# proycon/analiticcl

Hardware: AMD Instinct MI355X
Metric: scored (query,candidate) pairs/sec + queries/sec, 200k-lexicon, len≤16, 1/2/4/8 GPU (higher is better)
Workload: dtype u8

## Files before the change

### analiticcl_amd/csrc/conf.hip

```cpp
#include <hip/hip_runtime.h>

#include <mutex>
#include <string>
#include <vector>

#include <rocprim/device/device_radix_sort.hpp>

#include "engine_internal.h"

namespace anx {

#define HIP_TRY(expr)                                                                          \
  do {                                                                                         \
    hipError_t _e = (expr);                                                                    \
    if (_e != hipSuccess) {                                                                    \
      err = std::string(#expr) + ": " + hipGetErrorString(_e);                                 \
      return ANX_ENODEVICE;                                                                    \
    }                                                                                          \
  } while (0)

#include "kernels_common.hpp"

struct DeviceConf {
  int device = 0;
// ... 96 lines not shown
      if (need) {
        const uint32_t nin = t1 - t0, c0 = a.v_off[id], ncand = a.v_off[id + 1] - c0, nmin = nin < ncand ? nin : ncand;
        uint32_t p = 0;
        while (p < nmin) {
          const uint32_t x = a.text[t0 + p];
          if (x >= 128u || x != a.v_pool[c0 + p]) break;
          ++p;
        }
        uint32_t sfx = 0;
        while (sfx < nmin - p) {
          const uint32_t x = a.text[t1 - 1u - sfx];
          if (x >= 128u || x != a.v_pool[c0 + ncand - 1u - sfx]) break;
          ++sfx;
        }
        uint64_t im0 = 0, im1 = 0, cm0 = 0, cm1 = 0;
        for (uint32_t x = p; x < nin - sfx; ++x) {
          const uint32_t ch = a.text[t0 + x];
          if (ch < 64u) im0 |= 1ull << ch; else if (ch < 128u) im1 |= 1ull << (ch - 64u);
        }
        for (uint32_t x = p; x < ncand - sfx; ++x) {
          const uint32_t ch = a.v_pool[c0 + x];
          if (ch < 64u) cm0 |= 1ull << ch; else if (ch < 128u) cm1 |= 1ull << (ch - 64u);
        }
        need = false;
        for (uint32_t j = 0; j < a.P.nconf && !need; ++j) {
          const cdiff::FlatConf& cf = a.P.conf[j];
          bool may = true;
          for (uint32_t o_ = 0; o_ < cf.nops && may; ++o_) {
            const cdiff::FlatOp& o = a.P.ops[cf.op_begin + o_];
            if (!o.simple) continue;
            uint64_t h0 = o.bits[0], h1 = o.bits[1];
            if (o.op == '-') { h0 &= im0; h1 &= im1; }
            else if (o.op == '+') { h0 &= cm0; h1 &= cm1; }
            else { h0 &= ins.w[0] & cs.w[0]; h1 &= ins.w[1] & cs.w[1]; }
            if (!(h0 | h1)) may = false;
          }
          need = may;
        }
      }
    }
    a.weight[slot] = 1.0;
    if (need) {
      if (k < 64u) needmask |= 1ull << k;
      else a.need[atomicAdd(&a.ctr[0], 1u)] = make_uint2(slot, s);
    }
  }
  const uint32_t cnt = (uint32_t)__popcll(needmask), lane = threadIdx.x & 63u;
  uint32_t incl = cnt;
#pragma unroll
  for (int o = 1; o < 64; o <<= 1) {
    const uint32_t up = (uint32_t)__shfl_up((int)incl, o);
    if ((int)lane >= o) incl += up;
  }
  const uint32_t total = (uint32_t)__shfl((int)incl, 63);
  if (total == 0) return;
  uint32_t first = 0;
  if (lane == 0) first = atomicAdd(&a.ctr[0], total);
  uint32_t pos = (uint32_t)__shfl((int)first, 0) + incl - cnt;
  for (unsigned long long m = needmask; m; m &= m - 1ull) a.need[pos++] = make_uint2(base + (uint32_t)__ffsll((long long)m) - 1u, s);
}

__global__ void k_conf_iota(uint32_t* p, uint32_t n) {
  const uint32_t i = blockIdx.x * 256 + threadIdx.x;
  if (i < n) p[i] = i;
}
__global__ __launch_bounds__(256) void k_conf_key(ConfArgs a) {
  const uint32_t k = blockIdx.x * 256 + threadIdx.x;
  if (k >= a.row_cap) return;
  uint32_t key = 0x1FFFu;
  if (k < a.ctr[0]) {
    const uint32_t slot = a.need[k].x, s = a.need[k].y, id = row_item(a, slot);
    const uint32_t i = a.q_orig[s], t0 = a.textoff[i], nin = a.textoff[i + 1] - 1u - t0;
    const uint32_t c0 = a.v_off[id], ncand = a.v_off[id + 1] - c0;
    const uint32_t nmin = nin < ncand ? nin : ncand;
    uint32_t p = 0;
    while (p < nmin) {
      const uint32_t x = a.text[t0 + p];
      if (x >= 128u || x != a.v_pool[c0 + p]) break;
      ++p;
    }
    uint32_t sfx = 0;
    while (sfx < nmin - p) {
      const uint32_t x = a.text[t0 + nin - 1u - sfx];
      if (x >= 128u || x != a.v_pool[c0 + ncand - 1u - sfx]) break;
      ++sfx;
    }
    const uint32_t ma = nin - p - sfx, mb = ncand - p - sfx;
    key = ((ma < 6u ? ma : 6u) << 5) | ((mb < 6u ? mb : 6u) << 2) | (p ? 2u : 0u) | (sfx ? 1u : 0u);
    key = key << 5 | (nin < 31u ? nin : 31u);
  }
  a.key[k] = key;
}

__global__ __launch_bounds__(CF_THREADS) void k_conf_script(ConfArgs a) {
  const uint32_t n = a.ctr[0];
  static_assert(CF_THREADS == 64, "one wave per block: the lane memories of a wave interleave");
  cdiff::Ctx c;
  c.mem = a.work + (size_t)blockIdx.x * CF_WORDS * 64u + threadIdx.x * CF_G;
  c.arena_off = CF_ARENA_OFF; c.arena_cap = CF_ARENA; c.arena_used = 0;
  c.d_off = CF_D_OFF; c.d_cap = CF_DIFFS; c.nd = 0;
  c.v_off = CF_V_OFF; c.v_cap = CF_V;
  c.f_off = CF_F_OFF; c.frame_cap = CF_FRAMES;
  c.alpha = a.alpha; c.nalpha = a.nalpha;
  c.overflow = false;
  for (uint32_t k = blockIdx.x * CF_THREADS + threadIdx.x; k < n; k += gridDim.x * CF_THREADS) {
    const uint2 nd = a.need[a.order[k]];
    const uint32_t slot = nd.x, s = nd.y, id = row_item(a, slot);
    const uint32_t i = a.q_orig[s], t0 = a.textoff[i], t1 = a.textoff[i + 1] - 1u;
    uint32_t nin = 0;
    bool fits = true;
    for (uint32_t p = t0; p < t1;) {
      const uint32_t b0 = a.text[p];
      uint32_t cp = b0, len = 1;
      const uint32_t avail = t1 - p;
      if (b0 >= 0xC0u && b0 < 0xE0u && avail >= 2 && (a.text[p + 1] & 0xC0u) == 0x80u) { cp = ((b0 & 0x1Fu) << 6) | (a.text[p + 1] & 0x3Fu); len = 2; }
      else if (b0 >= 0xE0u && b0 < 0xF0u && avail >= 3 && (a.text[p + 1] & 0xC0u) == 0x80u && (a.text[p + 2] & 0xC0u) == 0x80u) {
        cp = ((b0 & 0x0Fu) << 12) | ((a.text[p + 1] & 0x3Fu) << 6) | (a.text[p + 2] & 0x3Fu); len = 3;
      } else if (b0 >= 0xF0u && b0 < 0xF8u && avail >= 4 && (a.text[p + 1] & 0xC0u) == 0x80u && (a.text[p + 2] & 0xC0u) == 0x80u && (a.text[p + 3] & 0xC0u) == 0x80u) {
        cp = ((b0 & 0x07u) << 18) | ((a.text[p + 1] & 0x3Fu) << 12) | ((a.text[p + 2] & 0x3Fu) << 6) | (a.text[p + 3] & 0x3Fu); len = 4;
      }
      if (nin >= CF_MAXCP) { fits = false; break; }
      DC::W(c, CF_IN_OFF + nin++) = cp;
      p += len;
    }
    const uint32_t c0 = a.v_off[id], ncand = a.v_off[id + 1] - c0;
    double w = 1.0;
    bool ok = fits && ncand <= CF_MAXCP;
    if (ok) {
      for (uint32_t x = 0; x < ncand; ++x) DC::W(c, CF_CAND_OFF + x) = a.v_pool[c0 + x];
      const cdiff::View in = cdiff::mk(CF_IN_OFF, nin), cand = cdiff::mk(CF_CAND_OFF, ncand);
      ok = DC::confusable_weight(c, a.P, in, DC::charset_of(c, in), cand, a.v_cs[id], &w);
    }
    if (!ok) atomicAdd(&a.ctr[1], 1u);
    a.weight[slot] = w;
  }
}

__global__ __launch_bounds__(256) void k_conf_apply_early(ConfArgs a) {
  const uint32_t slot = blockIdx.x * 256 + threadIdx.x;
  if (slot >= a.soff[a.nq] || a.soff[a.nq] > a.row_cap) return;
  const double w = a.weight[slot];
  if (w != 1.0) a.c_rows[slot].score *= w;
}

__device__ inline double conf_vr_score(const DevRow& r, float fw) {
  if (fw == 0.0f) return r.dist_score;
  return (r.dist_score + ((double)fw * r.freq_score)) / (1.0 + (double)fw);
}
__device__ inline bool conf_before(const DevRow& x, const DevRow& y, float fw) {
  if (fw > 0.0f) return conf_vr_score(x, fw) > conf_vr_score(y, fw);
  if (x.dist_score != y.dist_score) return x.dist_score > y.dist_score;
  return x.freq_score > y.freq_score;
}
__global__ __launch_bounds__(256) void k_conf_apply_late(ConfArgs a, uint32_t* __restrict__ r_count) {
  const uint32_t s = blockIdx.x * 256 + threadIdx.x;
  if (s >= a.nq || a.soff[a.nq] > a.row_cap || *a.overflow) return;
  const uint32_t n = r_count[s], base = a.soff[s];
  if (n == 0) return;
  DevRow* __restrict__ v = a.r_rows + base;
  bool any = false;
  for (uint32_t k = 0; k < n; ++k) {
    const double w = a.weight[base + k];
    if (w != 1.0) { v[k].dist_score *= w; any = true; }
  }
  if (any)
    for (uint32_t k = 1; k < n; ++k) {
      const DevRow x = v[k];
      uint32_t j = k;
      while (j > 0 && conf_before(x, v[j - 1], a.freq_weight)) { v[j] = v[j - 1]; --j; }
      v[j] = x;
    }
  uint32_t len = n;
  if (a.cutoff_threshold >= 1.0) {
    const double best = conf_vr_score(v[0], a.freq_weight);
    for (uint32_t k = 1; k < n; ++k)
      if (conf_vr_score(v[k], a.freq_weight) <= best / a.cutoff_threshold) { len = k; break; }
  }
  r_count[s] = len;
}

namespace {
std::mutex g_conf_mu;
template <typename T>
int cf_upload(T** dst, const void* src, size_t count, std::string& err) {
  if (*dst) { pool_free(*dst); *dst = nullptr; }
  HIP_TRY(pool_malloc(reinterpret_cast<void**>(dst), std::max<size_t>(count * sizeof(T), 16)));
  if (count) HIP_TRY(hipMemcpy(*dst, src, count * sizeof(T), hipMemcpyHostToDevice));
  return ANX_OK;
}
}

void conf_free(DeviceConf* dc) {
  if (!dc) return;
  (void)hipSetDevice(dc->device);
  for (void* p : {(void*)dc->conf, (void*)dc->ops, (void*)dc->opts, (void*)dc->pool, (void*)dc->v_pool, (void*)dc->v_off, (void*)dc->v_cs, (void*)dc->alpha})
    if (p) pool_free(p);
  delete dc;
}

static int conf_ensure(const HostModel& m, const DeviceLexicon* dl, std::string& err) {
  std::lock_guard<std::mutex> g(g_conf_mu);
  DeviceConf*& dc = dl->dconf;
  if (!dc) { dc = new DeviceConf(); dc->device = dl->device; }
  int rc;
  if (dc->built_patterns != m.confusables.size() || !dc->conf) {
    const HostModel::ConfTables& t = m.conf_tables;
    if ((rc = cf_upload(&dc->conf, t.conf.data(), t.conf.size(), err)) || (rc = cf_upload(&dc->ops, t.ops.data(), t.ops.size(), err)) ||
        (rc = cf_upload(&dc->opts, t.opts.data(), t.opts.size(), err)) || (rc = cf_upload(&dc->pool, t.pool.data(), t.pool.size(), err)))
      return rc;
    dc->nconf = (uint32_t)t.conf.size();
    dc->built_patterns = m.confusables.size();
  }
  if (dc->built_vocab != m.decoder.size() || !dc->v_cs) {
    const uint32_t *pool, *off;
    const void* cs;
    size_t npool, n;
    m.conf_vocab_arrays(&pool, &npool, &off, &cs, &n);
    if ((rc = cf_upload(&dc->v_pool, pool, npool, err)) || (rc = cf_upload(&dc->v_off, off, n + 1, err)) ||
        (rc = cf_upload(&dc->v_cs, cs, n, err)))
      return rc;
    dc->nvocab = (uint32_t)n;
    dc->built_vocab = m.decoder.size();
  }
  if (!dc->alpha) {
    uint32_t na = 0;
    const uint32_t(*al)[2] = alphabetic_ranges(&na);
    uint32_t* p = nullptr;
    if ((rc = cf_upload(&p, al, (size_t)na * 2, err))) return rc;
    dc->alpha = reinterpret_cast<uint32_t(*)[2]>(p);
    dc->nalpha = na;
  }
  return ANX_OK;
}

int conf_launch(const HostModel& m, const DeviceLexicon* dl, Batch* b, hipStream_t st, bool early, uint32_t row_cap, std::string& err) {
  int rc = conf_ensure(m, dl, err);
  if (rc) return rc;
  b->conf_skipped = false;
  const DeviceConf* dc = dl->dconf;
  const uint32_t nq = (uint32_t)b->nq;
  if (!b->cf_weight || b->cf_cap < row_cap) {
    for (void* p : {(void*)b->cf_weight, (void*)b->cf_need, (void*)b->cf_sort, b->cf_sort_tmp})
      if (p) pool_free(p);
    b->cf_weight = nullptr; b->cf_need = nullptr; b->cf_sort = nullptr; b->cf_sort_tmp = nullptr;
    HIP_TRY(pool_malloc(reinterpret_cast<void**>(&b->cf_weight), std::max<size_t>((size_t)row_cap * sizeof(double), 16)));
    HIP_TRY(pool_malloc(reinterpret_cast<void**>(&b->cf_need), std::max<size_t>((size_t)row_cap * sizeof(uint2), 16)));
    b->cf_cap = row_cap;
  }
  if (!b->cf_sort) {
    HIP_TRY(pool_malloc(reinterpret_cast<void**>(&b->cf_sort), std::max<size_t>(4 * (size_t)row_cap * sizeof(uint32_t), 16)));
    size_t bytes = 0;
    HIP_TRY(rocprim::radix_sort_pairs(nullptr, bytes, b->cf_sort, b->cf_sort, b->cf_sort, b->cf_sort, (size_t)row_cap, 0u, 13u, st));
    HIP_TRY(pool_malloc(&b->cf_sort_tmp, std::max<size_t>(bytes, 16)));
    b->cf_sort_tmp_bytes = bytes;
  }
  uint32_t* sort_buf = b->cf_sort;
  if (!b->cf_ctr) HIP_TRY(pool_malloc(reinterpret_cast<void**>(&b->cf_ctr), 16));
  const uint32_t cf_blocks = std::min<uint32_t>(CF_BLOCKS, std::max<uint32_t>(1u, (row_cap + 63u) / 64u));
  if (b->cf_work && b->cf_work_blocks < cf_blocks) { pool_free(b->cf_work); b->cf_work = nullptr; }
  if (!b->cf_work) {
    if (pool_malloc(&b->cf_work, (size_t)cf_blocks * CF_WORDS * 64u * sizeof(uint32_t)) != hipSuccess) {
      b->cf_work = nullptr;
      (void)hipGetLastError();
      b->conf_skipped = true;
      return ANX_OK;
    }
    b->cf_work_blocks = cf_blocks;
  }
  HIP_TRY(hipMemsetAsync(b->cf_ctr, 0, 16, st));
  ConfArgs a;
  a.nq = nq; a.row_cap = row_cap; a.early = early ? 1 : 0; a.soff = b->soff; a.r_count = b->r_count; a.c_rows = b->c_rows; a.r_rows = b->r_rows;
  a.overflow = b->counters + CTR_OVERFLOW;
  a.q_orig = b->q_orig; a.text = b->d_text; a.textoff = b->d_textoff; a.weight = b->cf_weight; a.need = reinterpret_cast<uint2*>(b->cf_need); a.ctr = b->cf_ctr;
  a.P.conf = dc->conf; a.P.nconf = dc->nconf; a.P.ops = dc->ops; a.P.opts = dc->opts; a.P.pool = dc->pool;
  a.v_pool = dc->v_pool; a.v_off = dc->v_off; a.v_cs = dc->v_cs; a.nvocab = dc->nvocab;
  a.alpha = dc->alpha; a.nalpha = dc->nalpha; a.work = static_cast<uint32_t*>(b->cf_work);
  a.key = sort_buf; a.order = sort_buf + 3 * (size_t)row_cap;
  a.cutoff_threshold = b->params.cutoff_threshold; a.freq_weight = b->params.freq_weight;
  const uint32_t nblk = (row_cap + 255u) / 256u;
  hipLaunchKernelGGL(k_conf_screen, dim3((nq + 255u) / 256u), dim3(256), 0, st, a);
  if (nblk) {
    hipLaunchKernelGGL(k_conf_key, dim3(nblk), dim3(256), 0, st, a);
    hipLaunchKernelGGL(k_conf_iota, dim3(nblk), dim3(256), 0, st, sort_buf + (size_t)row_cap, row_cap);
    HIP_TRY(rocprim::radix_sort_pairs(b->cf_sort_tmp, b->cf_sort_tmp_bytes, sort_buf, sort_buf + 2 * (size_t)row_cap, sort_buf + (size_t)row_cap,
                                      sort_buf + 3 * (size_t)row_cap, (size_t)row_cap, 0u, 13u, st));
  }
  const int kt = ktimer_begin("k_conf_script", st);
  hipLaunchKernelGGL(k_conf_script, dim3(b->cf_work_blocks), dim3(CF_THREADS), 0, st, a);
  ktimer_end(kt, st);
  if (early) { if (nblk) hipLaunchKernelGGL(k_conf_apply_early, dim3(nblk), dim3(256), 0, st, a); }
  else hipLaunchKernelGGL(k_conf_apply_late, dim3((nq + 255u) / 256u), dim3(256), 0, st, a, b->r_count);
  HIP_TRY(hipGetLastError());
  return ANX_OK;
}

}
```

### analiticcl_amd/csrc/engine.hip

```cpp
#include <hip/hip_runtime.h>

#include <algorithm>
#include <atomic>
#include <functional>
#include <chrono>
#include <cmath>
#include <cstdio>
#include <cstdlib>
#include <cstring>
#include <map>
#include <memory>
#include <mutex>
#include <unordered_map>
#include <numeric>
#include <thread>
#include <type_traits>

#include "engine_internal.h"

namespace anx {

#define HIP_TRY(expr)                                                                          \
  do {                                                                                         \
    hipError_t _e = (expr);                                                                    \
    if (_e != hipSuccess) {                                                                    \
      err = std::string(#expr) + ": " + hipGetErrorString(_e);                                 \
      return ANX_ENODEVICE;                                                                    \
    }                                                                                          \
  } while (0)

#include "kernels_common.hpp"
#include "kernels_swar.hpp"
#include "kernels_scan.hpp"
#include "kernels_prefix.hpp"
#include "kernels_score.hpp"
#include "kernels_rank.hpp"

enum { HR_RCTR = 0, HR_SCTR = SCAN_REGIONS * RC_STRIDE, HR_LCTR = 2 * SCAN_REGIONS * RC_STRIDE, HR_CTR = 5 * SCAN_REGIONS * RC_STRIDE,
       HR_TOTAL_SURV = HR_CTR + CTR_N, HR_TOTAL_RESULTS = HR_TOTAL_SURV + 1, HR_CONF = HR_TOTAL_RESULTS + 1 , HR_N = HR_CONF + 2 };
constexpr size_t HR_COLD_OFF = (HR_N * sizeof(uint32_t) + 63) & ~(size_t)63;
static void shells_destroy(int device);
static void small_ctxs_destroy(int device);

int device_count(std::string& err) {
  int n = 0;
  hipError_t e = hipGetDeviceCount(&n);
  if (e != hipSuccess) {
    err = std::string("hipGetDeviceCount: ") + hipGetErrorString(e);
    return 0;
  }
  return n;
}

struct SmallCtx;
namespace {
struct DevPool {
  std::mutex mu;
  std::multimap<size_t, void*> free_blocks;
  std::unordered_map<void*, size_t> size_of;
  size_t cached = 0;
  std::unordered_map<void*, uint64_t> freed_at;
  uint64_t clock = 0;
  int lexicons = 0;
  std::vector<hipStream_t> idle_streams;
  hipStream_t run_streams[2] = {nullptr, nullptr};
  unsigned run_counter = 0;
  std::vector<BatchShell> shells;
  std::vector<SmallCtx*> small_idle;
  std::vector<std::pair<void*, size_t>> doomed;
  size_t doomed_bytes = 0;
};
static size_t pool_cache_limit() {
  static const size_t lim = []() {
    const char* e = getenv("ANX_POOL_CACHE_MB");
    const long long v = e ? atoll(e) : -1;
    return v >= 0 ? (size_t)v << 20 : (size_t)96 << 30;
  }();
  return lim;
}
DevPool& pool_of(int device) {
  static DevPool pools[64];
  return pools[device >= 0 && device < 64 ? device : 0];
}
}
static thread_local hipStream_t t_encoder_stream = nullptr;
void* make_stream(bool high) {
  hipStream_t s = nullptr;
  int least = 0, greatest = 0;
  if (high && switches().enc_priority && hipDeviceGetStreamPriorityRange(&least, &greatest) == hipSuccess && greatest < least) {
    if (hipStreamCreateWithPriority(&s, hipStreamNonBlocking, greatest) == hipSuccess) return s;
    (void)hipGetLastError();
  }
  if (hipStreamCreateWithFlags(&s, hipStreamNonBlocking) != hipSuccess) { (void)hipGetLastError(); return nullptr; }
  return s;
}
void encoder_stream_set_override(void* s) { t_encoder_stream = reinterpret_cast<hipStream_t>(s); }
hipStream_t encoder_stream_acquire(int device) {
  if (t_encoder_stream) return t_encoder_stream;
  DevPool& pl = pool_of(device);
  {
    std::lock_guard<std::mutex> g(pl.mu);
    if (!pl.idle_streams.empty()) { hipStream_t s = pl.idle_streams.back(); pl.idle_streams.pop_back(); return s; }
  }
  return static_cast<hipStream_t>(make_stream(true));
}
void encoder_stream_release(int device, hipStream_t s) {
  if (!s || s == t_encoder_stream) return;
  DevPool& pl = pool_of(device);
  std::lock_guard<std::mutex> g(pl.mu);
  pl.idle_streams.push_back(s);
}
struct DeviceGuard {
  int prev = -1;
  DeviceGuard() { if (hipGetDevice(&prev) != hipSuccess) { prev = -1; (void)hipGetLastError(); } }
  ~DeviceGuard() { if (prev >= 0) (void)hipSetDevice(prev); }
};
void* thread_stream_begin(int device) {
  if (t_encoder_stream) return nullptr;
  DeviceGuard guard;
  if (hipSetDevice(device) != hipSuccess) { (void)hipGetLastError(); return nullptr; }
  hipStream_t s = encoder_stream_acquire(device);
  t_encoder_stream = s;
  return s;
}
void thread_stream_end(int device, void* s) {
  if (!s) return;
  t_encoder_stream = nullptr;
  encoder_stream_release(device, reinterpret_cast<hipStream_t>(s));
}
void* stream_create(int device, std::string& err, bool high_priority) {
  DeviceGuard guard;
  void* s = nullptr;
  if (hipSetDevice(device) != hipSuccess || !(s = make_stream(high_priority))) {
    err = std::string("hipStreamCreate: ") + hipGetErrorString(hipGetLastError());
    return nullptr;
  }
  return s;
}
void stream_destroy(int device, void* s) {
  DeviceGuard guard;
  if (!s) return;
  (void)hipSetDevice(device);
  (void)hipStreamDestroy(reinterpret_cast<hipStream_t>(s));
}

static void pool_reap(DevPool& pl) {
  std::vector<std::pair<void*, size_t>> drop;
  { std::lock_guard<std::mutex> g(pl.mu); drop.swap(pl.doomed); pl.doomed_bytes = 0; }
  for (auto& d : drop) (void)hipFree(d.first);
}
hipError_t pool_malloc(void** p, size_t bytes) {
  int dev = 0;
  (void)hipGetDevice(&dev);
  DevPool& pl = pool_of(dev);
  bytes = (bytes + 255) & ~(size_t)255;
  {
    std::lock_guard<std::mutex> g(pl.mu);
    auto it = pl.free_blocks.lower_bound(bytes);
    if (it != pl.free_blocks.end() && it->first <= 2 * bytes + (1u << 20)) {
      *p = it->second;
      pl.cached -= it->first;
      pl.free_blocks.erase(it);
      pl.freed_at.erase(*p);
      return hipSuccess;
    }
  }
  pool_reap(pl);
  hipError_t e = hipMalloc(p, bytes);
  if (e != hipSuccess) {
    std::vector<void*> drop;
    {
      std::lock_guard<std::mutex> g(pl.mu);
      for (auto& kv : pl.free_blocks) { drop.push_back(kv.second); pl.size_of.erase(kv.second); }
      pl.free_blocks.clear();
      pl.freed_at.clear();
      pl.cached = 0;
    }
    for (void* d : drop) (void)hipFree(d);
    (void)hipGetLastError();
    e = hipMalloc(p, bytes);
    if (e != hipSuccess) return e;
  }
  std::lock_guard<std::mutex> g(pl.mu);
  pl.size_of[*p] = bytes;
  return hipSuccess;
}
void pool_free(void* p) {
  if (!p) return;
  int dev = 0;
  (void)hipGetDevice(&dev);
  DevPool& pl = pool_of(dev);
  std::vector<void*> evicted;
// ... 576 lines not shown
      memcpy(&h_qrec[2 * s], row, 16);
      {
        uint32_t pw[3];
        symbol_planes16(reinterpret_cast<const uint8_t*>(row), e.meta & 0xFFu, pw);
        h_qrec[2 * s + 1] = make_uint4(e.meta, pw[0], pw[1], pw[2]);
      }
      h_meta[s] = e.meta;
      h_orig[s] = (uint32_t)i;
      h_kind[s] = e.kind;
      h_sig[s] = e.sig;
    }
  };
  {
    std::vector<std::thread> th;
    for (unsigned t = 0; t < nthreads; ++t) {
      const size_t lo = nq * t / nthreads, hi = nq * (t + 1) / nthreads;
      if (nthreads == 1) fill_range(lo, hi);
      else th.emplace_back(fill_range, lo, hi);
    }
    for (auto& x : th) x.join();
  }
  lap("fill device images");
  for (size_t i = 0; i < nq;) {
    size_t j = i;
    const bool sad = h_kind[i] == 0;
    while (j < nq && (h_kind[j] == 0) == sad && (h_meta[j] & 0xFF) == (h_meta[i] & 0xFF) && h_sig[j] == h_sig[i]) ++j;
    const uint32_t lq = h_meta[i] & 0xFF, k = (h_meta[i] >> 8) & 0xFF;
    const int lo = std::max<int>(1, (int)lq - (int)k), hi = std::min<int>(kMaxSymbols, (int)lq + (int)k);
    const uint32_t s0 = m.lex.siglen_begin[lo] & ~63u, s1 = (m.lex.siglen_begin[hi + 1] + 63u) & ~63u;
    const uint32_t tq = scan_tq_of(sig_group_count(m.lex.sym_group));
    uint32_t ball0 = 0, balln = 0;
    if (probe_enabled() && k <= 12 && tile_probes(dl->ball_n[k], s1 - s0, h_sig[i])) { ball0 = dl->ball_off[k]; balln = dl->ball_n[k]; }
    const uint32_t nsplit = (sad && !balln) ? 8u : 1u;
    const uint32_t step = (((s1 - s0) + nsplit - 1) / nsplit + 63u) & ~63u;
    uint32_t adj = 0;
    if (!sad && k <= (uint32_t)kAdjRadius && switches().scan_adj && dl->adj_mask && dl->adj_hash_host.empty()) {
      const int rca = adjacency_host_copies(dl, err);
      if (rca) return rca;
    }
    if (!sad && k <= (uint32_t)kAdjRadius && switches().scan_adj && !dl->adj_hash_host.empty()) {
      uint32_t h = sig_hash((uint32_t)h_sig[i], (uint32_t)(h_sig[i] >> 32)) & dl->adj_mask;
      for (int pr = 0; pr < 17; ++pr) {
        const AdjSlot& e = dl->adj_hash_host[h];
        if (!e.hdr1) break;
        if (e.lo == (uint32_t)h_sig[i] && e.hi == (uint32_t)(h_sig[i] >> 32)) { adj = e.hdr1; break; }
        h = (h + 1u) & dl->adj_mask;
      }
    }
    for (size_t s = i; s < j; s += tq) {
      const uint32_t tn = (uint32_t)std::min<size_t>(tq, j - s);
      uint32_t ke[3] = {0, 0, 0};
      for (uint32_t x = 0; x < tn; ++x)
        for (uint32_t kd = h_kind[s + x]; kd >= 1 && kd <= 3; ++kd) ke[kd - 1]++;
      const uint32_t kend = sad ? 0u : (ke[0] | ke[1] << 8 | ke[2] << 16);
      for (uint32_t part = 0; part < nsplit; ++part) {
        const uint32_t a0 = s0 + part * step, a1 = std::min(s1, a0 + step);
        if (a0 >= a1 && part) break;
        b->tiles.push_back(Tile{(uint32_t)s, tn, a0, a1, k, lq, (uint32_t)h_sig[i], (uint32_t)(h_sig[i] >> 32), sad ? 0u : 1u,
                                (h_meta[i] >> 16) & 0xFFu, kend, ball0, balln, adj, (s == i && part == 0u) ? 1u : 0u});
      }
    }
    i = j;
  }
  auto tile_cost = [&](const Tile& x) {
    return x.adj ? (uint64_t)dl->adj_hdr_host[x.adj - 1].cum[kAdjSections - 1] * (8u + x.nq) + 16u : (uint64_t)x.nq * (x.s1 - x.s0 + 64);
  };
  std::stable_sort(b->tiles.begin(), b->tiles.end(), [&](const Tile& x, const Tile& y) {
    if ((x.kind == 0) != (y.kind == 0)) return y.kind == 0;
    if ((x.adj == 0) != (y.adj == 0)) return y.adj == 0;
    return tile_cost(x) > tile_cost(y);
  });
  b->n_adj_tiles = 0;
  for (const Tile& t : b->tiles) { b->n_sad_tiles += t.kind == 0; b->n_adj_tiles += t.adj != 0; }
  lap("tiles + LPT order");
  std::vector<uint32_t> h_xcls(nq, 0xFFFFFFFFu);
  if (p.stop_at_exact_match) {
    auto lookup_range = [&](size_t lo, size_t hi) {
      std::string key(cvbytes, '\0');
      for (size_t s = lo; s < hi; ++s) {
        memcpy(&key[0], &cv_all[(size_t)b->order[s] * cvbytes], cvbytes);
        auto it = m.class_of_cv.find(key);
        if (it != m.class_of_cv.end()) h_xcls[s] = it->second;
      }
    };
    std::vector<std::thread> th;
    for (unsigned t = 0; t < nthreads; ++t) {
      const size_t lo = nq * t / nthreads, hi = nq * (t + 1) / nthreads;
      if (nthreads == 1) lookup_range(lo, hi);
      else th.emplace_back(lookup_range, lo, hi);
    }
    for (auto& x : th) x.join();
  }
  int rc;
  if ((rc = upload(&b->q_rec, h_qrec.data(), h_qrec.size(), err, nullptr)) ||
      (rc = upload(&b->qexact, h_xcls.data(), nq, err, nullptr)) ||
      (rc = upload(&b->q_cv, h_cv.data(), h_cv.size(), err, nullptr)) ||
      (rc = upload(&b->q_bits, h_bits.data(), h_bits.size(), err, nullptr)) ||
      (rc = upload(reinterpret_cast<uint8_t**>(&b->q_rows), h_rows.data(), h_rows.size(), err, nullptr)) ||
      (rc = upload(&b->q_meta, h_meta.data(), nq, err, nullptr)) || (rc = upload(&b->q_orig, h_orig.data(), nq, err, nullptr)) ||
      (rc = upload(&b->d_tiles, b->tiles.data(), b->tiles.size(), err, nullptr)))
    return rc;
  b->ntiles = (uint32_t)b->tiles.size();
  std::vector<Tile>().swap(b->tiles);
  lap("uploads");
  return ANX_OK;
}

static int shell_acquire(Batch* b, std::string& err) {
  DevPool& pl = pool_of(b->device);
  BatchShell sh;
  bool have = false;
  {
    std::lock_guard<std::mutex> g(pl.mu);
    if (!pl.shells.empty()) { sh = pl.shells.back(); pl.shells.pop_back(); have = true; }
  }
  if (!have) {
    for (auto& e : sh.ev) HIP_TRY(hipEventCreate(&e));
    HIP_TRY(hipEventCreate(&sh.ev_fs0));
    HIP_TRY(hipEventCreate(&sh.ev_fs1));
    HIP_TRY(hipEventCreate(&sh.ev_scan0));
    HIP_TRY(hipEventCreate(&sh.ev_done));
    HIP_TRY(hipEventCreateWithFlags(&sh.ev_in, hipEventDisableTiming));
    HIP_TRY(hipHostMalloc(reinterpret_cast<void**>(&sh.h_read), HR_COLD_OFF + sizeof(FsCold), hipHostMallocDefault));
  }
  for (int i = 0; i < 6; ++i) b->ev[i] = sh.ev[i];
  b->ev_fs0 = sh.ev_fs0; b->ev_fs1 = sh.ev_fs1; b->ev_scan0 = sh.ev_scan0; b->ev_done = sh.ev_done; b->ev_in = sh.ev_in; b->h_read = sh.h_read;
  return ANX_OK;
}
static void shell_release(Batch* b) {
  if (!b->ev_done) return;
  BatchShell sh;
  for (int i = 0; i < 6; ++i) { sh.ev[i] = b->ev[i]; b->ev[i] = nullptr; }
  sh.ev_fs0 = b->ev_fs0; sh.ev_fs1 = b->ev_fs1; sh.ev_scan0 = b->ev_scan0; sh.ev_done = b->ev_done; sh.ev_in = b->ev_in; sh.h_read = b->h_read;
  b->ev_fs0 = b->ev_fs1 = b->ev_scan0 = b->ev_done = b->ev_in = nullptr; b->h_read = nullptr;
  DevPool& pl = pool_of(b->device);
  std::lock_guard<std::mutex> g(pl.mu);
  pl.shells.push_back(sh);
}
static void shells_destroy(int device) {
  DevPool& pl = pool_of(device);
  std::vector<BatchShell> drop;
  { std::lock_guard<std::mutex> g(pl.mu); drop.swap(pl.shells); }
  for (BatchShell& sh : drop) {
    for (auto& e : sh.ev) if (e) (void)hipEventDestroy(e);
    for (hipEvent_t e : {sh.ev_fs0, sh.ev_fs1, sh.ev_scan0, sh.ev_done, sh.ev_in}) if (e) (void)hipEventDestroy(e);
    if (sh.h_read) (void)hipHostFree(sh.h_read);
  }
}

static int encode_tail(Batch* b, std::string& err) {
  const size_t nq = b->nq;
  int rc;
  const size_t nblk = (nq + SCAN_TILE - 1) / SCAN_TILE + 2;
  if ((rc = dalloc(&b->counters, CTR_N, err)) || (rc = dalloc(&b->rctr, SCAN_REGIONS * RC_STRIDE, err)) || (rc = dalloc(&b->sctr, SCAN_REGIONS * RC_STRIDE, err)) || (rc = dalloc(&b->lctr, 3 * SCAN_REGIONS * RC_STRIDE, err)) || (rc = dalloc(&b->qexpand, nq, err)) || (rc = dalloc(&b->qsurv, nq, err)) ||
      (rc = dalloc(&b->soff, nq + 1, err)) || (rc = dalloc(&b->qcur, nq, err)) || (rc = dalloc(&b->qmaxfreq, nq, err)) ||
      (rc = dalloc(&b->scan_tmp, nblk, err)) || (rc = dalloc(&b->r_count, nq, err)) || (rc = dalloc(&b->r_off, nq + 1, err)))
    return rc;
  return shell_acquire(b, err);
}

Batch* batch_encode_spans(const HostModel& m, const DeviceLexicon* dl, const char* blob, size_t blob_bytes, const uint32_t* off, size_t n,
                          const anx_params& p, std::string& err, int* code, bool keep_text, bool blob_on_device, bool after_stream, void* src_stream) {
  *code = ANX_OK;
  if (blob_on_device && (off || switches().encode_host)) { err = "inputs in device memory need the device-side encoder and no host offsets"; *code = ANX_EINVAL; return nullptr; }
  if (!dl) { err = "model is not resident on a device (no HIP device / anx_model_to_device not called)"; *code = ANX_ENODEVICE; return nullptr; }
  if (hipSetDevice(dl->device) != hipSuccess) { err = "hipSetDevice failed"; *code = ANX_ENODEVICE; return nullptr; }
  if (n >= (1u << 27)) { err = "more than 2^27 inputs per batch"; *code = ANX_ELIMIT; return nullptr; }
  Batch* b = new Batch();
  b->device = dl->device;
  b->params = p;
  b->n_input = n;
  b->keep_text = keep_text;
  int rc;
  if (switches().encode_host) {
    std::vector<uint32_t> hoff;
    if (!off) {
      if (!packed_offsets(blob, blob_bytes, n, hoff)) { err = "packed inputs hold fewer strings than announced"; *code = ANX_EINVAL; batch_free(b); return nullptr; }
      off = hoff.data();
    }
    std::vector<const char*> ptrs(n);
    for (size_t i = 0; i < n; ++i) ptrs[i] = blob + off[i];
    rc = encode_host(m, dl, b, ptrs.data(), n, p, err);
    if (!rc && keep_text) {
      const size_t bytes = n ? (size_t)off[n] : 0;
      std::vector<uint32_t> o(off, off + n + 1);
      if (!n) o.assign(1, 0u);
      if ((rc = upload(&b->d_text, blob, bytes, err, nullptr)) == 0) rc = upload(&b->d_textoff, o.data(), o.size(), err, nullptr);
      b->text_bytes = bytes;
    }
  } else {
    rc = batch_encode_device(m, dl, b, blob, blob_bytes, off, n, p, err, blob_on_device, after_stream, src_stream);
  }
  if (!rc) rc = encode_tail(b, err);
  if (rc) { *code = rc; batch_free(b); return nullptr; }
  return b;
}

Batch* batch_encode(const HostModel& m, const DeviceLexicon* dl, const char* const* utf8, size_t n, const anx_params& p,
                    std::string& err, int* code, bool keep_text) {
  std::vector<uint32_t> off(n + 1, 0);
  unsigned nthreads = std::max(1u, std::min(16u, usable_hw_threads()));
  if (n < 16384) nthreads = 1;
  std::vector<size_t> part(nthreads + 1, 0);
  auto run_threads = [&](const std::function<void(unsigned, size_t, size_t)>& f) {
    std::vector<std::thread> th;
    for (unsigned t = 0; t < nthreads; ++t) {
      const size_t lo = n * t / nthreads, hi = n * (t + 1) / nthreads;
      if (nthreads == 1) f(0, lo, hi);
      else th.emplace_back(f, t, lo, hi);
    }
    for (auto& x : th) x.join();
  };
  std::vector<uint32_t> lens(n);
  std::atomic<bool> too_big{false};
  run_threads([&](unsigned t, size_t lo, size_t hi) {
    size_t sum = 0;
    for (size_t i = lo; i < hi; ++i) {
      const size_t l = utf8[i] ? strlen(utf8[i]) : 0;
      if (l >= (1u << 28)) too_big.store(true, std::memory_order_relaxed);
      lens[i] = (uint32_t)l;
      sum += l + 1;
    }
    part[t + 1] = sum;
  });
  for (unsigned t = 0; t < nthreads; ++t) part[t + 1] += part[t];
  if (too_big.load() || part[nthreads] >= ((size_t)1 << 32)) { err = "inputs exceed 4 GB per batch: split the batch"; *code = ANX_ELIMIT; return nullptr; }
  HostBuf<char> blob(part[nthreads] + 1);
  if (!blob.data()) { err = "out of memory"; *code = ANX_ELIMIT; return nullptr; }
  run_threads([&](unsigned t, size_t lo, size_t hi) {
    size_t pos = part[t];
    for (size_t i = lo; i < hi; ++i) {
      off[i] = (uint32_t)pos;
      if (lens[i]) memcpy(&blob[pos], utf8[i], lens[i]);
      blob[pos + lens[i]] = '\0';
      pos += (size_t)lens[i] + 1;
    }
  });
  off[n] = (uint32_t)part[nthreads];
  return batch_encode_spans(m, dl, blob.data(), blob.size(), off.data(), n, p, err, code, keep_text);
}

static int exclusive_scan(const uint32_t* in, uint32_t n, uint32_t* out, uint32_t* tmp, hipStream_t st, uint32_t* maxout = nullptr, uint32_t* copy = nullptr) {
  const uint32_t nb = (n + SCAN_TILE - 1) / SCAN_TILE;
  if (nb == 0) return hipMemsetAsync(out, 0, sizeof(uint32_t), st) == hipSuccess ? 0 : -1;
  hipLaunchKernelGGL(k_scan_local, dim3(nb), dim3(SCAN_THREADS), 0, st, in, n, out, tmp, maxout);
  hipLaunchKernelGGL(k_scan_sums, dim3(1), dim3(SCAN_THREADS), 0, st, tmp, nb);
  hipLaunchKernelGGL(k_scan_add, dim3(nb), dim3(SCAN_THREADS), 0, st, out, n, tmp, nb, copy);
  return 0;
}

namespace {
struct KTimerRec { std::string name; hipEvent_t e0 = nullptr, e1 = nullptr; int device = 0; bool closed = false; };
struct KTimer {
  std::mutex mu;
  std::atomic<bool> on{false};
  std::vector<KTimerRec> pending;
  uint32_t generation = 0;
  std::map<std::string, std::pair<double, uint64_t>> acc;
};
KTimer& ktimer() { static KTimer* t = new KTimer; return *t; }
void ktimer_resolve_locked(KTimer& t) {
  for (KTimerRec& r : t.pending) {
    if (r.closed && hipEventSynchronize(r.e1) == hipSuccess) {
      float ms = 0.f;
      if (hipEventElapsedTime(&ms, r.e0, r.e1) == hipSuccess) { auto& a = t.acc[r.name]; a.first += ms; a.second += 1; }
    }
    if (r.e0) (void)hipEventDestroy(r.e0);
    if (r.e1) (void)hipEventDestroy(r.e1);
  }
  t.pending.clear();
  ++t.generation;
}
}
int ktimer_begin(const char* name, hipStream_t st) {
  KTimer& t = ktimer();
  if (!t.on.load(std::memory_order_relaxed)) return -1;
  KTimerRec r;
  r.name = name;
  if (hipEventCreate(&r.e0) != hipSuccess || hipEventCreate(&r.e1) != hipSuccess || hipEventRecord(r.e0, st) != hipSuccess) {
    if (r.e0) (void)hipEventDestroy(r.e0);
    if (r.e1) (void)hipEventDestroy(r.e1);
    return -1;
  }
  std::lock_guard<std::mutex> lk(t.mu);
  if (t.pending.size() >= 0xFFFFu) return -1;
  t.pending.push_back(r);
  return (int)(((t.generation & 0x7FFFu) << 16) | (uint32_t)(t.pending.size() - 1));
}
void ktimer_end(int handle, hipStream_t st) {
  if (handle < 0) return;
  KTimer& t = ktimer();
  std::lock_guard<std::mutex> lk(t.mu);
  const uint32_t idx = (uint32_t)handle & 0xFFFFu;
  if ((((uint32_t)handle >> 16) & 0x7FFFu) != (t.generation & 0x7FFFu) || idx >= t.pending.size()) return;
  KTimerRec& r = t.pending[idx];
  if (hipEventRecord(r.e1, st) == hipSuccess) r.closed = true;
}
void kernel_timer_enable(bool on) {
  KTimer& t = ktimer();
  std::lock_guard<std::mutex> lk(t.mu);
  ktimer_resolve_locked(t);
  t.acc.clear();
  t.on.store(on);
}
bool kernel_timer_read(const char* name, double* total_ms, uint64_t* launches) {
  KTimer& t = ktimer();
  std::lock_guard<std::mutex> lk(t.mu);
  ktimer_resolve_locked(t);
  auto it = t.acc.find(name ? name : "");
  if (it == t.acc.end()) { if (total_ms) *total_ms = 0.0; if (launches) *launches = 0; return false; }
  if (total_ms) *total_ms = it->second.first;
  if (launches) *launches = it->second.second;
  return true;
}

#include "launch_plan.hpp"

template <int NP>
static void launch_scan(ScanArgs A, uint32_t nadj, uint32_t nbits, uint32_t nsad, hipStream_t st, hipEvent_t e0, hipEvent_t e1) {
  (void)hipEventRecord(e0, st);
  const bool gen = A.want_exact || A.qpairs || !A.drop_len;
  if (nadj) {
    A.ntiles = nadj;
    if (gen) hipLaunchKernelGGL((k_scan_adj<true>), dim3((nadj + 3) / 4), dim3(256), 0, st, A);
    else hipLaunchKernelGGL((k_scan_adj<false>), dim3((nadj + 3) / 4), dim3(256), 0, st, A);
    A.tiles += nadj;
    nbits -= nadj;
  }
  if (nbits) {
    A.ntiles = nbits;
    if (A.want_exact || A.qpairs || !A.drop_len) hipLaunchKernelGGL((k_scan_bits<true>), dim3((nbits + 3) / 4), dim3(256), 0, st, A);
    else hipLaunchKernelGGL((k_scan_bits<false>), dim3((nbits + 3) / 4), dim3(256), 0, st, A);
  }
  (void)hipEventRecord(e1, st);
  if (nsad) {
    A.tiles += nbits;
    A.ntiles = nsad;
    hipLaunchKernelGGL((k_scan_sad<NP>), dim3((nsad + 3) / 4), dim3(256), 0, st, A);
  }
}

static int ensure_raw(Batch* b, size_t slots_per_region, std::string& err) {
  uint32_t shift = 10;
  while (((size_t)1 << shift) < slots_per_region) ++shift;
  if (shift > 25) { err = "pair list exceeds 2^31 slots: split the batch"; return ANX_ELIMIT; }
  const size_t cap = (size_t)SCAN_REGIONS << shift;
  if (cap <= b->raw_cap) return ANX_OK;
  for (void* p : {(void*)b->raw, (void*)b->p_score, (void*)b->p_meta})
    if (p) pool_free(p);
  b->raw = nullptr; b->p_score = nullptr; b->p_meta = nullptr; b->raw_cap = 0;
  int rc;
  if ((rc = dalloc(&b->raw, cap, err))) return rc;
  b->raw_cap = cap;
  b->region_shift = shift;
  return ANX_OK;
}
static int ensure_pair_outputs(Batch* b, std::string& err) {
  if (b->p_meta) return ANX_OK;
  int rc;
  if ((rc = dalloc(&b->p_score, b->raw_cap, err)) || (rc = dalloc(&b->p_meta, b->raw_cap, err))) return rc;
  return ANX_OK;
}

static int ensure_surv(Batch* b, size_t cap, std::string& err) {
  if (cap <= b->surv_cap) return ANX_OK;
  for (void* p : {(void*)b->c_rows, (void*)b->r_rows, (void*)b->t_key})
    if (p) pool_free(p);
  b->c_rows = nullptr;
  b->r_rows = nullptr;
  b->t_key = nullptr;
  b->surv_cap = 0;
  int rc;
  if ((rc = dalloc(&b->c_rows, cap, err)) || (rc = dalloc(&b->r_rows, cap, err)) || (rc = dalloc(&b->t_key, cap, err))) return rc;
  b->surv_cap = cap;
  return ANX_OK;
}
static int ensure_surv_records(Batch* b, size_t need, std::string& err) {
  if (need <= b->surv_region_cap) return ANX_OK;
  if (b->surv) pool_free(b->surv);
  b->surv = nullptr;
  b->surv_region_cap = 0;
  int rc;
  if ((rc = dalloc(&b->surv, need * SCAN_REGIONS, err))) return rc;
  b->surv_region_cap = need;
  return ANX_OK;
}
static int ensure_slot_lists(Batch* b, size_t need, std::string& err) {
  if (need <= b->list_cap) return ANX_OK;
  for (void* p : {(void*)b->list8, (void*)b->listg, (void*)b->listw})
    if (p) pool_free(p);
  b->list8 = b->listg = b->listw = nullptr;
  b->list_cap = 0;
  int rc;
  if ((rc = dalloc(&b->list8, need * SCAN_REGIONS, err)) || (rc = dalloc(&b->listg, need * SCAN_REGIONS, err)) || (rc = dalloc(&b->listw, need * SCAN_REGIONS, err))) return rc;
  b->list_cap = need;
  return ANX_OK;
}


static size_t cap_div() { return (size_t)switches().cap_div; }

constexpr size_t kSegBudget = (size_t)4 << 30;
static uint32_t seg_wanted(const Batch* b) {
  const uint32_t C = (uint32_t)switches().surv_seg;
  return (b->conf_mode == 2 || b->params.stop_at_exact_match || b->params.freq_weight != 0.0f) ? 0u : C;
}
static uint32_t seg_capacity(const DeviceLexicon* dl, Batch* b) {
  const uint32_t C = seg_wanted(b);
  if (!C || dl->any_variants) return 0;
  const size_t need = b->nq * (size_t)C;
  if (need * sizeof(SurvSeg) > kSegBudget) return 0;
  if (need > b->sseg_cap) {
    if (b->sseg) pool_free(b->sseg);
    b->sseg = nullptr;
    b->sseg_cap = 0;
    std::string e;
    if (dalloc(&b->sseg, need, e)) { (void)hipGetLastError(); return 0; }
    b->sseg_cap = need;
  }
  return C;
}
static bool same_threshold(const anx_threshold& a, const anx_threshold& b) { return a.kind == b.kind && a.value == b.value && a.ratio == b.ratio; }
static bool hints_match(const RunHints& h, const Batch* b) {
  return h.valid && same_threshold(h.kth, b->params.max_anagram_distance) && same_threshold(h.dth, b->params.max_edit_distance) &&
         h.score_threshold == b->params.score_threshold && h.stop == (b->params.stop_at_exact_match ? 1 : 0) && h.seg == seg_wanted(b);
}
static void hints_apply(const DeviceLexicon* dl, Batch* b) {
  if (b->runs_finished || b->hinted || b->prev_maxfill || !switches().hints || switches().cap_div != 1 || b->nq < 4096) return;
  RunHints& h = dl->hints;
  std::lock_guard<std::mutex> g(h.mu);
  if (!hints_match(h, b)) return;
  const double nq = (double)b->nq, m = 1.25;
  const double worst_fill = (nq * 140.0 + (double)b->ntiles * SCAN_CHUNK) / SCAN_REGIONS + 4096.0;
  const double fill = h.maxfill * nq * m + 8192.0;
  if (fill >= worst_fill) return;
  b->prev_maxfill = (uint32_t)fill;
  b->prev_surv_fill = (uint32_t)(h.surv_fill * nq * m + 1024.0);
  b->prev_list_fill = h.list_fill > 0 ? (uint32_t)(h.list_fill * nq * m + 1024.0) : 0u;
  b->hint_rows = (size_t)std::min(nq * 16.0 + 1024.0, h.total_surv * nq * m + 4096.0);
  b->hinted = true;
}
static void hints_record(const DeviceLexicon* dl, const Batch* b, uint32_t maxfill, uint32_t surv_fill, uint32_t list_fill, uint32_t total_surv) {
  if (b->nq < 4096 || !switches().hints) return;
  RunHints& h = dl->hints;
  std::lock_guard<std::mutex> g(h.mu);
  const double nq = (double)b->nq, decay = hints_match(h, b) ? 0.9 : 0.0;
  h.maxfill = std::max(maxfill / nq, h.maxfill * decay);
  h.surv_fill = std::max(surv_fill / nq, h.surv_fill * decay);
  h.list_fill = std::max(list_fill / nq, h.list_fill * decay);
  h.total_surv = std::max(total_surv / nq, h.total_surv * decay);
  h.kth = b->params.max_anagram_distance; h.dth = b->params.max_edit_distance; h.score_threshold = b->params.score_threshold;
  h.stop = b->params.stop_at_exact_match ? 1 : 0;
  h.seg = seg_wanted(b);
  h.nq = nq;
  h.valid = true;
}

namespace {
struct Run {
  const HostModel& m;
  const DeviceLexicon* dl;
  Batch* b;
  hipStream_t st;
  std::string& err;
  uint32_t nq;
  int stop;
  uint32_t region_cap = 0, fill_cap = 0;
  SurvOut so{};
  int setup(), scan(), score(), compact_rank(), readback();
};
}

int Run::setup() {
  int rc;
  hints_apply(dl, b);
  if (b->raw_cap == 0 && b->hinted && (rc = ensure_raw(b, (size_t)b->prev_maxfill + (b->prev_maxfill >> 3) + 4096, err))) return rc;
  if (b->raw_cap == 0 && (rc = ensure_raw(b, (nq * (size_t)140 + (size_t)b->ntiles * SCAN_CHUNK) / SCAN_REGIONS / cap_div() + 4096, err)))
    return rc;
  region_cap = 1u << b->region_shift;
  fill_cap = b->prev_maxfill ? (uint32_t)std::min<size_t>(region_cap, (size_t)b->prev_maxfill + (b->prev_maxfill >> 3) + FS_BLK) : region_cap;
  b->fill_cap_launched = fill_cap;
  HIP_TRY(hipEventRecord(b->ev[0], st));
  return ANX_OK;
}

int Run::scan() {
  int rc;
  HIP_TRY(hipMemsetAsync(b->counters, 0, CTR_N * sizeof(uint32_t), st));
  HIP_TRY(hipMemsetAsync(b->rctr, 0, SCAN_REGIONS * RC_STRIDE * sizeof(uint32_t), st));
  if (b->ntiles == 0) { HIP_TRY(hipEventRecord(b->ev_scan0, st)); HIP_TRY(hipEventRecord(b->ev[5], st)); }
  if (b->ntiles) {
    ScanArgs A = scan_args_of(dl);
    A.tiles = b->d_tiles; A.ntiles = b->ntiles; A.q_bits = b->q_bits; A.q_cv = b->q_cv;
    A.chunk = SCAN_CHUNK;
    A.chunk_fused = switches().scan_chunk_fused ? (uint32_t)switches().scan_chunk_fused : SCAN_CHUNK_FUSED;
#ifdef ANX_DEBUG_SWITCHES
    { const char* e = getenv("ANX_SCAN_CHUNK"); const int v = e ? atoi(e) : 0; if (v >= 32 && v <= 1024) A.chunk = (uint32_t)v; }
#endif
    A.raw = b->raw; A.region_cap = region_cap; A.rctr = b->rctr; A.qexact = b->qexact; A.want_exact = stop;
    A.drop_len = (!stop && !b->keep_all_pairs) ? 1 : 0;
    A.q_rec = b->q_rec;
    A.fuse = (switches().fuse_prefilter && switches().prefilter && A.drop_len) ? 1 : 0;
    A.qpairs = nullptr;
    if (b->count_pairs) {
      if (!b->qpairs && (rc = dalloc(&b->qpairs, nq, err))) return rc;
      HIP_TRY(hipMemsetAsync(b->qpairs, 0, nq * sizeof(uint32_t), st));
      A.qpairs = b->qpairs;
    }
    A.dbg = 0;
#ifdef ANX_DEBUG_SWITCHES
    { const char* e = getenv("ANX_SCAN_DBG"); A.dbg = e ? atoi(e) : 0; }
#endif
    const uint32_t nsad = b->n_sad_tiles, nbits = A.ntiles - nsad, nadj = std::min(b->n_adj_tiles, nbits);
    with_nplanes(dl->nplanes, [&](auto np) { launch_scan<decltype(np)::value>(A, nadj, nbits, nsad, st, b->ev_scan0, b->ev[5]); });
  }
  HIP_TRY(hipMemcpyAsync(b->h_read + HR_RCTR, b->rctr, SCAN_REGIONS * RC_STRIDE * sizeof(uint32_t), hipMemcpyDeviceToHost, st));
  HIP_TRY(hipEventRecord(b->ev[1], st));
  b->n_raw = (uint32_t)(SCAN_REGIONS << b->region_shift);
  return ANX_OK;
}

int Run::score() {
  int rc;
  HIP_TRY(hipMemsetAsync(b->qsurv, 0, nq * sizeof(uint32_t), st));
  HIP_TRY(hipMemsetAsync(b->qmaxfreq, 0, nq * sizeof(uint32_t), st));
  if (dl->any_variants) HIP_TRY(hipMemsetAsync(b->qexpand, 0, nq * sizeof(uint32_t), st));
  ScorePlan plan = score_plan_of(m, dl, b->params.score_threshold, b->qw, b->dmax);
  ScoreArgs& sa = plan.sa;
#ifdef ANX_DEBUG_SWITCHES
  { const char* e = getenv("ANX_SCORE_DBG"); sa.dbg = e ? atoi(e) : 0; }
#endif
  sa.store_pairs = b->keep_all_pairs ? 1 : 0;
  if (sa.store_pairs && (rc = ensure_pair_outputs(b, err))) return rc;
  if (!plan.fits()) { err = "per-lane scoring state exceeds the LDS budget"; return ANX_ELIMIT; }
  const int fastD = plan.fastD;
  if ((rc = ensure_surv_records(b, b->prev_surv_fill ? (size_t)b->prev_surv_fill + (b->prev_surv_fill >> 3) + 256 : (size_t)fill_cap / 2 / cap_div() + 256, err))) return rc;
  so = SurvOut{b->surv, b->sctr, (uint32_t)b->surv_region_cap, nullptr, seg_capacity(dl, b)};
  so.seg = so.seg_cap ? b->sseg : nullptr;
  const bool need_lists = !fastD || plan.have_long_q || dl->max_len > 16;
  if (need_lists && (rc = ensure_slot_lists(b, b->prev_list_fill ? (size_t)b->prev_list_fill + (b->prev_list_fill >> 3) + 256 : (fastD ? (size_t)fill_cap / 2 : (size_t)fill_cap) / cap_div() + 256, err)))
    return rc;
  HIP_TRY(hipMemsetAsync(b->sctr, 0, SCAN_REGIONS * RC_STRIDE * sizeof(uint32_t), st));
  HIP_TRY(hipMemsetAsync(b->lctr, 0, 3 * SCAN_REGIONS * RC_STRIDE * sizeof(uint32_t), st));
  const SlotLists sl = slot_lists_of(b->list8, b->listg, b->listw, b->lctr, (uint32_t)b->list_cap);
  const PairArgs pa = pair_args_of(dl, b->raw, b->q_meta, b->q_rows, b->q_rec, b->p_score, b->p_meta, b->qmaxfreq, b->qsurv, b->qexpand);
  FilterArgs fa;
  fa.region_shift = b->region_shift; fa.rctr = b->rctr; fa.qexact = b->qexact; fa.stop = stop; fa.enable = plan.enable_filter;
  fa.use_nw8 = (plan.have_long_q || fastD > 0) ? 1 : 0; fa.counters = b->counters; fa.stat_ctr = b->sctr; fa.fill_cap = fill_cap; fa.blk = FS_BLK;
  const dim3 fgrid(((fill_cap + FS_BLK - 1) / FS_BLK) * SCAN_REGIONS);
  {
    FsCold* cold = reinterpret_cast<FsCold*>(reinterpret_cast<char*>(b->h_read) + HR_COLD_OFF);
    *cold = FsCold{sa, so, sl.l8, sl.lg, sl.lw};
    if (!b->d_cold && (rc = dalloc(reinterpret_cast<char**>(&b->d_cold), sizeof(FsCold), err))) return rc;
    HIP_TRY(hipMemcpyAsync(b->d_cold, cold, sizeof(FsCold), hipMemcpyHostToDevice, st));
  }
  HIP_TRY(hipEventRecord(b->ev_fs0, st));
  launch_filter_score(plan, fgrid, st, fa, pa, static_cast<const FsCold*>(b->d_cold));
  HIP_TRY(hipEventRecord(b->ev_fs1, st));
  if (need_lists) {
    const dim3 lgrid(LIST_P * SCAN_REGIONS);
    if (plan.split_wide && plan.enable_filter) hipLaunchKernelGGL(k_filter_wide, lgrid, dim3(256), 0, st, sl.lw, fa, pa, sa, fastD, sl.l8, sl.lg);
    if (fastD) launch_score_fast8(fastD, lgrid, st, sl.l8, pa, sa, so);
    hipLaunchKernelGGL(k_score_pairs, lgrid, dim3(plan.threads), plan.lds_bytes(), st, sl.lg, pa, sa, so);
  }
  HIP_TRY(hipEventRecord(b->ev[2], st));
  return ANX_OK;
}

int Run::compact_rank() {
  int rc;
  const RankArgs ra = rank_args_of(m, dl, b->params, b->conf_mode == 1 ? 0.0 : b->params.cutoff_threshold);
  exclusive_scan(b->qsurv, nq, b->soff, b->scan_tmp, st, nullptr, b->qcur);
  if (dl->any_variants) {
    uint32_t total_surv = 0;
    HIP_TRY(hipMemcpyAsync(&total_surv, b->soff + nq, sizeof(uint32_t), hipMemcpyDeviceToHost, st));
    HIP_TRY(hipMemcpyAsync(b->h_read + HR_SCTR, b->sctr, SCAN_REGIONS * RC_STRIDE * sizeof(uint32_t), hipMemcpyDeviceToHost, st));
    HIP_TRY(hipStreamSynchronize(st));
    uint32_t surv_fill = 0;
    for (uint32_t r = 0; r < SCAN_REGIONS; ++r) surv_fill = std::max(surv_fill, b->h_read[HR_SCTR + r * RC_STRIDE]);
    if ((size_t)surv_fill > b->surv_region_cap) {
      surv_fill = 0;
      HIP_TRY(hipMemsetAsync(b->counters + CTR_OVERFLOW, 0xFF, sizeof(uint32_t), st));
    }
    if ((rc = ensure_surv(b, (size_t)total_surv + (total_surv >> 2) + 1024, err))) return rc;
    if (surv_fill) {
      CompactArgs ca{m.have_freq ? 1 : 0, dl->any_variants};
      hipLaunchKernelGGL(k_compact, dim3(((surv_fill + 255) / 256) * SCAN_REGIONS), dim3(256), 0, st, b->surv, b->sctr,
                         (uint32_t)b->surv_region_cap, ca, b->qcur, dl->ent_rec, dl->ent_var_off, dl->var_target,
                         dl->var_target_freq, dl->var_score, b->c_rows);
    }
  } else if (b->surv_cap == 0 && (rc = ensure_surv(b, b->hint_rows ? b->hint_rows : (size_t)nq * 16 / cap_div() + 1024, err))) return rc;
  const uint32_t row_cap = (uint32_t)std::min<size_t>(b->surv_cap, 0xFFFFFFFFu);
  if (!dl->any_variants)
    hipLaunchKernelGGL(k_compact_grouped, dim3(COMPACT_P * SCAN_REGIONS), dim3(COMPACT_B), 0, st, b->surv, b->sctr,
                       (uint32_t)b->surv_region_cap, m.have_freq ? 1 : 0, b->qcur, dl->ent_rec, b->c_rows, b->soff + nq, row_cap,
                       b->counters + CTR_OVERFLOW);
  HIP_TRY(hipEventRecord(b->ev[3], st));
  if (b->conf_mode == 2 && (rc = conf_launch(m, dl, b, st, true, row_cap, err))) return rc;
  launch_rank(ra, st, nq, b->soff, b->c_rows, b->qmaxfreq, b->qexpand, b->t_key, b->r_rows, b->r_count, dl->any_variants ? 0xFFFFFFFFu : row_cap, b->counters + CTR_OVERFLOW,
              dl->any_variants ? SegRows{nullptr, 0u, nullptr} : SegRows{so.seg, so.seg_cap, dl->ent_rec});
  if (b->conf_mode == 1 && (rc = conf_launch(m, dl, b, st, false, row_cap, err))) return rc;
  exclusive_scan(b->r_count, nq, b->r_off, b->scan_tmp, st, b->counters + CTR_MAXROWS);
  HIP_TRY(hipEventRecord(b->ev[4], st));
  return ANX_OK;
}

int Run::readback() {
  HIP_TRY(hipMemcpyAsync(b->h_read + HR_SCTR, b->sctr, SCAN_REGIONS * RC_STRIDE * sizeof(uint32_t), hipMemcpyDeviceToHost, st));
  HIP_TRY(hipMemcpyAsync(b->h_read + HR_LCTR, b->lctr, 3 * SCAN_REGIONS * RC_STRIDE * sizeof(uint32_t), hipMemcpyDeviceToHost, st));
  HIP_TRY(hipMemcpyAsync(b->h_read + HR_CTR, b->counters, CTR_N * sizeof(uint32_t), hipMemcpyDeviceToHost, st));
  HIP_TRY(hipMemcpyAsync(b->h_read + HR_TOTAL_SURV, b->soff + nq, sizeof(uint32_t), hipMemcpyDeviceToHost, st));
  HIP_TRY(hipMemcpyAsync(b->h_read + HR_TOTAL_RESULTS, b->r_off + nq, sizeof(uint32_t), hipMemcpyDeviceToHost, st));
  b->h_read[HR_CONF] = b->h_read[HR_CONF + 1] = 0;
  if (b->conf_mode && b->cf_ctr) HIP_TRY(hipMemcpyAsync(b->h_read + HR_CONF, b->cf_ctr, 2 * sizeof(uint32_t), hipMemcpyDeviceToHost, st));
  HIP_TRY(hipEventRecord(b->ev_done, st));
  HIP_TRY(hipGetLastError());
  return ANX_OK;
}

static int batch_launch(const HostModel& m, const DeviceLexicon* dl, Batch* b, void* stream, std::string& err) {
  if (!dl) { err = "model is not resident on a device"; return ANX_ENODEVICE; }
  if (b->nq >= (1u << 27) || dl->nentries >= (1u << 26)) { err = "more than 2^27 queries per batch or 2^26 lexicon entries (32-bit record offsets, packed pair records)"; return ANX_ELIMIT; }
  HIP_TRY(hipSetDevice(dl->device));
  if (b->launched) {
    HIP_TRY(hipEventSynchronize(b->ev_done));
    b->launched = false;
  }
  b->last_stream = stream;
  b->ran = false;
  b->ran_keep_all = b->keep_all_pairs;
  b->n_pairs = b->n_results = b->n_surv = 0;
  b->n_raw = 0;
  if (b->nq == 0) { b->ran = true; return ANX_OK; }
  Run r{m, dl, b, reinterpret_cast<hipStream_t>(stream), err, (uint32_t)b->nq, b->params.stop_at_exact_match ? 1 : 0};
  int rc;
  if ((rc = r.setup()) || (rc = r.scan()) || (rc = r.score()) || (rc = r.compact_rank()) || (rc = r.readback())) return rc;
  b->launched = true;
  return ANX_OK;
}

static int batch_finish(const HostModel& m, const DeviceLexicon* dl, Batch* b, bool* retry, std::string& err) {
  (void)m;
  *retry = false;
  if (!b->launched) return ANX_OK;
  HIP_TRY(hipSetDevice(dl->device));
  HIP_TRY(hipEventSynchronize(b->ev_done));
  b->launched = false;
  const uint32_t nq = (uint32_t)b->nq;
  const uint32_t* h = b->h_read;
  uint32_t maxfill = 0, surv_fill = 0, list_fill = 0;
  uint64_t n_valid = 0, n_slots = 0, nsel = 0, n_fused = 0, n_adj_rows = 0, n_adj_rows_first = 0;
  b->n_class_tests = 0;
  for (int i = 0; i <= NBITPLANES; ++i) b->n_tests_kind[i] = 0;
  for (uint32_t r = 0; r < SCAN_REGIONS; ++r) {
    const uint32_t* c = h + HR_RCTR + r * RC_STRIDE;
    maxfill = std::max(maxfill, c[RC_RAW]);
    b->region_fill[r] = c[RC_RAW];
    n_slots += c[RC_RAW];
    n_valid += c[RC_VALID];
    n_fused += c[RC_FUSED];
    n_adj_rows += c[RC_ADJ];
    n_adj_rows_first += c[RC_ADJ_FIRST];
    for (int i = 0; i <= NBITPLANES; ++i) {
      uint64_t v;
      memcpy(&v, c + RC_TESTS + 2 * i, sizeof v);
      b->n_tests_kind[i] += v;
      b->n_class_tests += v;
    }
    surv_fill = std::max(surv_fill, h[HR_SCTR + r * RC_STRIDE]);
    nsel += h[HR_SCTR + r * RC_STRIDE + 1];
    for (int l = 0; l < 3; ++l) list_fill = std::max(list_fill, h[HR_LCTR + (l * SCAN_REGIONS + r) * RC_STRIDE]);
  }
  const uint32_t total_surv = h[HR_TOTAL_SURV], total_results = h[HR_TOTAL_RESULTS];
  b->conf_fallback = b->conf_mode != 0 && (h[HR_CONF + 1] != 0 || b->conf_skipped);
  b->stats.n_conf_scripts = b->conf_mode ? h[HR_CONF] : 0;
  b->stats.n_adj_tiles = std::min(b->n_adj_tiles, b->ntiles - b->n_sad_tiles);
  int rc;
  bool again = false;
  if (maxfill > (1u << b->region_shift)) {
    if ((rc = ensure_raw(b, (size_t)maxfill + (maxfill >> 3) + 4096, err))) return rc;
    again = true;
  }
  if (maxfill > b->fill_cap_launched) again = true;
  if ((size_t)surv_fill > b->surv_region_cap) again = true;
  if (list_fill && (size_t)list_fill > b->list_cap) again = true;
  if (!dl->any_variants && (size_t)total_surv > b->surv_cap) {
    if ((rc = ensure_surv(b, (size_t)total_surv + (total_surv >> 2) + 1024, err))) return rc;
    again = true;
  }
  b->prev_maxfill = std::max(b->prev_maxfill, maxfill);
  b->prev_surv_fill = std::max(b->prev_surv_fill, surv_fill);
  b->prev_list_fill = std::max(b->prev_list_fill, list_fill);
  if (again) { *retry = true; b->runs_finished++; return ANX_OK; }
  if (b->runs_finished++ == 0) hints_record(dl, b, maxfill, surv_fill, list_fill, total_surv);
  if (maxfill == 0) b->n_raw = 0;
  b->n_pairs = n_valid - h[HR_CTR + CTR_SKIPPED];
  b->n_surv = total_surv;
  b->n_sel = nsel;
  b->n_results = total_results;
  b->max_rows = h[HR_CTR + CTR_MAXROWS];
  b->ran = true;
  anx_batch_stats& s = b->stats;
  s.n_queries = nq;
  s.n_pairs = b->n_pairs;
  s.n_class_tests = b->n_class_tests;
  s.n_results = total_results;
  s.n_scan_blocks = b->ntiles;
  for (int i = 0; i <= NBITPLANES; ++i) s.n_tests_kind[i] = b->n_tests_kind[i];
  s.n_pair_slots = n_slots;
  s.n_survivors = total_surv;
  s.n_selected = b->n_sel;
  s.n_prefiltered_in_scan = n_fused;
  s.n_adj_records = n_adj_rows * kAdjRow;
  s.n_adj_records_first = n_adj_rows_first * kAdjRow;
  (void)hipEventElapsedTime(&s.ms_scan, b->ev[0], b->ev[1]);
  (void)hipEventElapsedTime(&s.ms_score, b->ev[1], b->ev[2]);
  (void)hipEventElapsedTime(&s.ms_group, b->ev[2], b->ev[3]);
  (void)hipEventElapsedTime(&s.ms_rank, b->ev[3], b->ev[4]);
  (void)hipEventElapsedTime(&s.ms_total, b->ev[0], b->ev[4]);
  (void)hipEventElapsedTime(&s.ms_scan_kernel, b->ev_scan0, b->ev[5]);
  (void)hipEventElapsedTime(&s.ms_filter_score_kernel, b->ev_fs0, b->ev_fs1);
  return ANX_OK;
}

int batch_run_async(const HostModel& m, const DeviceLexicon* dl, Batch* b, void* stream, bool own_streams, std::string& err) {
  void* use = stream;
  if (own_streams && dl && switches().run_overlap) {
    HIP_TRY(hipSetDevice(dl->device));
    DevPool& pl = pool_of(dl->device);
    hipStream_t s = nullptr;
    {
      std::lock_guard<std::mutex> g(pl.mu);
      hipStream_t& slot = pl.run_streams[pl.run_counter++ & 1u];
      if (!slot && hipStreamCreateWithFlags(&slot, hipStreamNonBlocking) != hipSuccess) { (void)hipGetLastError(); slot = nullptr; }
      s = slot;
    }
    if (s) {
      HIP_TRY(hipEventRecord(b->ev_in, reinterpret_cast<hipStream_t>(stream)));
      HIP_TRY(hipStreamWaitEvent(s, b->ev_in, 0));
      use = s;
    }
  }
  const int rc = batch_launch(m, dl, b, use, err);
  if (rc == ANX_OK && use != stream) b->last_stream = stream;
  return rc;
}
int batch_wait(const HostModel& m, const DeviceLexicon* dl, Batch* b, std::string& err) {
  for (int attempt = 0;; ++attempt) {
    bool retry = false;
    int rc = batch_finish(m, dl, b, &retry, err);
    if (rc || !retry) return rc;
    if (attempt == 3) { err = "the run did not fit its buffers after three regrows"; return ANX_ENODEVICE; }
    if ((rc = batch_launch(m, dl, b, b->last_stream, err))) return rc;
  }
}
int batch_run(const HostModel& m, const DeviceLexicon* dl, Batch* b, void* stream, std::string& err) {
  const int rc = batch_launch(m, dl, b, stream, err);
  return rc ? rc : batch_wait(m, dl, b, err);
}

void batch_set_last_stream(Batch* b, void* stream) { if (b && !b->launched) b->last_stream = stream; }
size_t batch_n_results(const Batch* b) { return b->ran ? (size_t)b->n_results : 0; }
size_t batch_n_input(const Batch* b) { return b->n_input; }

static size_t scan_tmp_bytes(size_t n) { return ((n + SCAN_TILE - 1) / SCAN_TILE + 2) * sizeof(uint32_t); }
template <typename Emit>
static int enqueue_rows(const Batch* b, uint32_t* d_cnt, uint32_t* d_off, uint32_t* d_tmp, hipStream_t st, const Emit& emit, std::string& err) {
  const uint32_t n32 = (uint32_t)b->n_input, nq32 = (uint32_t)b->nq;
  HIP_TRY(hipMemsetAsync(d_cnt, 0, n32 * sizeof(uint32_t), st));
  hipLaunchKernelGGL(k_fetch_counts, dim3((nq32 + 255) / 256), dim3(256), 0, st, nq32, b->r_count, b->q_orig, d_cnt);
  exclusive_scan(d_cnt, n32, d_off, d_tmp, st);
  hipLaunchKernelGGL(k_emit_rows<Emit>, dim3((nq32 + 255) / 256), dim3(256), 0, st, nq32, b->soff, b->r_count, b->r_rows, b->q_orig, d_off, emit);
  return ANX_OK;
}

template <typename Row, typename Off, typename MakeEmit>
static int fetch_rows(const Batch* b, Row* out, Off* off, uint32_t* via, Off base, const MakeEmit& make_emit, std::string& err) {
  if (!b->ran) { err = "batch has not been run"; return ANX_EINVAL; }
  HIP_TRY(hipSetDevice(b->device));
  const size_t n = b->n_input;
  if (!b->nq || !b->n_results) {
    for (size_t i = 0; i <= n; ++i) off[i] = base;
    return ANX_OK;
  }
  uint32_t *d_cnt = nullptr, *d_off = nullptr, *d_tmp = nullptr, *d_via = nullptr;
  Row* d_out = nullptr;
  hipStream_t st = reinterpret_cast<hipStream_t>(b->last_stream);
  auto body = [&]() -> int {
    HIP_TRY(pool_malloc(reinterpret_cast<void**>(&d_cnt), n * sizeof(uint32_t)));
    HIP_TRY(pool_malloc(reinterpret_cast<void**>(&d_off), (n + 1) * sizeof(uint32_t)));
    HIP_TRY(pool_malloc(reinterpret_cast<void**>(&d_tmp), scan_tmp_bytes(n)));
    HIP_TRY(pool_malloc(reinterpret_cast<void**>(&d_out), b->n_results * sizeof(Row)));
    if (via) HIP_TRY(pool_malloc(reinterpret_cast<void**>(&d_via), b->n_results * sizeof(uint32_t)));
    if (const int rc = enqueue_rows(b, d_cnt, d_off, d_tmp, st, make_emit(d_out, d_via), err)) return rc;
    std::vector<uint32_t> staged;
    uint32_t* h_off;
    if constexpr (sizeof(Off) == sizeof(uint32_t)) h_off = off;
    else { staged.resize(n + 1); h_off = staged.data(); }
    HIP_TRY(hipMemcpyAsync(h_off, d_off, (n + 1) * sizeof(uint32_t), hipMemcpyDeviceToHost, st));
    HIP_TRY(hipMemcpyAsync(out, d_out, b->n_results * sizeof(Row), hipMemcpyDeviceToHost, st));
    if (via) HIP_TRY(hipMemcpyAsync(via, d_via, b->n_results * sizeof(uint32_t), hipMemcpyDeviceToHost, st));
    HIP_TRY(hipStreamSynchronize(st));
    if (base || !staged.empty())
      for (size_t i = 0; i <= n; ++i) off[i] = base + h_off[i];
    return ANX_OK;
  };
  const int rc = body();
  if (rc) (void)hipStreamSynchronize(st);
  for (void* p : {(void*)d_cnt, (void*)d_off, (void*)d_tmp, (void*)d_out, (void*)d_via}) pool_free(p);
  return rc;
}

int batch_fetch_into(const Batch* b, anx_result* out, size_t* off, size_t base, std::string& err) {
  return fetch_rows(b, out, off, nullptr, base, [](anx_result* d_out, uint32_t*) { return EmitResult{d_out}; }, err);
}

int batch_fetch_compact_into(const Batch* b, anx_topk_record* out, uint32_t* off, uint32_t* via, uint32_t base, bool plain, std::string& err) {
  if (via && !plain)
    return fetch_rows(b, out, off, via, base, [](anx_topk_record* d_out, uint32_t* d_via) { return EmitRecordVia{d_out, d_via}; }, err);
  const int rc = fetch_rows(b, out, off, nullptr, base, [](anx_topk_record* d_out, uint32_t*) { return EmitRecord{d_out}; }, err);
  if (rc == ANX_OK && via && b->n_results) memset(via, 0xFF, (size_t)b->n_results * sizeof(uint32_t));
  return rc;
}

int batch_fetch(const HostModel& m, const DeviceLexicon* dl, const Batch* b, anx_result** rows, size_t** offs,
                std::string& err) {
  (void)m;
  (void)dl;
  if (!b->ran) { err = "batch has not been run"; return ANX_EINVAL; }
  HIP_TRY(hipSetDevice(b->device));
  size_t* off = static_cast<size_t*>(malloc((b->n_input + 1) * sizeof(size_t)));
  anx_result* out = static_cast<anx_result*>(host_result_alloc(std::max<size_t>(1, b->n_results) * sizeof(anx_result)));
  if (!off || !out) { free(off); host_result_free(out); err = "out of memory"; return ANX_EINVAL; }
  const int rc = batch_fetch_into(b, out, off, 0, err);
  if (rc) { free(off); host_result_free(out); return rc; }
  *rows = out;
  *offs = off;
  return ANX_OK;
}

static int ensure_order(const Batch* cb, std::string& err) {
  Batch* b = const_cast<Batch*>(cb);
  if (b->order.size() == b->nq) return ANX_OK;
  b->order.resize(b->nq);
  if (b->nq) HIP_TRY(hipMemcpy(b->order.data(), b->q_orig, b->nq * sizeof(uint32_t), hipMemcpyDeviceToHost));
  return ANX_OK;
}

int batch_fetch_pairs(const HostModel& m, const DeviceLexicon* dl, const Batch* cb, anx_pair** out, size_t* n,
                      std::string& err) {
  if (!cb->ran) { err = "batch has not been run"; return ANX_EINVAL; }
  HIP_TRY(hipSetDevice(cb->device));
  if (!cb->ran_keep_all) {
// ... 16 lines not shown
    HIP_TRY(hipMemcpy(pm.data(), b->p_meta, R * 4, hipMemcpyDeviceToHost));
    HIP_TRY(hipMemcpy(ps.data(), b->p_score, R * 8, hipMemcpyDeviceToHost));
    HIP_TRY(hipMemcpy(ev.data(), dl->ent_vocab, (size_t)dl->nentries * 4, hipMemcpyDeviceToHost));
    for (size_t i = 0; i < R; ++i) {
      if ((i & (((size_t)1 << b->region_shift) - 1)) >= b->region_fill[i >> b->region_shift]) continue;
      if (pm[i] == META_SKIPPED || w >= b->n_pairs) continue;
      anx_pair& r = res[w++];
      r.query = b->order[pr[i].x];
      r.vocab_id = ev[pr[i].y & RAW_ENTRY_MASK];
      const uint32_t ld = pm[i] & 0x7F;
      r.ld = ld == PAIR_NONE ? (int16_t)-1 : (int16_t)ld;
      r.samecase = (pm[i] >> 7) & 1;
      r.lcs = (pm[i] >> 8) & 0xFF;
      r.prefixlen = (pm[i] >> 16) & 0xFF;
      r.suffixlen = (pm[i] >> 24) & 0xFF;
      r._pad = 0;
      r.score = ld == PAIR_NONE ? 0.0 : ps[i];
    }
  }
  *out = res;
  *n = w;
  return ANX_OK;
}

int batch_export_topk(const DeviceLexicon* dl, const Batch* b, void* dst, uint32_t stride, void* stream,
                      std::string& err) {
  (void)dl;
  if (!b->ran) { err = "batch has not been run"; return ANX_EINVAL; }
  if (!dst || stride == 0) { err = "bad export arguments"; return ANX_EINVAL; }
  if (stride < b->max_rows) {
    err = "export stride " + std::to_string(stride) + " is smaller than the longest result list (" + std::to_string(b->max_rows) + " rows): use a larger stride or anx_batch_export_compact";
    return ANX_ELIMIT;
  }
  HIP_TRY(hipSetDevice(b->device));
  b->async_stream = stream; b->async_pending = true;
  const uint64_t total = (uint64_t)b->nq * stride;
  if (total)
    hipLaunchKernelGGL(k_export_topk, dim3((uint32_t)((total + 255) / 256)), dim3(256), 0,
                       reinterpret_cast<hipStream_t>(stream), (uint32_t)b->nq, stride, b->soff, b->r_count,
                       b->r_rows, b->q_orig, static_cast<anx_topk_record*>(dst));
  HIP_TRY(hipGetLastError());
  return ANX_OK;
}

int batch_export_compact(const DeviceLexicon* dl, const Batch* b, void* dst, size_t capacity, void* stream,
                         size_t* used, std::string& err) {
  (void)dl;
  if (!b->ran) { err = "batch has not been run"; return ANX_EINVAL; }
  if (!dst || !used) { err = "bad export arguments"; return ANX_EINVAL; }
  const size_t n = b->n_input;
  const size_t off_bytes = ((n + 1) * sizeof(uint32_t) + 15) & ~(size_t)15;
  *used = off_bytes + (size_t)b->n_results * sizeof(anx_topk_record);
  if (capacity < *used) { err = "export buffer too small: " + std::to_string(*used) + " bytes needed"; return ANX_ELIMIT; }
  HIP_TRY(hipSetDevice(b->device));
  hipStream_t st = reinterpret_cast<hipStream_t>(stream);
  b->async_stream = stream; b->async_pending = true;
  uint32_t* d_off = static_cast<uint32_t*>(dst);
  anx_topk_record* d_rows = reinterpret_cast<anx_topk_record*>(static_cast<char*>(dst) + off_bytes);
  if (n == 0 || b->nq == 0) { HIP_TRY(hipMemsetAsync(d_off, 0, off_bytes, st)); return ANX_OK; }
  if (!b->x_cnt) {
    HIP_TRY(pool_malloc(reinterpret_cast<void**>(&b->x_cnt), n * sizeof(uint32_t)));
    HIP_TRY(pool_malloc(reinterpret_cast<void**>(&b->x_tmp), scan_tmp_bytes(n)));
  }
  if (const int rc = enqueue_rows(b, b->x_cnt, d_off, b->x_tmp, st, EmitRecord{d_rows}, err)) return rc;
  HIP_TRY(hipGetLastError());
  return ANX_OK;
}

size_t batch_compact_bytes(const Batch* b) {
  return (((b->n_input + 1) * sizeof(uint32_t) + 15) & ~(size_t)15) + (b->ran ? (size_t)b->n_results : 0) * sizeof(anx_topk_record);
}
int batch_gather_compact(const DeviceLexicon* dl, const Batch* b, int dst_device, void* dst, size_t capacity, void* stream, std::string& err) {
  if (!b->ran) { err = "batch has not been run"; return ANX_EINVAL; }
  const size_t need = batch_compact_bytes(b);
  if (capacity < need) { err = "gather buffer too small: " + std::to_string(need) + " bytes needed for this shard"; return ANX_ELIMIT; }
  size_t used = 0;
  if (b->device == dst_device) {
    const int rc = batch_export_compact(dl, b, dst, capacity, stream, &used, err);
    if (rc) return rc;
    HIP_TRY(hipStreamSynchronize(reinterpret_cast<hipStream_t>(stream)));
    return ANX_OK;
  }
  HIP_TRY(hipSetDevice(b->device));
  {
    int can = 0;
    if (hipDeviceCanAccessPeer(&can, b->device, dst_device) == hipSuccess && can) {
      const hipError_t e = hipDeviceEnablePeerAccess(dst_device, 0);
      if (e != hipSuccess && e != hipErrorPeerAccessAlreadyEnabled) (void)hipGetLastError();
      else (void)hipGetLastError();
    } else (void)hipGetLastError();
  }
  void* tmp = nullptr;
  HIP_TRY(pool_malloc(&tmp, std::max<size_t>(need, 16)));
  hipStream_t st = reinterpret_cast<hipStream_t>(stream);
  int rc = batch_export_compact(dl, b, tmp, need, stream, &used, err);
  if (rc == ANX_OK) {
    const hipError_t e = hipMemcpyPeerAsync(dst, dst_device, tmp, b->device, used, st);
    if (e != hipSuccess) { err = std::string("hipMemcpyPeerAsync: ") + hipGetErrorString(e); rc = ANX_ENODEVICE; }
  }
  (void)hipStreamSynchronize(st);
  pool_free(tmp);
  return rc;
}

int batch_pair_counts(const HostModel& m, const DeviceLexicon* dl, Batch* b, uint32_t** out, std::string& err) {
  if (!b->ran) { err = "batch has not been run"; return ANX_EINVAL; }
  HIP_TRY(hipSetDevice(b->device));
  const bool keep = b->keep_all_pairs;
  b->keep_all_pairs = false;
  b->count_pairs = true;
  const int rc = batch_run(m, dl, b, b->last_stream, err);
  b->count_pairs = false;
  b->keep_all_pairs = keep;
  if (rc) return rc;
  { const int rc2 = ensure_order(b, err); if (rc2) return rc2; }
  uint32_t* res = static_cast<uint32_t*>(calloc(std::max<size_t>(1, b->n_input), sizeof(uint32_t)));
  if (!res) { err = "out of memory"; return ANX_EINVAL; }
  if (b->nq) {
    std::vector<uint32_t> h(b->nq);
    if (hipMemcpy(h.data(), b->qpairs, b->nq * sizeof(uint32_t), hipMemcpyDeviceToHost) != hipSuccess) { free(res); err = "hipMemcpy failed"; return ANX_ENODEVICE; }
    for (size_t s = 0; s < b->nq; ++s) res[b->order[s]] = h[s];
  }
  *out = res;
  return ANX_OK;
}

void batch_set_run_mode(Batch* b, const anx_params& p, int conf_mode) {
  b->params = p;
  b->conf_mode = conf_mode;
}
bool batch_conf_fallback(const Batch* b) { return b->conf_fallback; }
int batch_download_text(const Batch* b, std::string& text, std::vector<uint32_t>& off, std::string& err) {
  if (b->n_input == 0) {
    text.clear();
    off.assign(1, 0u);
    return ANX_OK;
  }
  if (!b->d_text || !b->d_textoff) { err = "the batch does not hold its inputs"; return ANX_EINVAL; }
  HIP_TRY(hipSetDevice(b->device));
  off.assign(b->n_input + 1, 0u);
  HIP_TRY(hipMemcpy(off.data(), b->d_textoff, (b->n_input + 1) * sizeof(uint32_t), hipMemcpyDeviceToHost));
  text.assign(b->n_input ? (size_t)off[b->n_input] : 0, '\0');
  if (!text.empty()) HIP_TRY(hipMemcpy(&text[0], b->d_text, text.size(), hipMemcpyDeviceToHost));
  return ANX_OK;
}

void batch_stats(const Batch* b, anx_batch_stats* s) { *s = b->stats; }

void batch_free(Batch* b) {
  if (!b) return;
  (void)hipSetDevice(b->device);
  if (b->async_pending) (void)hipStreamSynchronize(reinterpret_cast<hipStream_t>(b->async_stream));
  if (b->launched) (void)hipEventSynchronize(b->ev_done);
  for (void* p : {(void*)b->q_cv, (void*)b->q_bits, (void*)b->q_rows, (void*)b->q_rec, (void*)b->q_meta, (void*)b->q_orig, (void*)b->d_tiles, (void*)b->rctr, (void*)b->sctr, (void*)b->surv,
                  (void*)b->counters, (void*)b->qexact, (void*)b->qsurv, (void*)b->soff, (void*)b->qcur,
                  (void*)b->qmaxfreq, (void*)b->d_cold, (void*)b->qpairs, (void*)b->x_cnt, (void*)b->x_tmp, (void*)b->scan_tmp, (void*)b->raw, (void*)b->p_score, (void*)b->p_meta, (void*)b->list8, (void*)b->listg, (void*)b->listw, (void*)b->lctr,
                  (void*)b->c_rows, (void*)b->sseg, (void*)b->qexpand, (void*)b->r_rows, (void*)b->t_key, (void*)b->r_count, (void*)b->r_off,
                  (void*)b->d_text, (void*)b->d_textoff, (void*)b->cf_weight, (void*)b->cf_need, (void*)b->cf_ctr, b->cf_work, (void*)b->cf_sort, b->cf_sort_tmp})
    if (p) pool_free(p);
  shell_release(b);
  delete b;
}

#include "small_path.hpp"

__global__ __launch_bounds__(64) void k_debug_band_bound(const uint4* __restrict__ q, const uint4* __restrict__ c, const uint8_t* __restrict__ lqs,
                                                         const uint8_t* __restrict__ lcs, uint32_t n, int d, int form, uint8_t* __restrict__ out) {
  const uint32_t i = blockIdx.x * 64u + threadIdx.x;
  const bool act = i < n;
  const uint4 Q = act ? q[i] : make_uint4(0xFEFEFEFEu, 0xFEFEFEFEu, 0xFEFEFEFEu, 0xFEFEFEFEu);
  const uint4 C = act ? c[i] : make_uint4(0xFFFFFFFFu, 0xFFFFFFFFu, 0xFFFFFFFFu, 0xFFFFFFFFu);
  const int lq = act ? lqs[i] : 1, lc = act ? lcs[i] : 1;
  const int ml = lq > lc ? lq : lc;
  bool rej;
  if (form == 2) {
    constexpr uint32_t M = 0xFFFFFFFFu;
    if (__any(act && ml > 12)) { const uint32_t q4[4] = {Q.x, Q.y, Q.z, Q.w}, c6[6] = {M, C.x, C.y, C.z, C.w, M}; rej = band_bound_rejects<4, false>(q4, c6, act, d, lq, lc); }
    else if (__any(act && ml > 8)) { const uint32_t q3[3] = {Q.x, Q.y, Q.z}, c5[5] = {M, C.x, C.y, C.z, M}; rej = band_bound_rejects<3, false>(q3, c5, act, d, lq, lc); }
    else { const uint32_t q2[2] = {Q.x, Q.y}, c4[4] = {M, C.x, C.y, M}; rej = band_bound_rejects<2, false>(q2, c4, act, d, lq, lc); }
  } else {
    constexpr uint32_t M = 0x7F7F7F7Fu;
    const uint32_t q4[4] = {Q.x & M, Q.y & M, Q.z & M, Q.w & M}, c6[6] = {M, C.x & M, C.y & M, C.z & M, C.w & M, M};
    const uint32_t q3[3] = {q4[0], q4[1], q4[2]}, c5[5] = {M, c6[1], c6[2], c6[3], M};
    const uint32_t q2[2] = {q4[0], q4[1]}, c4[4] = {M, c6[1], c6[2], M};
    if (form == 0) {
      if (__any(act && ml > 12)) rej = band_bound_rejects<4, true, true>(q4, c6, act, d, lq, lc);
      else if (__any(act && ml > 8)) rej = band_bound_rejects<3, true, true>(q3, c5, act, d, lq, lc);
      else rej = band_bound_rejects<2, true, true>(q2, c4, act, d, lq, lc);
    } else {
      if (__any(act && ml > 12)) rej = band_bound_rejects<4, true>(q4, c6, act, d, lq, lc);
      else if (__any(act && ml > 8)) rej = band_bound_rejects<3, true>(q3, c5, act, d, lq, lc);
      else rej = band_bound_rejects<2, true>(q2, c4, act, d, lq, lc);
    }
  }
  if (act) out[i] = rej ? 1 : 0;
}
int debug_band_bound(int device, const uint8_t* q_rows, const uint8_t* c_rows, const uint8_t* lq, const uint8_t* lc, size_t n, int d, int form,
                     uint8_t* out, std::string& err) {
  if (n == 0) return ANX_OK;
  if (n > (1u << 30) || d < 0 || d > 3 || form < 0 || form > 2) { err = "band bound: bad arguments"; return ANX_EINVAL; }
  HIP_TRY(hipSetDevice(device));
  uint4 *dq = nullptr, *dc = nullptr;
  uint8_t *dlq = nullptr, *dlc = nullptr, *dout = nullptr;
  int rc = ANX_OK;
  auto cleanup = [&]() { for (void* p : {(void*)dq, (void*)dc, (void*)dlq, (void*)dlc, (void*)dout}) if (p) (void)hipFree(p); };
  auto fail_hip = [&](hipError_t e) { err = std::string("HIP: ") + hipGetErrorString(e); cleanup(); return ANX_ENODEVICE; };
  hipError_t e;
  if ((e = hipMalloc(reinterpret_cast<void**>(&dq), n * 16)) != hipSuccess || (e = hipMalloc(reinterpret_cast<void**>(&dc), n * 16)) != hipSuccess ||
      (e = hipMalloc(reinterpret_cast<void**>(&dlq), n)) != hipSuccess || (e = hipMalloc(reinterpret_cast<void**>(&dlc), n)) != hipSuccess ||
      (e = hipMalloc(reinterpret_cast<void**>(&dout), n)) != hipSuccess)
    return fail_hip(e);
  if ((e = hipMemcpy(dq, q_rows, n * 16, hipMemcpyHostToDevice)) != hipSuccess || (e = hipMemcpy(dc, c_rows, n * 16, hipMemcpyHostToDevice)) != hipSuccess ||
      (e = hipMemcpy(dlq, lq, n, hipMemcpyHostToDevice)) != hipSuccess || (e = hipMemcpy(dlc, lc, n, hipMemcpyHostToDevice)) != hipSuccess)
    return fail_hip(e);
  hipLaunchKernelGGL(k_debug_band_bound, dim3((uint32_t)((n + 63) / 64)), dim3(64), 0, 0, dq, dc, dlq, dlc, (uint32_t)n, d, form, dout);
  if ((e = hipDeviceSynchronize()) != hipSuccess || (e = hipMemcpy(out, dout, n, hipMemcpyDeviceToHost)) != hipSuccess) return fail_hip(e);
  cleanup();
  return rc;
}

}
```

### analiticcl_amd/csrc/kernels_common.hpp

```cpp
#pragma once

struct Tile {
  uint32_t q0, nq;
  uint32_t s0, s1;
  uint32_t k;
  uint32_t lq;
  uint32_t sig_lo, sig_hi;
  uint32_t kind;
  uint32_t d;
  uint32_t kend;
  uint32_t ball0, balln;
  uint32_t adj;
  uint32_t flags;
};
constexpr uint32_t BALL_MAX = 4096;
constexpr uint32_t SIG_BYTE_MAX = 120;

constexpr int kSymbolPlanesMaxA = 61;
__host__ __device__ inline void symbol_planes16(const uint8_t* row, uint32_t len, uint32_t (&w)[3]) {
  uint32_t p[6] = {0u, 0u, 0u, 0u, 0u, 0u};
  for (uint32_t i = 0; i < 16u && i < len; ++i) {
    const uint32_t v = (uint32_t)row[i] + 1u;
    for (uint32_t b = 0; b < 6u; ++b) p[b] |= ((v >> b) & 1u) << i;
  }
  w[0] = p[0] | p[1] << 16; w[1] = p[2] | p[3] << 16; w[2] = p[4] | p[5] << 16;
}

constexpr int NBITPLANES = 4;
constexpr uint32_t SCAN_TQ = 64;
constexpr uint32_t SCAN_TQ_DEFAULT = 48;
constexpr uint32_t SCAN_HITS = 512;
constexpr uint32_t SCAN_MASKW = 2048;
constexpr uint32_t SCAN_PBUF = 128;
constexpr uint32_t SCAN_CHUNK = 256;
constexpr uint32_t SCAN_CHUNK_FUSED = 128;
constexpr uint32_t SCAN_REGIONS = 64;
constexpr uint32_t RC_STRIDE = 32;
constexpr uint32_t RAW_INVALID = 0xFFFFFFFFu;
constexpr uint32_t RAW_ENTRY_MASK = 0x3FFFFFFFu;
constexpr uint32_t RAW_PREFILTERED = 0x40000000u;
constexpr uint32_t META_SKIPPED = 0xFFFFFFFFu;

struct EntRec {
  uint32_t vocab, freq, order, meta;
};

struct DevAlphabet {
  int16_t* fast = nullptr;
  uint32_t* coff = nullptr;
  uint4* cand = nullptr;
  uint8_t* bytes = nullptr;
  uint8_t* sym_group = nullptr;
  uint2* lower = nullptr;
  uint32_t nlower = 0;
  uint32_t* siglen_begin = nullptr;
};

struct BatchShell {
  hipEvent_t ev[6] = {};
  hipEvent_t ev_scan0 = nullptr, ev_fs0 = nullptr, ev_fs1 = nullptr, ev_done = nullptr, ev_in = nullptr;
  uint32_t* h_read = nullptr;
};
struct RunHints {
  std::mutex mu;
  bool valid = false;
  anx_threshold kth = {}, dth = {};
  double score_threshold = 0.0;
  int stop = 0;
  uint32_t seg = 0;
  double nq = 0, maxfill = 0, surv_fill = 0, list_fill = 0, total_surv = 0;
};
struct DeviceLexicon {
  int device = 0;
  int nplanes = 0;
  int nsym = 0;
  uint32_t nclasses = 0, nentries = 0, cstride = 0, max_len = 0;
  uint32_t* cls_planes = nullptr;
  uint32_t* cls_bits = nullptr;
  uint8_t* cls_len = nullptr;
  uint32_t* cls_off = nullptr;
  uint4* scan_rec = nullptr;
  uint2* scan_rec34 = nullptr;
  uint4* sig_e = nullptr;
  uint4* sighash = nullptr;
  uint4* sighash_e = nullptr;
  uint32_t hash_mask = 0;
  unsigned long long* ball = nullptr;
  uint32_t* ball_tab = nullptr;
  uint32_t ball_off[13] = {}, ball_n[13] = {};
  uint4* adj_hash = nullptr;
  uint32_t adj_mask = 0;
  uint32_t* adj_hdr = nullptr;
  uint2* adj_planes = nullptr;
  uint32_t* adj_ids = nullptr;
  uint32_t adj_nhdr = 0;
  mutable std::vector<AdjSlot> adj_hash_host;
  mutable std::vector<AdjHdr> adj_hdr_host;
  uint4* sig = nullptr;
  uint32_t* sig_cbeg = nullptr;
  uint32_t* ent_vocab = nullptr;
  uint32_t* ent_freq = nullptr;
  uint32_t* ent_meta = nullptr;
  uint32_t* ent_rowoff = nullptr;
  uint32_t* ent_order = nullptr;
  EntRec* ent_rec = nullptr;
  uint4* e_rec = nullptr;
  uint4* e_planes = nullptr;
  uint32_t* ent_var_off = nullptr;
  uint32_t* var_target = nullptr;
  uint32_t* var_target_freq = nullptr;
  double* var_score = nullptr;
  int any_variants = 0;
  uint4* rows = nullptr;
  DevAlphabet alpha;
  size_t bytes = 0;
  double* quot = nullptr;
  mutable RunHints hints;
  mutable struct DeviceLm* dlm = nullptr;
  mutable struct DeviceConf* dconf = nullptr;
};

enum { CTR_SKIPPED = 2, CTR_MAXROWS = 3 , CTR_OVERFLOW = 4 , CTR_N = 8 };

struct SurvRow {
  double score;
  unsigned long long ord;
  uint32_t vocab, freq;
  uint32_t via, pad;
};
struct SurvRec {
  uint32_t q, e;
  double score;
};
struct SurvSeg {
  double score;
  uint32_t e, pad;
};
struct DevRow {
  uint32_t vocab_id, via;
  double dist_score, freq_score;
};

struct Batch {
  int device = 0;
  size_t nq = 0;
  anx_params params;
  std::vector<uint32_t> order;
  std::vector<int32_t> status;
  size_t n_input = 0;
  std::vector<Tile> tiles;
  uint32_t ntiles = 0;
  uint32_t n_sad_tiles = 0;
  uint32_t n_adj_tiles = 0;
  uint32_t qw = 1;
  uint32_t dmax = 0;
  uint64_t n_class_tests = 0;
  uint64_t n_tests_kind[NBITPLANES + 1] = {};
  uint32_t* q_cv = nullptr;
  uint32_t* q_bits = nullptr;
  uint4* q_rows = nullptr;
  uint4* q_rec = nullptr;
  uint32_t* q_meta = nullptr;
  uint32_t* q_orig = nullptr;
  Tile* d_tiles = nullptr;
  uint32_t* counters = nullptr;
  uint32_t* rctr = nullptr;
  uint32_t region_shift = 0;
  uint32_t region_fill[SCAN_REGIONS] = {};
  uint32_t* qexact = nullptr;
  uint32_t* qsurv = nullptr;
  uint32_t* soff = nullptr;
  uint32_t* qcur = nullptr;
  uint32_t* qmaxfreq = nullptr;
  void* d_cold = nullptr;
  uint32_t* qpairs = nullptr;
  bool count_pairs = false;
  int conf_mode = 0;
  bool keep_text = false;
  uint8_t* d_text = nullptr;
  uint32_t* d_textoff = nullptr;
  size_t text_bytes = 0;
  double* cf_weight = nullptr;
  uint32_t* cf_need = nullptr;
  uint32_t* cf_ctr = nullptr;
  void* cf_work = nullptr;
  uint32_t cf_work_blocks = 0;
  uint32_t* cf_sort = nullptr;
  void* cf_sort_tmp = nullptr;
  size_t cf_sort_tmp_bytes = 0;
  size_t cf_cap = 0;
  bool conf_fallback = false;
  bool conf_skipped = false;
  uint32_t* scan_tmp = nullptr;
  uint2* raw = nullptr;
  double* p_score = nullptr;
  uint32_t* p_meta = nullptr;
  uint32_t* list8 = nullptr;
  uint32_t* listg = nullptr;
  uint32_t* listw = nullptr;
  uint32_t* lctr = nullptr;
  size_t list_cap = 0;
  size_t raw_cap = 0;
  SurvRec* surv = nullptr;
  uint32_t* sctr = nullptr;
  size_t surv_region_cap = 0;
  SurvRow* c_rows = nullptr;
  SurvSeg* sseg = nullptr;
  size_t sseg_cap = 0;
  uint32_t* qexpand = nullptr;
  DevRow* r_rows = nullptr;
  double* t_key = nullptr;
  size_t surv_cap = 0;
  uint32_t* r_count = nullptr;
  uint32_t* r_off = nullptr;
  uint32_t n_raw = 0;
  uint64_t n_sel = 0;
  uint64_t n_pairs = 0, n_surv = 0, n_results = 0;
  mutable uint32_t *x_cnt = nullptr, *x_tmp = nullptr;
  uint32_t max_rows = 0;
  void* last_stream = nullptr;
  mutable void* async_stream = nullptr;
  mutable bool async_pending = false;
  bool ran = false;
  bool keep_all_pairs = false;
  bool ran_keep_all = false;
  hipEvent_t ev[6] = {};
  hipEvent_t ev_scan0 = nullptr;
  hipEvent_t ev_fs0 = nullptr, ev_fs1 = nullptr;
  hipEvent_t ev_done = nullptr;
  hipEvent_t ev_in = nullptr;
  uint32_t* h_read = nullptr;
  bool launched = false;
  uint32_t fill_cap_launched = 0;
  uint32_t prev_maxfill = 0, prev_surv_fill = 0, prev_list_fill = 0;
  bool hinted = false;
  size_t hint_rows = 0;
  int runs_finished = 0;
  anx_batch_stats stats = {};
};

#ifdef ANX_DEBUG_SWITCHES
#define ANX_DBG(x) (x)
#else
#define ANX_DBG(x) 0
#endif

typedef const __attribute__((address_space(4))) uint32_t* cptr_u32;
```

### analiticcl_amd/csrc/kernels_prefix.hpp

```cpp
#pragma once

constexpr int SCAN_ITEMS = 8, SCAN_THREADS = 256, SCAN_TILE = SCAN_ITEMS * SCAN_THREADS;

__device__ inline uint32_t block_exclusive_scan(uint32_t v, uint32_t* total) {
  __shared__ uint32_t wsum[SCAN_THREADS / 64];
  const int lane = threadIdx.x & 63, wid = threadIdx.x >> 6;
  uint32_t inc = v;
#pragma unroll
  for (int o = 1; o < 64; o <<= 1) {
    const uint32_t u = __shfl_up(inc, o);
    if (lane >= o) inc += u;
  }
  if (lane == 63) wsum[wid] = inc;
  __syncthreads();
  uint32_t base = 0, tot = 0;
  for (int i = 0; i < SCAN_THREADS / 64; ++i) {
    if (i < wid) base += wsum[i];
    tot += wsum[i];
  }
  __syncthreads();
  *total = tot;
  return base + inc - v;
}
__global__ __launch_bounds__(SCAN_THREADS) void k_scan_local(const uint32_t* __restrict__ in, uint32_t n,
                                                             uint32_t* __restrict__ out,
                                                             uint32_t* __restrict__ blocksum, uint32_t* __restrict__ maxout) {
  const uint32_t i0 = blockIdx.x * SCAN_TILE + threadIdx.x * SCAN_ITEMS;
  uint32_t v[SCAN_ITEMS], s = 0;
#pragma unroll
  for (int i = 0; i < SCAN_ITEMS; ++i) {
    v[i] = i0 + i < n ? in[i0 + i] : 0;
    s += v[i];
  }
  uint32_t tot;
  uint32_t ex = block_exclusive_scan(s, &tot);
#pragma unroll
  for (int i = 0; i < SCAN_ITEMS; ++i) {
    if (i0 + i < n) out[i0 + i] = ex;
    ex += v[i];
  }
  if (threadIdx.x == 0) blocksum[blockIdx.x] = tot;
  if (maxout) {
    uint32_t mx = 0;
#pragma unroll
    for (int i = 0; i < SCAN_ITEMS; ++i) mx = max(mx, v[i]);
#pragma unroll
    for (int o = 32; o; o >>= 1) mx = max(mx, (uint32_t)__shfl_xor((int)mx, o));
    if ((threadIdx.x & 63) == 0 && mx) atomicMax(maxout, mx);
  }
}
__global__ __launch_bounds__(SCAN_THREADS) void k_scan_sums(uint32_t* __restrict__ blocksum, uint32_t nb) {
  uint32_t carry = 0;
  for (uint32_t b0 = 0; b0 < nb; b0 += SCAN_THREADS) {
    const uint32_t i = b0 + threadIdx.x;
    const uint32_t v = i < nb ? blocksum[i] : 0;
    uint32_t tot;
    const uint32_t ex = block_exclusive_scan(v, &tot);
    if (i < nb) blocksum[i] = carry + ex;
    carry += tot;
  }
  if (threadIdx.x == 0) blocksum[nb] = carry;
}
__global__ __launch_bounds__(SCAN_THREADS) void k_scan_add(uint32_t* __restrict__ out, uint32_t n,
                                                           const uint32_t* __restrict__ blocksum, uint32_t nb, uint32_t* __restrict__ copy) {
  const uint32_t i0 = blockIdx.x * SCAN_TILE + threadIdx.x * SCAN_ITEMS;
  const uint32_t add = blocksum[blockIdx.x];
#pragma unroll
  for (int i = 0; i < SCAN_ITEMS; ++i)
    if (i0 + i < n) {
      const uint32_t v = out[i0 + i] + add;
      out[i0 + i] = v;
      if (copy) copy[i0 + i] = v;
    }
  if (blockIdx.x == 0 && threadIdx.x == 0) out[n] = blocksum[nb];
}
```

### analiticcl_amd/csrc/kernels_rank.hpp

```cpp
#pragma once

struct CompactArgs {
  int have_freq, any_variants;
};
__global__ __launch_bounds__(256) void k_compact(const SurvRec* __restrict__ surv, const uint32_t* __restrict__ sctr,
                                                 uint32_t region_cap, CompactArgs a,
                                                 uint32_t* __restrict__ qcur, const EntRec* __restrict__ ent_rec,
                                                 const uint32_t* __restrict__ ent_var_off,
                                                 const uint32_t* __restrict__ var_target,
                                                 const uint32_t* __restrict__ var_target_freq,
                                                 const double* __restrict__ var_score, SurvRow* __restrict__ c_rows) {
  const uint32_t region = blockIdx.x % SCAN_REGIONS, i = (blockIdx.x / SCAN_REGIONS) * 256 + threadIdx.x;
  const bool live = i < sctr[region * RC_STRIDE];
  if (!live) return;
  const SurvRec sr = surv[(size_t)region * region_cap + i];
  const double s = sr.score;
  const uint32_t e = sr.e, q = sr.q;
  const EntRec er = ent_rec[e];
  const uint32_t f = a.have_freq ? er.freq : 1u;
  const unsigned long long ord = (unsigned long long)er.order << 20;
  uint32_t v0 = 0, v1 = 0, self = 1;
  if (a.any_variants) {
    v0 = ent_var_off[e];
    v1 = ent_var_off[e + 1];
    self = (er.meta & 0x400u) ? 0u : 1u;
  }
  const uint32_t nrows = (v1 - v0) + self;
  uint32_t pos = atomicAdd(&qcur[q], nrows);
  for (uint32_t j = v0; j < v1; ++j, ++pos) {
    const uint32_t tf = var_target_freq[j];
    c_rows[pos] = SurvRow{s * var_score[j], ord | (unsigned long long)(j - v0), var_target[j],
                          a.have_freq ? (tf < f ? tf : f) : (tf < 1u ? tf : 1u), er.vocab, 0u};
  }
  if (self) c_rows[pos] = SurvRow{s, ord | (unsigned long long)(v1 - v0), er.vocab, f, 0xFFFFFFFFu, 0u};
}

constexpr uint32_t COMPACT_B = 1024, COMPACT_H = 2048;
constexpr uint32_t COMPACT_P = 16;
__global__ __launch_bounds__(COMPACT_B) void k_compact_grouped(const SurvRec* __restrict__ surv, const uint32_t* __restrict__ sctr,
                                                               uint32_t region_cap, int have_freq, uint32_t* __restrict__ qcur,
                                                               const EntRec* __restrict__ ent_rec, SurvRow* __restrict__ c_rows,
                                                               const uint32_t* __restrict__ total_rows, uint32_t row_cap, uint32_t* __restrict__ overflow) {
  __shared__ uint32_t h_key[COMPACT_H], h_cnt[COMPACT_H], h_base[COMPACT_H];
  if (*total_rows > row_cap) return;
  const uint32_t region = blockIdx.x % SCAN_REGIONS;
  uint32_t fill = sctr[region * RC_STRIDE];
  if (fill > region_cap) {
    fill = region_cap;
    if (threadIdx.x == 0) *overflow = 1u;
  }
  for (uint32_t i0 = (blockIdx.x / SCAN_REGIONS) * COMPACT_B; i0 < fill; i0 += (gridDim.x / SCAN_REGIONS) * COMPACT_B) {
    for (uint32_t h = threadIdx.x; h < COMPACT_H; h += COMPACT_B) { h_key[h] = 0xFFFFFFFFu; h_cnt[h] = 0; }
    __syncthreads();
    const uint32_t i = i0 + threadIdx.x;
    const bool live = i < fill;
    SurvRec sr{0u, 0u, 0.0};
    uint32_t slot = 0, rank = 0;
    bool owner = false;
    if (live) sr = surv[(size_t)region * region_cap + i];
    EntRec er{};
    if (live) er = ent_rec[sr.e];
    {
      const uint32_t lane = threadIdx.x & 63u;
      const uint32_t qprev = (uint32_t)__shfl_up((int)sr.q, 1);
      const bool head = live && (lane == 0u || qprev != sr.q);
      const unsigned long long hm = __ballot(head), lm = __ballot(live);
      const unsigned long long below = hm & ((2ull << lane) - 1ull);
      const uint32_t start = live ? 63u - (uint32_t)__clzll((long long)below) : 0u;
      const unsigned long long above = hm & ~((2ull << lane) - 1ull);
      const uint32_t nlive = (uint32_t)__popcll(lm);
      const uint32_t end = above ? (uint32_t)__ffsll((long long)above) - 1u : nlive;
      uint32_t base_rank = 0;
      if (head) {
        slot = (sr.q * 2654435761u) >> 21;
        for (;;) {
          const uint32_t prev = atomicCAS(&h_key[slot], 0xFFFFFFFFu, sr.q);
          if (prev == 0xFFFFFFFFu) { owner = true; break; }
          if (prev == sr.q) break;
          slot = (slot + 1u) & (COMPACT_H - 1u);
        }
        base_rank = atomicAdd(&h_cnt[slot], end - lane);
      }
      slot = (uint32_t)__shfl((int)slot, (int)start);
      rank = (uint32_t)__shfl((int)base_rank, (int)start) + (lane - start);
    }
    __syncthreads();
    if (owner) h_base[slot] = atomicAdd(&qcur[sr.q], h_cnt[slot]);
    __syncthreads();
    if (live) {
      c_rows[h_base[slot] + rank] = SurvRow{sr.score, (unsigned long long)er.order << 20, er.vocab, have_freq ? er.freq : 1u, 0xFFFFFFFFu, 0u};
    }
    __syncthreads();
  }
}

constexpr uint32_t EXPAND_B = 256, EXPAND_P = 4;
__global__ __launch_bounds__(EXPAND_B) void k_compact_expand(const SurvRec* __restrict__ surv, const uint32_t* __restrict__ sctr,
                                                             uint32_t region_cap, int have_freq, uint32_t* __restrict__ qcur,
                                                             const EntRec* __restrict__ ent_rec, const uint32_t* __restrict__ ent_var_off,
                                                             const uint32_t* __restrict__ var_target,
                                                             const uint32_t* __restrict__ var_target_freq,
                                                             const double* __restrict__ var_score, SurvRow* __restrict__ c_rows,
                                                             const uint32_t* __restrict__ total_rows, uint32_t row_cap,
                                                             uint32_t* __restrict__ overflow) {
  if (*total_rows > row_cap) return;
  const uint32_t region = blockIdx.x % SCAN_REGIONS;
  const uint32_t fill = sctr[region * RC_STRIDE];
  if (fill > region_cap) {
    if (threadIdx.x == 0) *overflow = 1u;
    return;
  }
  for (uint32_t i = (blockIdx.x / SCAN_REGIONS) * EXPAND_B + threadIdx.x; i < fill; i += (gridDim.x / SCAN_REGIONS) * EXPAND_B) {
    const SurvRec sr = surv[(size_t)region * region_cap + i];
    const uint32_t e = sr.e;
    const EntRec er = ent_rec[e];
    const uint32_t v0 = ent_var_off[e], v1 = ent_var_off[e + 1];
    const uint32_t self = (er.meta & 0x400u) ? 0u : 1u;
    const uint32_t nrows = (v1 - v0) + self;
    const uint32_t f = have_freq ? er.freq : 1u;
    const unsigned long long ord = (unsigned long long)er.order << 20;
    uint32_t pos = atomicAdd(&qcur[sr.q], nrows);
    if (pos > row_cap || nrows > row_cap - pos) { *overflow = 1u; continue; }
    for (uint32_t j = v0; j < v1; ++j, ++pos) {
      const uint32_t tf = var_target_freq[j];
      c_rows[pos] = SurvRow{sr.score * var_score[j], ord | (unsigned long long)(j - v0), var_target[j],
                            have_freq ? (tf < f ? tf : f) : (tf < 1u ? tf : 1u), er.vocab, 0u};
    }
    if (self) c_rows[pos] = SurvRow{sr.score, ord | (unsigned long long)(v1 - v0), er.vocab, f, 0xFFFFFFFFu, 0u};
  }
}

struct RankArgs {
  double cutoff_threshold;
  uint64_t max_matches;
  float freq_weight;
  int have_freq, any_variants;
};
constexpr int RANK_LCAP = 128;

struct SegRows {
  const SurvSeg* seg;
  uint32_t cap;
  const EntRec* ent_rec;
};
__device__ __forceinline__ SurvRow row_of(const SurvRow* __restrict__ c_rows, const SegRows& sr, int have_freq, uint32_t q, uint32_t seg0, uint32_t i) {
  if (i < sr.cap) {
    const uint4 g = *reinterpret_cast<const uint4*>(sr.seg + (size_t)q * sr.cap + i);
    const EntRec er = sr.ent_rec[g.z];
    return SurvRow{__longlong_as_double((long long)((unsigned long long)g.x | (unsigned long long)g.y << 32)), (unsigned long long)er.order << 20,
                   er.vocab, have_freq ? er.freq : 1u, 0xFFFFFFFFu, 0u};
  }
  return c_rows[seg0 + i - sr.cap];
}
__device__ __forceinline__ unsigned long long rank_key1(double score) {
  const unsigned long long b = (unsigned long long)__double_as_longlong(score + 0.0);
  return (b >> 63) ? ~b : b | (1ull << 63);
}
__device__ __forceinline__ unsigned long long rank_key2(uint32_t freq, unsigned long long ord) {
  return (unsigned long long)freq << 32 | (uint32_t)~(uint32_t)(ord >> 20);
}

__device__ inline double result_score(double dist, double freq, float fw) {
  if (fw == 0.0f) return dist;
  return (dist + ((double)fw * freq)) / (1.0 + (double)fw);
}

template <int G, int LCAP>
__device__ inline void rank_query_all(uint32_t q, bool valid, int gl, int gshift, double* __restrict__ s_key,
                                  unsigned long long* __restrict__ s_ord, uint32_t* __restrict__ s_freq,
                                  double* __restrict__ s_sdist, double* __restrict__ s_sfreq, uint32_t seg0, uint32_t n,
                                  uint32_t maxf, uint32_t qex, const SurvRow* __restrict__ c_rows, const SegRows& sr, const RankArgs& a,
                                  double* __restrict__ t_key, DevRow* __restrict__ r_rows, uint32_t* __restrict__ r_count) {
  const unsigned long long gmask = G >= 64 ? ~0ull : ((1ull << (G & 63)) - 1ull);
  if (!valid) n = 0;
  if (valid && n == 0 && gl == 0) r_count[q] = 0;
  const double max_freq = a.have_freq ? (double)maxf : (maxf ? 1.0 : 0.0);
  const bool sort_weighted = a.freq_weight > 0.0f;
  const bool score_weighted = a.freq_weight != 0.0f;
  const bool expanded = n && a.any_variants && qex != 0;
  SurvRow mine{0.0, 0ull, 0u, 0u, 0u, 0u};
  for (uint32_t i = gl; i < n; i += G) {
    const SurvRow r = row_of(c_rows, sr, a.have_freq, q, seg0, i);
    if (i == (uint32_t)gl) mine = r;
    double key = r.score;
    if (sort_weighted) {
      const double fs = max_freq > 0.0 ? (double)r.freq / max_freq : (double)r.freq;
      key = result_score(key, fs, a.freq_weight);
    }
    if (i < (uint32_t)LCAP) { s_key[i] = key; s_freq[i] = r.freq; s_ord[i] = r.ord; }
    else t_key[seg0 + i] = key;
  }
  __builtin_amdgcn_fence(__ATOMIC_SEQ_CST, "workgroup");
  const bool full = score_weighted || a.max_matches == 0 || expanded;
  const uint32_t M = full ? n : (uint32_t)min((uint64_t)n, a.max_matches + 1);
  for (uint32_t i = gl; i < n; i += G) {
    double ki; uint32_t fi; unsigned long long oi;
    if (i < (uint32_t)LCAP) { ki = s_key[i]; fi = s_freq[i]; oi = s_ord[i]; }
    else { ki = t_key[seg0 + i]; const SurvRow r = row_of(c_rows, sr, a.have_freq, q, seg0, i); fi = r.freq; oi = r.ord; }
    uint32_t rank = 0;
    for (uint32_t j = 0; j < n; ++j) {
      double kj; uint32_t fj; unsigned long long oj;
      if (j < (uint32_t)LCAP) { kj = s_key[j]; fj = s_freq[j]; oj = s_ord[j]; }
      else { kj = t_key[seg0 + j]; const SurvRow r = row_of(c_rows, sr, a.have_freq, q, seg0, j); fj = r.freq; oj = r.ord; }
      bool before;
      if (sort_weighted) before = kj > ki || (kj == ki && oj < oi);
      else before = kj > ki || (kj == ki && (fj > fi || (fj == fi && oj < oi)));
      rank += before;
    }
    if (rank < M) {
      const SurvRow r = i == (uint32_t)gl ? mine : row_of(c_rows, sr, a.have_freq, q, seg0, i);
      const double ff = max_freq > 0.0 ? (double)fi / max_freq : (double)fi;
      r_rows[seg0 + rank] = DevRow{r.vocab, a.any_variants ? r.via : 0xFFFFFFFFu, r.score, ff};
      if (rank < (uint32_t)G) { s_sdist[rank] = r.score; s_sfreq[rank] = ff; }
    }
  }
  __builtin_amdgcn_fence(__ATOMIC_SEQ_CST, "workgroup");
  const bool parallel_tail = n && !expanded && M <= (uint32_t)G;
  {
    const float fw = a.freq_weight;
    const bool have = parallel_tail && (uint32_t)gl < M;
    const double di = have ? s_sdist[gl] : 0.0;
    const double si = have ? result_score(di, s_sfreq[gl], fw) : 0.0;
    uint32_t len = n;
    const uint64_t mm = a.max_matches;
    const bool crop = parallel_tail && mm > 0 && (uint64_t)n > mm;
    double last = 0.0, cropped = 0.0;
    if (crop) {
      last = result_score(s_sdist[mm - 1], s_sfreq[mm - 1], fw);
      cropped = result_score(s_sdist[mm], s_sfreq[mm], fw);
    }
    const unsigned long long lt = (__ballot(have && crop && di < cropped) >> gshift) & gmask;
    const uint32_t stop_at = lt ? (uint32_t)__ffsll((long long)lt) - 1 : (uint32_t)G;
    const unsigned long long eq = (__ballot(have && crop && gl >= 1 && (uint32_t)gl <= stop_at && di == cropped) >> gshift) & gmask;
    if (crop) {
      if (cropped < last) len = (uint32_t)mm;
      else {
        const uint32_t early = eq ? (uint32_t)__ffsll((long long)eq) - 1 : 0;
        const uint32_t late = lt ? stop_at : 0;
        if (early > 0) len = early + 1;
        else if (late > 0) len = late + 1;
      }
    }
    const bool docut = parallel_tail && a.cutoff_threshold >= 1.0;
    const double best = docut ? result_score(s_sdist[0], s_sfreq[0], fw) : 0.0;
    const unsigned long long cut = (__ballot(have && docut && gl >= 1 && (uint32_t)gl < len && si <= best / a.cutoff_threshold) >> gshift) & gmask;
    if (cut) len = (uint32_t)__ffsll((long long)cut) - 1;
    if (parallel_tail && gl == 0) r_count[q] = len;
  }
  if (n && !parallel_tail && gl == 0) {
    const float fw = a.freq_weight;
    DevRow* rr = r_rows + seg0;
    uint32_t len = n, avail = M;
    if (expanded) {
      uint32_t w = 0;
      for (uint32_t i = 0; i < n; ++i)
        if (w == 0 || rr[w - 1].vocab_id != rr[i].vocab_id) {
          rr[w] = rr[i];
          ++w;
        }
      len = w;
      avail = w;
    }
    const uint64_t mm = a.max_matches;
    if (mm > 0 && (uint64_t)len > mm) {
      const double last = result_score(rr[mm - 1].dist_score, rr[mm - 1].freq_score, fw);
      const double cropped = result_score(rr[mm].dist_score, rr[mm].freq_score, fw);
      if (cropped < last) len = (uint32_t)mm;
      else {
        uint32_t early = 0, late = 0;
        for (uint32_t i = 0; i < avail; ++i) {
          if (rr[i].dist_score == cropped && early == 0) early = i;
          if (rr[i].dist_score < cropped) { late = i; break; }
        }
        if (early > 0) len = early + 1;
        else if (late > 0) len = late + 1;
      }
    }
    uint32_t cutoff = 0;
    if (a.cutoff_threshold >= 1.0) {
      bool have = false;
      double best = 0.0;
      for (uint32_t i = 0; i < len; ++i) {
        const double sc = result_score(rr[i].dist_score, rr[i].freq_score, fw);
        if (have) {
          if (sc <= best / a.cutoff_threshold) { cutoff = i; break; }
        } else { best = sc; have = true; }
      }
    }
    if (cutoff > 0) len = cutoff;
    r_count[q] = len;
  }
}

template <int G, int LCAP>
__device__ inline void rank_query(uint32_t q, bool valid, int gl, int gshift, uint32_t nloop, double* __restrict__ s_key,
                                  unsigned long long* __restrict__ s_ord, uint32_t* __restrict__ s_freq,
                                  uint16_t* __restrict__ s_src, double* __restrict__ s_sdist, double* __restrict__ s_sfreq,
                                  uint32_t seg0, uint32_t n, uint32_t maxf, uint32_t qex,
                                  const SurvRow* __restrict__ c_rows, const SegRows& sr, const RankArgs& a, double* __restrict__ t_key,
                                  DevRow* __restrict__ r_rows, uint32_t* __restrict__ r_count) {
  const unsigned long long gmask = G >= 64 ? ~0ull : ((1ull << (G & 63)) - 1ull);
  if (!valid) n = 0;
  const double max_freq = a.have_freq ? (double)maxf : (maxf ? 1.0 : 0.0);
  const bool sort_weighted = a.freq_weight > 0.0f;
  const bool score_weighted = a.freq_weight != 0.0f;
  const bool expanded = n && a.any_variants && qex != 0;
  const bool prune = a.cutoff_threshold >= 1.0 && !expanded && !score_weighted && n <= 0xFFFFu;
  const bool packed = !sort_weighted && !a.any_variants;
  unsigned long long* const s_key64 = reinterpret_cast<unsigned long long*>(s_key);
  auto key_of = [&](const SurvRow& r) {
    if (!sort_weighted) return r.score;
    const double fs = max_freq > 0.0 ? (double)r.freq / max_freq : (double)r.freq;
    return result_score(r.score, fs, a.freq_weight);
  };
  SurvRow mine{0.0, 0ull, 0u, 0u, 0u, 0u};
  double best = -1.0;
  for (uint32_t i = gl; i < n; i += G) {
    const SurvRow r = row_of(c_rows, sr, a.have_freq, q, seg0, i);
    if (i == (uint32_t)gl) mine = r;
    best = fmax(best, key_of(r));
  }
#pragma unroll
  for (int o = G / 2; o; o >>= 1) best = fmax(best, __shfl_xor(best, o));
  const double thr = best / a.cutoff_threshold;
  double tau = -1.0;
  if (G == 64 && n > 32 && !(score_weighted || a.max_matches == 0 || expanded)) {
    const uint32_t want = (uint32_t)a.max_matches + 1u;
    double lo = -1.0, hi = __builtin_inf();
    for (int round = 0; round < 96; ++round) {
      double pivot = 0.0;
      bool found = false;
      for (uint32_t base = 0; base < n && !found; base += G) {
        const uint32_t i = base + (uint32_t)gl;
        SurvRow r = mine;
        if (base && i < n) r = row_of(c_rows, sr, a.have_freq, q, seg0, i);
        const double key = key_of(r);
        const bool inr = i < n && !(prune && key <= thr && key < best) && key > lo && key < hi;
        const unsigned long long m = __ballot(inr);
        if (m) {
          const int src = (round & 1) ? 63 - __clzll((long long)m) : __ffsll((long long)m) - 1;
          pivot = __shfl(key, src);
          found = true;
        }
      }
      if (!found) break;
      uint32_t cgt = 0, cge = 0;
      for (uint32_t base = 0; base < n; base += G) {
        const uint32_t i = base + (uint32_t)gl;
        SurvRow r = mine;
        if (base && i < n) r = row_of(c_rows, sr, a.have_freq, q, seg0, i);
        const double key = key_of(r);
        const bool pa = i < n && !(prune && key <= thr && key < best);
        cgt += (uint32_t)__popcll(__ballot(pa && key > pivot));
        cge += (uint32_t)__popcll(__ballot(pa && key >= pivot));
      }
      if (cgt < want && want <= cge) { tau = pivot; break; }
      if (cgt >= want) lo = pivot;
      else hi = pivot;
    }
  }
  uint32_t kept = 0;
  for (uint32_t base = 0; base < nloop; base += G) {
    const uint32_t i = base + (uint32_t)gl;
    SurvRow r = mine;
    if (base && i < n) r = row_of(c_rows, sr, a.have_freq, q, seg0, i);
    const double key = key_of(r);
    const bool keep = i < n && !(prune && key <= thr && key < best) && key >= tau;
    const unsigned long long m = (__ballot(keep) >> gshift) & gmask;
    const uint32_t pos = kept + (uint32_t)__popcll(m & ((1ull << gl) - 1ull));
    if (keep && pos < (uint32_t)LCAP) {
      if (packed) { s_key64[pos] = rank_key1(key); s_ord[pos] = rank_key2(r.freq, r.ord); }
      else { s_key[pos] = key; s_ord[pos] = r.ord; }
      s_freq[pos] = r.freq; s_src[pos] = (uint16_t)i;
    }
    kept += (uint32_t)__popcll(m);
  }
  if (kept > (uint32_t)LCAP) {
    rank_query_all<G, LCAP>(q, valid, gl, gshift, s_key, s_ord, s_freq, s_sdist, s_sfreq, seg0, n, maxf, qex, c_rows, sr, a, t_key,
                            r_rows, r_count);
    return;
  }
  const bool one_row_per_lane = nloop <= (uint32_t)G;
  n = kept;
  if (valid && n == 0 && gl == 0) r_count[q] = 0;
  __builtin_amdgcn_fence(__ATOMIC_SEQ_CST, "workgroup");
  const bool full = score_weighted || a.max_matches == 0 || expanded;
  const uint32_t M = full ? n : (uint32_t)min((uint64_t)n, a.max_matches + 1);
  for (uint32_t base = 0; base < nloop; base += G) {
    const uint32_t i = base + (uint32_t)gl;
    const bool have = i < n;
    const uint32_t fi = have ? s_freq[i] : 0u;
    const unsigned long long oi = have ? s_ord[i] : 0ull;
    uint32_t rank = have ? 0u : 0xFFFFFFFFu;
    if (have) {
    if (packed) {
      const unsigned long long ki = s_key64[i];
#pragma unroll 2
      for (uint32_t j = 0; j < n; ++j) {
        const unsigned long long kj = s_key64[j], oj = s_ord[j];
        rank += (uint32_t)((kj > ki) | ((kj == ki) & (oj > oi)));
      }
    } else if (sort_weighted) {
      const double ki = s_key[i];
      for (uint32_t j = 0; j < n; ++j) {
        const double kj = s_key[j];
        const unsigned long long oj = s_ord[j];
        rank += (uint32_t)((kj > ki) | ((kj == ki) & (oj < oi)));
      }
    } else {
      const double ki = s_key[i];
      for (uint32_t j = 0; j < n; ++j) {
        const double kj = s_key[j];
        const uint32_t fj = s_freq[j];
        const unsigned long long oj = s_ord[j];
        rank += (uint32_t)((kj > ki) | ((kj == ki) & ((fj > fi) | ((fj == fi) & (oj < oi)))));
      }
    }
    }
    uint32_t r_vocab = 0, r_via = 0;
    double r_score = 0.0;
    if (one_row_per_lane) {
      const int from = gshift + (have ? (int)s_src[i] : gl);
      const unsigned long long sbits = (unsigned long long)__double_as_longlong(mine.score);
      r_vocab = (uint32_t)__shfl((int)mine.vocab, from);
      r_via = (uint32_t)__shfl((int)mine.via, from);
      const uint32_t s_lo = (uint32_t)__shfl((int)(uint32_t)sbits, from), s_hi = (uint32_t)__shfl((int)(uint32_t)(sbits >> 32), from);
      r_score = __longlong_as_double((long long)((unsigned long long)s_lo | (unsigned long long)s_hi << 32));
    } else if (have && rank < M) {
      const SurvRow r = row_of(c_rows, sr, a.have_freq, q, seg0, s_src[i]);
      r_vocab = r.vocab; r_via = r.via; r_score = r.score;
    }
    if (have && rank < M) {
      const double ff = (a.have_freq && max_freq > 0.0) ? (double)fi / max_freq : (double)fi;
      r_rows[seg0 + rank] = DevRow{r_vocab, a.any_variants ? r_via : 0xFFFFFFFFu, r_score, ff};
      if (rank < (uint32_t)G) { s_sdist[rank] = r_score; s_sfreq[rank] = ff; }
    }
  }
  __builtin_amdgcn_fence(__ATOMIC_SEQ_CST, "workgroup");
  const bool parallel_tail = n && !expanded && M <= (uint32_t)G;
  {
    const float fw = a.freq_weight;
    const bool have = parallel_tail && (uint32_t)gl < M;
    const double di = have ? s_sdist[gl] : 0.0;
    const double si = have ? result_score(di, s_sfreq[gl], fw) : 0.0;
    uint32_t len = n;
    const uint64_t mm = a.max_matches;
    const bool crop = parallel_tail && mm > 0 && (uint64_t)n > mm;
    double last = 0.0, cropped = 0.0;
    if (crop) {
      last = result_score(s_sdist[mm - 1], s_sfreq[mm - 1], fw);
      cropped = result_score(s_sdist[mm], s_sfreq[mm], fw);
    }
    const unsigned long long lt = (__ballot(have && crop && di < cropped) >> gshift) & gmask;
    const uint32_t stop_at = lt ? (uint32_t)__ffsll((long long)lt) - 1 : (uint32_t)G;
    const unsigned long long eq = (__ballot(have && crop && gl >= 1 && (uint32_t)gl <= stop_at && di == cropped) >> gshift) & gmask;
    if (crop) {
      if (cropped < last) len = (uint32_t)mm;
      else {
        const uint32_t early = eq ? (uint32_t)__ffsll((long long)eq) - 1 : 0;
        const uint32_t late = lt ? stop_at : 0;
        if (early > 0) len = early + 1;
        else if (late > 0) len = late + 1;
      }
    }
    const bool docut = parallel_tail && a.cutoff_threshold >= 1.0;
    double cutthr = thr;
    if (docut && !prune) cutthr = result_score(s_sdist[0], s_sfreq[0], fw) / a.cutoff_threshold;
    const unsigned long long cut = (__ballot(have && docut && gl >= 1 && (uint32_t)gl < len && si <= cutthr) >> gshift) & gmask;
    if (cut) len = (uint32_t)__ffsll((long long)cut) - 1;
    if (parallel_tail && gl == 0) r_count[q] = len;
  }
  if (n && !parallel_tail && gl == 0) {
    const float fw = a.freq_weight;
    DevRow* rr = r_rows + seg0;
    uint32_t len = n, avail = M;
    if (expanded) {
      uint32_t w = 0;
      for (uint32_t i = 0; i < n; ++i)
        if (w == 0 || rr[w - 1].vocab_id != rr[i].vocab_id) {
          rr[w] = rr[i];
          ++w;
        }
      len = w;
      avail = w;
    }
    const uint64_t mm = a.max_matches;
    if (mm > 0 && (uint64_t)len > mm) {
      const double last = result_score(rr[mm - 1].dist_score, rr[mm - 1].freq_score, fw);
      const double cropped = result_score(rr[mm].dist_score, rr[mm].freq_score, fw);
      if (cropped < last) len = (uint32_t)mm;
      else {
        uint32_t early = 0, late = 0;
        for (uint32_t i = 0; i < avail; ++i) {
          if (rr[i].dist_score == cropped && early == 0) early = i;
          if (rr[i].dist_score < cropped) { late = i; break; }
        }
        if (early > 0) len = early + 1;
        else if (late > 0) len = late + 1;
      }
    }
    uint32_t cutoff = 0;
    if (a.cutoff_threshold >= 1.0) {
      bool have = false;
      double best = 0.0;
      for (uint32_t i = 0; i < len; ++i) {
        const double sc = result_score(rr[i].dist_score, rr[i].freq_score, fw);
        if (have) {
          if (sc <= best / a.cutoff_threshold) { cutoff = i; break; }
        } else { best = sc; have = true; }
      }
    }
    if (cutoff > 0) len = cutoff;
    r_count[q] = len;
  }
}

constexpr int RANK_QPW = 4;
constexpr int RANK_WAVE_BYTES = RANK_LCAP * 22 + 64 * 16;
template <bool SIMPLE>
__global__ __launch_bounds__(256) void k_rank(uint32_t nq, const uint32_t* __restrict__ soff,
                                              const SurvRow* __restrict__ c_rows,
                                              const uint32_t* __restrict__ qmaxfreq,
                                              const uint32_t* __restrict__ qexpand, RankArgs aa,
                                              double* __restrict__ t_key, DevRow* __restrict__ r_rows,
                                              uint32_t* __restrict__ r_count, uint32_t row_cap, const uint32_t* __restrict__ overflow,
                                              SegRows sr) {
  RankArgs a = aa;
  if (SIMPLE) { a.any_variants = 0; a.freq_weight = 0.0f; }
  __shared__ __attribute__((aligned(16))) uint8_t s_raw[4 * RANK_WAVE_BYTES];
  if (soff[nq] > row_cap || *overflow) return;
  const int lane = threadIdx.x & 63, wid = threadIdx.x >> 6;
  uint8_t* wl = s_raw + wid * RANK_WAVE_BYTES;
  const uint32_t qbase = (blockIdx.x * 4 + wid) * RANK_QPW;
  uint32_t my_seg0 = 0, my_n = 0, my_maxf = 0, my_qex = 0;
  if (lane < RANK_QPW && qbase + lane < nq) {
    my_seg0 = soff[qbase + lane];
    my_n = soff[qbase + lane + 1] - my_seg0;
    my_maxf = qmaxfreq[qbase + lane];
    if (a.any_variants) my_qex = qexpand[qbase + lane];
  }
  uint32_t nmax = my_n;
  nmax = max(nmax, (uint32_t)__shfl_xor((int)nmax, 1));
  nmax = max(nmax, (uint32_t)__shfl_xor((int)nmax, 2));
  nmax = (uint32_t)__builtin_amdgcn_readfirstlane((int)nmax);
  {
    const int grp = lane >> 4, gl = lane & 15;
    uint8_t* gb = wl + grp * 608;
    const uint32_t ng = (uint32_t)__shfl((int)my_n, grp);
    rank_query<16, 16>(qbase + grp, qbase + grp < nq && ng <= 16u, gl, grp * 16, 16u, reinterpret_cast<double*>(gb),
                       reinterpret_cast<unsigned long long*>(gb + 128), reinterpret_cast<uint32_t*>(gb + 256),
                       reinterpret_cast<uint16_t*>(gb + 320), reinterpret_cast<double*>(gb + 352), reinterpret_cast<double*>(gb + 480),
                       (uint32_t)__shfl((int)my_seg0, grp), ng, (uint32_t)__shfl((int)my_maxf, grp),
                       (uint32_t)__shfl((int)my_qex, grp), c_rows, sr, a, t_key, r_rows, r_count);
  }
  if (nmax > 16) {
    __builtin_amdgcn_fence(__ATOMIC_SEQ_CST, "workgroup");
    uint32_t mask32 = 0;
    for (int k = 0; k < RANK_QPW; ++k) {
      const uint32_t nk = (uint32_t)__builtin_amdgcn_readlane((int)my_n, k);
      if (qbase + k < nq && nk > 16u && nk <= 32u) mask32 |= 1u << k;
    }
    while (mask32) {
      const int k0 = __ffs((int)mask32) - 1;
      mask32 &= mask32 - 1u;
      const int k1 = mask32 ? __ffs((int)mask32) - 1 : -1;
      if (k1 >= 0) mask32 &= mask32 - 1u;
      const int half = lane >> 5, gl = lane & 31, kk = half ? k1 : k0;
      const bool valid = kk >= 0;
      const int src = valid ? kk : 0;
      uint8_t* gb = wl + half * 1216;
      rank_query<32, 32>(qbase + (uint32_t)src, valid, gl, half * 32, 32u, reinterpret_cast<double*>(gb),
                         reinterpret_cast<unsigned long long*>(gb + 256), reinterpret_cast<uint32_t*>(gb + 512),
                         reinterpret_cast<uint16_t*>(gb + 640), reinterpret_cast<double*>(gb + 704), reinterpret_cast<double*>(gb + 960),
                         (uint32_t)__shfl((int)my_seg0, src), (uint32_t)__shfl((int)my_n, src), (uint32_t)__shfl((int)my_maxf, src),
                         (uint32_t)__shfl((int)my_qex, src), c_rows, sr, a, t_key, r_rows, r_count);
      __builtin_amdgcn_fence(__ATOMIC_SEQ_CST, "workgroup");
    }
    for (int k = 0; k < RANK_QPW; ++k) {
      if (qbase + k >= nq) break;
      const uint32_t nk = (uint32_t)__builtin_amdgcn_readlane((int)my_n, k);
      if (nk <= 32u) continue;
      rank_query<64, RANK_LCAP>(qbase + k, true, lane, 0, nk, reinterpret_cast<double*>(wl),
                                reinterpret_cast<unsigned long long*>(wl + RANK_LCAP * 8),
                                reinterpret_cast<uint32_t*>(wl + RANK_LCAP * 16), reinterpret_cast<uint16_t*>(wl + RANK_LCAP * 20),
                                reinterpret_cast<double*>(wl + RANK_LCAP * 22), reinterpret_cast<double*>(wl + RANK_LCAP * 22 + 512),
                                (uint32_t)__shfl((int)my_seg0, k), nk, (uint32_t)__shfl((int)my_maxf, k), (uint32_t)__shfl((int)my_qex, k),
                                c_rows, sr, a, t_key, r_rows, r_count);
      __builtin_amdgcn_fence(__ATOMIC_SEQ_CST, "workgroup");
    }
  }
}

__global__ __launch_bounds__(256) void k_pack_rows(uint32_t nq, const uint32_t* __restrict__ soff,
                                                   const uint32_t* __restrict__ r_off,
                                                   const uint32_t* __restrict__ r_count,
                                                   const DevRow* __restrict__ r_rows, DevRow* __restrict__ out) {
  const uint32_t q = blockIdx.x * 256 + threadIdx.x;
  if (q >= nq) return;
  const uint32_t n = r_count[q], src = soff[q], dst = r_off[q];
  for (uint32_t i = 0; i < n; ++i) out[dst + i] = r_rows[src + i];
}
__global__ __launch_bounds__(256) void k_fetch_counts(uint32_t nq, const uint32_t* __restrict__ r_count,
                                                      const uint32_t* __restrict__ q_orig, uint32_t* __restrict__ cnt_orig) {
  const uint32_t s = blockIdx.x * 256 + threadIdx.x;
  if (s < nq) cnt_orig[q_orig[s]] = r_count[s];
}
__device__ inline anx_topk_record topk_record_of(const DevRow& d) {
  anx_topk_record r;
  r.vocab_id = d.vocab_id;
  r.freq_score = (float)d.freq_score;
  r.dist_score = d.dist_score;
  return r;
}
struct EmitResult {
  anx_result* out;
  __device__ void operator()(uint32_t at, const DevRow& d) const {
    anx_result r;
    r.vocab_id = d.vocab_id;
    r.dist_score = d.dist_score;
    r.freq_score = d.freq_score;
    r.via = d.via == 0xFFFFFFFFu ? ANX_NO_VIA : (uint64_t)d.via;
    out[at] = r;
  }
};
struct EmitRecord {
  anx_topk_record* out;
  __device__ void operator()(uint32_t at, const DevRow& d) const { out[at] = topk_record_of(d); }
};
struct EmitRecordVia {
  anx_topk_record* out;
  uint32_t* via;
  __device__ void operator()(uint32_t at, const DevRow& d) const {
    out[at] = topk_record_of(d);
    via[at] = d.via;
  }
};
template <typename Emit>
__global__ __launch_bounds__(256) void k_emit_rows(uint32_t nq, const uint32_t* __restrict__ soff, const uint32_t* __restrict__ r_count,
                                                   const DevRow* __restrict__ r_rows, const uint32_t* __restrict__ q_orig,
                                                   const uint32_t* __restrict__ off_orig, Emit emit) {
  const uint32_t s = blockIdx.x * 256 + threadIdx.x;
  if (s >= nq) return;
  const uint32_t n = r_count[s], src = soff[s], dst = off_orig[q_orig[s]];
  for (uint32_t i = 0; i < n; ++i) emit(dst + i, r_rows[src + i]);
}
__global__ __launch_bounds__(256) void k_export_topk(uint32_t nq, uint32_t stride, const uint32_t* __restrict__ soff,
                                                     const uint32_t* __restrict__ r_count,
                                                     const DevRow* __restrict__ r_rows,
                                                     const uint32_t* __restrict__ q_orig,
                                                     anx_topk_record* __restrict__ out) {
  const uint64_t t = (uint64_t)blockIdx.x * 256 + threadIdx.x;
  if (t >= (uint64_t)nq * stride) return;
  const uint32_t q = (uint32_t)(t / stride), i = (uint32_t)(t % stride);
  anx_topk_record r;
  r.vocab_id = 0xFFFFFFFFu;
  r.freq_score = 0.0f;
  r.dist_score = 0.0;
  if (i < r_count[q]) r = topk_record_of(r_rows[soff[q] + i]);
  out[(size_t)q_orig[q] * stride + i] = r;
}

constexpr uint32_t SMALL_MAX = 4096;
constexpr uint32_t SMALL_T = 1024;
__device__ inline uint32_t small_block_exscan(uint32_t v, uint32_t* s_w, uint32_t* total) {
  const uint32_t lane = threadIdx.x & 63u, wid = threadIdx.x >> 6;
  uint32_t inc = v;
#pragma unroll
  for (int o = 1; o < 64; o <<= 1) {
    const uint32_t u = (uint32_t)__shfl_up((int)inc, o);
    if ((int)lane >= o) inc += u;
  }
  if (lane == 63u) s_w[wid] = inc;
  __syncthreads();
  uint32_t base = 0, tot = 0;
  for (uint32_t i = 0; i < SMALL_T / 64u; ++i) {
    if (i < wid) base += s_w[i];
    tot += s_w[i];
  }
  __syncthreads();
  *total = tot;
  return base + inc - v;
}
__global__ __launch_bounds__(SMALL_T) void k_small_offsets(const uint32_t* __restrict__ qsurv, uint32_t n, uint32_t* __restrict__ soff, uint32_t* __restrict__ qcur) {
  __shared__ uint32_t s_w[SMALL_T / 64];
  uint32_t v[4], s = 0;
#pragma unroll
  for (uint32_t i = 0; i < 4u; ++i) {
    const uint32_t q = threadIdx.x * 4u + i;
    v[i] = q < n ? qsurv[q] : 0u;
    s += v[i];
  }
  uint32_t tot;
  uint32_t ex = small_block_exscan(s, s_w, &tot);
#pragma unroll
  for (uint32_t i = 0; i < 4u; ++i) {
    const uint32_t q = threadIdx.x * 4u + i;
    if (q < n) { soff[q] = ex; qcur[q] = ex; }
    ex += v[i];
  }
  if (threadIdx.x == 0) soff[n] = tot;
}
struct SmallCtl { uint32_t rows, maxfill, surv_fill, list_fill, total_surv, overflow, pad0, pad1; };
__global__ __launch_bounds__(SMALL_T) void k_small_fetch(uint32_t n, const uint32_t* __restrict__ soff, const uint32_t* __restrict__ r_count, const DevRow* __restrict__ r_rows,
                                                         const uint32_t* __restrict__ rctr, const uint32_t* __restrict__ sctr, const uint32_t* __restrict__ lctr,
                                                         const uint32_t* __restrict__ counters, unsigned long long* __restrict__ off, anx_result* __restrict__ out, uint32_t row_cap,
                                                         uint32_t crow_cap, SmallCtl* __restrict__ ctl) {
  __shared__ uint32_t s_w[SMALL_T / 64];
  __shared__ uint32_t s_max[3];
  if (threadIdx.x < 3u) s_max[threadIdx.x] = 0u;
  const bool ranked = soff[n] <= crow_cap && counters[CTR_OVERFLOW] == 0u;
  uint32_t v[4], s = 0;
#pragma unroll
  for (uint32_t i = 0; i < 4u; ++i) {
    const uint32_t q = threadIdx.x * 4u + i;
    v[i] = (ranked && q < n) ? r_count[q] : 0u;
    s += v[i];
  }
  __shared__ uint32_t s_off[SMALL_MAX + 1];
  uint32_t tot;
  uint32_t ex = small_block_exscan(s, s_w, &tot);
  const bool fits = tot <= row_cap;
#pragma unroll
  for (uint32_t i = 0; i < 4u; ++i) {
    const uint32_t q = threadIdx.x * 4u + i;
    if (q < n) { if (blockIdx.x == 0) off[q] = ex; s_off[q] = ex; }
    ex += v[i];
  }
  if (threadIdx.x == 0) s_off[n] = tot;
  __syncthreads();
  if (fits)
    for (uint32_t r = blockIdx.x * SMALL_T + threadIdx.x; r < tot; r += gridDim.x * SMALL_T) {
      uint32_t lo = 0, hi = n;
      while (hi - lo > 1u) {
        const uint32_t mid = (lo + hi) >> 1;
        if (s_off[mid] <= r) lo = mid; else hi = mid;
      }
      const DevRow d = r_rows[soff[lo] + (r - s_off[lo])];
      anx_result o;
      o.vocab_id = d.vocab_id;
      o.dist_score = d.dist_score;
      o.freq_score = d.freq_score;
      o.via = d.via == 0xFFFFFFFFu ? ANX_NO_VIA : (uint64_t)d.via;
      out[r] = o;
    }
  if (blockIdx.x != 0) return;
  if (threadIdx.x < SCAN_REGIONS) {
    atomicMax(&s_max[0], rctr[threadIdx.x * RC_STRIDE + RC_RAW]);
    atomicMax(&s_max[1], sctr[threadIdx.x * RC_STRIDE]);
    atomicMax(&s_max[2], max(max(lctr[threadIdx.x * RC_STRIDE], lctr[(SCAN_REGIONS + threadIdx.x) * RC_STRIDE]), lctr[(2u * SCAN_REGIONS + threadIdx.x) * RC_STRIDE]));
  }
  __syncthreads();
  if (threadIdx.x == 0) {
    off[n] = tot;
    SmallCtl c;
// ... 7 lines not shown
```

### analiticcl_amd/csrc/launch_plan.hpp

```cpp
#pragma once

static inline ScanArgs scan_args_of(const DeviceLexicon* dl) {
  ScanArgs A{};
  A.cls_bits = dl->cls_bits; A.cls_planes = dl->cls_planes; A.scan_rec = dl->scan_rec; A.scan_rec34 = dl->scan_rec34; A.pad_rec = dl->nentries; A.cstride = dl->cstride; A.pad_class = dl->nclasses;
  A.cls_len = dl->cls_len; A.cls_off = dl->cls_off; A.sig = dl->sig; A.sig_e = dl->sig_e; A.sig_cbeg = dl->sig_cbeg; A.sighash = dl->sighash; A.sighash_e = dl->sighash_e; A.hash_mask = dl->hash_mask; A.ball = dl->ball;
  A.adj_hdr = dl->adj_hdr; A.adj_planes = dl->adj_planes; A.adj_ids = dl->adj_ids;
  A.e_rec = dl->e_rec;
  return A;
}
template <typename F>
static inline void with_nplanes(int nplanes, F&& f) {
  switch (nplanes) {
    case 8: f(std::integral_constant<int, 8>{}); break;
    case 16: f(std::integral_constant<int, 16>{}); break;
    case 24: f(std::integral_constant<int, 24>{}); break;
    case 32: f(std::integral_constant<int, 32>{}); break;
    default: f(std::integral_constant<int, 42>{}); break;
  }
}

struct ScorePlan {
  ScoreArgs sa;
  uint32_t threads;
  int fastD;
  bool have_long_q;
  int enable_filter;
  bool split_wide;
  bool b7;
  bool planes;
  bool fits() const { return threads != 0; }
  size_t lds_bytes() const { return (size_t)threads * sa.stride; }
};
static inline ScorePlan score_plan_of(const HostModel& m, const DeviceLexicon* dl, double score_threshold, uint32_t qw, uint32_t d) {
  const Switches& sw = switches();
  ScorePlan pl{};
  ScoreArgs& sa = pl.sa;
  sa.quot = dl->quot;
  sa.w_ld = m.weights.ld; sa.w_lcs = m.weights.lcs; sa.w_prefix = m.weights.prefix; sa.w_suffix = m.weights.suffix; sa.w_case = m.weights.casew;
  sa.w_sum = m.weights.ld + m.weights.lcs + m.weights.prefix + m.weights.suffix + m.weights.casew;
  sa.score_threshold = score_threshold;
  sa.have_freq = m.have_freq ? 1 : 0;
  sa.any_variants = dl->any_variants;
  sa.lqp = qw * 16;
  sa.lcp = (dl->max_len + 15) / 16 * 16;
  uint32_t stride = sa.lqp + sa.lcp + (d + 2) * (2 * d + 3);
  stride = (stride + 3) / 4;
  if ((stride & 1) == 0) stride++;
  sa.stride = stride * 4;
  sa.qw = qw;
  pl.threads = 256;
  while (pl.threads > 64 && (size_t)pl.threads * sa.stride > 64 * 1024) pl.threads >>= 1;
  if ((size_t)pl.threads * sa.stride > 64 * 1024) pl.threads = 0;
  pl.have_long_q = qw > 1;
  pl.enable_filter = sw.prefilter;
  pl.fastD = (sw.score_fast && d >= 1 && d <= 3) ? (int)d : 0;
  pl.split_wide = sw.fs_split != 0;
  pl.b7 = sw.fs_b7 && m.alphabet.size() + 1 < 0x7E;
  pl.planes = pl.b7 && sw.fs_planes && (int)m.alphabet.size() <= kSymbolPlanesMaxA;
  return pl;
}
struct SlotLists { SlotList l8, lg, lw; };
static inline SlotLists slot_lists_of(uint32_t* list8, uint32_t* listg, uint32_t* listw, uint32_t* lctr, uint32_t cap) {
  return SlotLists{{list8, lctr, cap}, {listg, lctr + SCAN_REGIONS * RC_STRIDE, cap}, {listw, lctr + 2 * SCAN_REGIONS * RC_STRIDE, cap}};
}
static inline PairArgs pair_args_of(const DeviceLexicon* dl, const uint2* raw, const uint32_t* q_meta, const uint4* q_rows, const uint4* q_rec, double* p_score, uint32_t* p_meta,
                                    uint32_t* qmaxfreq, uint32_t* qsurv, uint32_t* qexpand) {
  return PairArgs{raw, q_meta, q_rows, q_rec, dl->e_rec, dl->ent_meta, dl->ent_rowoff, dl->rows, dl->ent_freq, dl->ent_var_off, p_score, p_meta, qmaxfreq, qsurv, qexpand, dl->e_planes};
}

template <int D, bool WIDE, int MODE>
static inline void launch_filter_score_as(dim3 grid, hipStream_t st, const FilterArgs& fa, const PairArgs& pa, const FsCold* cold) {
  hipLaunchKernelGGL((k_filter_score<D, WIDE, MODE>), grid, dim3(256), 0, st, fa, pa, cold);
}
template <bool WIDE, int MODE>
static inline void launch_filter_score_d(int fastD, dim3 grid, hipStream_t st, const FilterArgs& fa, const PairArgs& pa, const FsCold* cold) {
  switch (fastD) {
    case 1: launch_filter_score_as<1, WIDE, MODE>(grid, st, fa, pa, cold); break;
    case 2: launch_filter_score_as<2, WIDE, MODE>(grid, st, fa, pa, cold); break;
    case 3: launch_filter_score_as<3, WIDE, MODE>(grid, st, fa, pa, cold); break;
    default: launch_filter_score_as<0, WIDE, MODE>(grid, st, fa, pa, cold); break;
  }
}
static inline void launch_filter_score(const ScorePlan& pl, dim3 grid, hipStream_t st, const FilterArgs& fa, const PairArgs& pa, const FsCold* cold) {
  if (pl.split_wide) {
    if (pl.planes) launch_filter_score_d<false, 2>(pl.fastD, grid, st, fa, pa, cold);
    else if (pl.b7) launch_filter_score_d<false, 1>(pl.fastD, grid, st, fa, pa, cold);
    else launch_filter_score_d<false, 0>(pl.fastD, grid, st, fa, pa, cold);
  } else {
    if (pl.b7) launch_filter_score_d<true, 1>(pl.fastD, grid, st, fa, pa, cold);
    else launch_filter_score_d<true, 0>(pl.fastD, grid, st, fa, pa, cold);
  }
}
static inline void launch_score_fast8(int fastD, dim3 grid, hipStream_t st, const SlotList& l8, const PairArgs& pa, const ScoreArgs& sa, const SurvOut& so) {
  if (fastD == 1) hipLaunchKernelGGL(k_score_fast8<1>, grid, dim3(256), 0, st, l8, pa, sa, so);
  else if (fastD == 2) hipLaunchKernelGGL(k_score_fast8<2>, grid, dim3(256), 0, st, l8, pa, sa, so);
  else hipLaunchKernelGGL(k_score_fast8<3>, grid, dim3(256), 0, st, l8, pa, sa, so);
}
static inline void launch_small_lists(const ScorePlan& pl, hipStream_t st, const SmallListArgs& L, const FilterArgs& fa, const PairArgs& pa, const SurvOut& so) {
  const dim3 grid(SCAN_REGIONS);
  const size_t dyn = pl.lds_bytes();
  if (pl.fastD == 1) hipLaunchKernelGGL(k_small_lists<1>, grid, dim3(256), dyn, st, L, fa, pa, pl.sa, so);
  else if (pl.fastD == 2) hipLaunchKernelGGL(k_small_lists<2>, grid, dim3(256), dyn, st, L, fa, pa, pl.sa, so);
  else if (pl.fastD == 3) hipLaunchKernelGGL(k_small_lists<3>, grid, dim3(256), dyn, st, L, fa, pa, pl.sa, so);
  else hipLaunchKernelGGL(k_small_lists<0>, grid, dim3(256), dyn, st, L, fa, pa, pl.sa, so);
}

static inline RankArgs rank_args_of(const HostModel& m, const DeviceLexicon* dl, const anx_params& p, double cutoff) {
  RankArgs ra{};
  ra.cutoff_threshold = cutoff;
  ra.max_matches = p.max_matches;
  ra.freq_weight = p.freq_weight;
  ra.have_freq = m.have_freq ? 1 : 0;
  ra.any_variants = dl->any_variants;
  return ra;
}
static inline void launch_rank(const RankArgs& ra, hipStream_t st, uint32_t nq, const uint32_t* soff, const SurvRow* c_rows, const uint32_t* qmaxfreq, const uint32_t* qexpand, double* t_key,
                               DevRow* r_rows, uint32_t* r_count, uint32_t row_cap, const uint32_t* overflow, const SegRows& seg) {
  const dim3 grid((nq + 4 * RANK_QPW - 1) / (4 * RANK_QPW));
  if (!ra.any_variants && ra.freq_weight == 0.0f) hipLaunchKernelGGL(k_rank<true>, grid, dim3(256), 0, st, nq, soff, c_rows, qmaxfreq, qexpand, ra, t_key, r_rows, r_count, row_cap, overflow, seg);
  else hipLaunchKernelGGL(k_rank<false>, grid, dim3(256), 0, st, nq, soff, c_rows, qmaxfreq, qexpand, ra, t_key, r_rows, r_count, row_cap, overflow, seg);
}
```

### analiticcl_amd/csrc/small_path.hpp

```cpp
#pragma once

constexpr uint32_t SMALL_MAX_BYTES = 64;
constexpr uint32_t SMALL_SHIFT = 15;
constexpr uint32_t SMALL_SURV_CAP = 16384;
constexpr uint32_t SMALL_LIST_BLOCKS = 2;
constexpr uint32_t SMALL_FS_BLK = 512;
constexpr uint32_t SMALL_FETCH_BLOCKS = 8;
constexpr uint32_t SMALL_ROWS_PER_Q = 16;

struct SmallCtx {
  int device = 0;
  hipStream_t st = nullptr;
  char* h_in = nullptr;
  char* h_out = nullptr;
  SmallEnc enc;
  uint32_t *counters = nullptr, *rctr = nullptr, *sctr = nullptr, *lctr = nullptr, *qsurv = nullptr, *soff = nullptr, *qcur = nullptr, *qmaxfreq = nullptr, *qexpand = nullptr,
           *r_count = nullptr;
  uint2* raw = nullptr;
  SurvRec* surv = nullptr;
  uint32_t *list8 = nullptr, *listg = nullptr, *listw = nullptr;
  SurvRow* c_rows = nullptr;
  DevRow* r_rows = nullptr;
  double* t_key = nullptr;
  FsCold* d_cold = nullptr;
// ... 38 lines not shown
  SmallEnc& e = c->enc;
  dev(&e.codes, SMALL_IN_BLOB + 4 * N + 16); dev(&e.meta, N); dev(&e.bits, N * NBITPLANES); dev(&e.kind, N); dev(&e.cv, N * NP); dev(&e.blk, 3 * (N / 256 + 1));
  dev(&e.perm, N); dev(&e.key, N); dev(&e.sig, N);
  dev(&e.q_rec, 2 * N); dev(&e.q_rows, N * QW); dev(&e.q_bits, N * NBITPLANES); dev(&e.q_cv, N * NP); dev(&e.q_meta, N); dev(&e.q_orig, N); dev(&e.qexact, N);
  dev(&e.s_kind, N); dev(&e.s_sig, N); dev(&e.tiles, 8 * N);
  dev(&c->counters, CTR_N); dev(&c->rctr, SCAN_REGIONS * RC_STRIDE); dev(&c->sctr, SCAN_REGIONS * RC_STRIDE); dev(&c->lctr, 3 * SCAN_REGIONS * RC_STRIDE);
  dev(&c->qsurv, N); dev(&c->soff, N + 1); dev(&c->qcur, N); dev(&c->qmaxfreq, N); dev(&c->qexpand, N); dev(&c->r_count, N);
  dev(&c->raw, (size_t)SCAN_REGIONS << SMALL_SHIFT);
  dev(&c->surv, (size_t)SCAN_REGIONS * SMALL_SURV_CAP);
  dev(&c->list8, (size_t)SCAN_REGIONS * SMALL_SURV_CAP); dev(&c->listg, (size_t)SCAN_REGIONS * SMALL_SURV_CAP); dev(&c->listw, (size_t)SCAN_REGIONS * SMALL_SURV_CAP);
  c->row_cap = N * SMALL_ROWS_PER_Q + 1024;
  dev(&c->c_rows, c->row_cap); dev(&c->r_rows, c->row_cap); dev(&c->t_key, c->row_cap);
  dev(&c->d_cold, 1);
  if (!ok) { (void)hipGetLastError(); err = "small path: device buffers"; return nullptr; }
  if (small_iota(e.perm, SMALL_MAX, c->st) != ANX_OK || hipStreamSynchronize(c->st) != hipSuccess) { err = "small path: set-up kernel"; return nullptr; }
  return c.release();
}
static SmallCtx* small_ctx_acquire(const DeviceLexicon* dl, std::string& err) {
  DevPool& pl = pool_of(dl->device);
  {
    std::lock_guard<std::mutex> g(pl.mu);
    if (!pl.small_idle.empty()) { SmallCtx* c = pl.small_idle.back(); pl.small_idle.pop_back(); return c; }
  }
  return small_ctx_create(dl, err);
}
static void small_ctx_release(SmallCtx* c) {
  DevPool& pl = pool_of(c->device);
  std::lock_guard<std::mutex> g(pl.mu);
  pl.small_idle.push_back(c);
}
static void small_ctxs_destroy(int device) {
  DevPool& pl = pool_of(device);
  std::vector<SmallCtx*> drop;
  { std::lock_guard<std::mutex> g(pl.mu); drop.swap(pl.small_idle); }
  for (SmallCtx* c : drop) small_ctx_destroy(c);
}

static std::atomic<uint64_t> g_small_taken{0}, g_small_overflow{0};
void small_stats(uint64_t* out) { out[0] = g_small_taken.load(); out[1] = g_small_overflow.load(); }

int small_find(const HostModel& m, const DeviceLexicon* dl, const char* const* utf8, size_t n, const anx_params& p, anx_result** out_rows, size_t** out_offs,
               std::string& err) {
  if (!dl || n == 0 || n > SMALL_MAX || !switches().small_path || p.stop_at_exact_match || dl->nplanes > 42) return 1;
  uint32_t lens[SMALL_MAX];
  uint32_t maxbytes = 0;
  for (size_t i = 0; i < n; ++i) {
    const size_t l = utf8[i] ? strlen(utf8[i]) : 0;
    if (l > SMALL_MAX_BYTES) return 1;
    lens[i] = (uint32_t)l;
    maxbytes = std::max(maxbytes, (uint32_t)l);
  }
  if (hipSetDevice(dl->device) != hipSuccess) { err = "hipSetDevice failed"; return ANX_ENODEVICE; }
  SmallCtx* c = small_ctx_acquire(dl, err);
  if (!c) { (void)hipGetLastError(); return 1; }
  struct Release { SmallCtx* c; ~Release() { small_ctx_release(c); } } rel{c};
  hipStream_t st = c->st;
  uint32_t* h_off = reinterpret_cast<uint32_t*>(c->h_in + SMALL_IN_BLOB);
  {
    size_t pos = 0;
    for (size_t i = 0; i < n; ++i) {
      h_off[i] = (uint32_t)pos;
      if (lens[i]) memcpy(c->h_in + pos, utf8[i], lens[i]);
      c->h_in[pos + lens[i]] = '\0';
      pos += (size_t)lens[i] + 1;
    }
    h_off[n] = (uint32_t)pos;
    memset(c->h_in + pos, 0, 16);
  }
  const uint32_t n32 = (uint32_t)n;
  const uint32_t qw = std::max<uint32_t>(1u, (maxbytes + 15u) / 16u);
  const uint32_t d = (uint32_t)clamp_threshold(p.max_edit_distance, (int)maxbytes, kMaxEditDistance);
  const size_t row_cap = std::min<size_t>(c->row_cap, n * (size_t)SMALL_ROWS_PER_Q + 64);
  anx_result* rows = static_cast<anx_result*>(host_result_alloc(row_cap * sizeof(anx_result)));
  if (!rows) return 1;
  struct RowsGuard {
    anx_result* rows; hipStream_t st; bool drain;
    ~RowsGuard() { if (!rows) return; if (drain) (void)hipStreamSynchronize(st); host_result_free(rows); }
  } guard{rows, st, false};
  if (!host_result_is_pinned(rows)) return 1;
  SmallCtl* h_ctl = reinterpret_cast<SmallCtl*>(c->h_out);
  unsigned long long* h_off64 = reinterpret_cast<unsigned long long*>(c->h_out + 64);
  h_ctl->rows = 0xFFFFFFFEu;
  SmallZero z{};
  {
    uint32_t* zp[8] = {c->counters, c->rctr, c->sctr, c->lctr, c->qsurv, c->qmaxfreq, c->qexpand, nullptr};
    const uint32_t zn[8] = {CTR_N, SCAN_REGIONS * RC_STRIDE, SCAN_REGIONS * RC_STRIDE, 3 * SCAN_REGIONS * RC_STRIDE, n32, n32, n32, 0u};
    for (int i = 0; i < 8; ++i) { z.p[i] = zp[i]; z.n[i] = zn[i]; }
  }
  const uint8_t* in_blob = reinterpret_cast<const uint8_t*>(c->h_in);
  const uint32_t* in_off = h_off;
  const uint32_t slots = n32 <= 128u ? 32u : n32 <= 512u ? 16u : 8u;
  guard.drain = true;
  int rc = small_encode_launch(m, dl, c->enc, in_blob, in_off, n32, qw, p, z, slots, true, h_off, st, err);
  if (rc) return rc;
  const uint32_t region_cap = 1u << SMALL_SHIFT;
  {
    ScanArgs A = scan_args_of(dl);
    A.tiles = c->enc.tiles; A.ntiles = slots * n32; A.q_bits = c->enc.q_bits; A.q_cv = c->enc.q_cv;
    A.chunk = 64; A.chunk_fused = 32;
    A.raw = c->raw; A.region_cap = region_cap; A.rctr = c->rctr; A.qexact = c->enc.qexact; A.want_exact = 0; A.drop_len = 1;
    A.q_rec = c->enc.q_rec;
    A.fuse = (switches().fuse_prefilter && switches().prefilter) ? 1 : 0;
    A.qpairs = nullptr; A.dbg = 0;
    const dim3 grid((A.ntiles + 3) / 4);
    with_nplanes(dl->nplanes, [&](auto np) { hipLaunchKernelGGL(k_scan_small<decltype(np)::value>, grid, dim3(256), 0, st, A); });
  }
  ScorePlan plan = score_plan_of(m, dl, p.score_threshold, qw, d);
  plan.sa.dbg = 0; plan.sa.store_pairs = 0;
  if (!plan.fits()) return 1;
  const ScoreArgs& sa = plan.sa;
  const uint32_t threads = plan.threads;
  const int fastD = plan.fastD;
  const SurvOut so{c->surv, c->sctr, SMALL_SURV_CAP, nullptr, 0u};
  const SlotLists sl = slot_lists_of(c->list8, c->listg, c->listw, c->lctr, SMALL_SURV_CAP);
  const PairArgs pa = pair_args_of(dl, c->raw, c->enc.q_meta, c->enc.q_rows, c->enc.q_rec, nullptr, nullptr, c->qmaxfreq, c->qsurv, c->qexpand);
  uint32_t fs_cap = 2048;
  while (fs_cap < region_cap && fs_cap < n32 * 12u + 2048u) fs_cap *= 2u;
  FilterArgs fa;
  fa.region_shift = SMALL_SHIFT; fa.rctr = c->rctr; fa.qexact = c->enc.qexact; fa.stop = 0; fa.enable = plan.enable_filter;
  const bool use8 = fastD > 0 && threads == 256;
  fa.use_nw8 = (plan.have_long_q || use8) ? 1 : 0; fa.counters = c->counters; fa.stat_ctr = c->sctr; fa.fill_cap = fs_cap; fa.blk = SMALL_FS_BLK;
  {
    const double key[12] = {sa.w_ld, sa.w_lcs, sa.w_prefix, sa.w_suffix, sa.w_case, sa.w_sum, sa.score_threshold, (double)sa.have_freq + 2.0 * (double)sa.any_variants, (double)sa.lqp, (double)sa.lcp, (double)sa.stride,
                            (double)sa.qw + 1e3 * (double)(reinterpret_cast<uintptr_t>(sa.quot) & 0xFFFFFFFFu)};
    if (!c->cold_valid || memcmp(key, c->cold_key, sizeof key) != 0) {
      memcpy(c->cold_key, key, sizeof key);
      c->h_cold_last = FsCold{sa, so, sl.l8, sl.lg, sl.lw};
      if (hipMemcpyAsync(c->d_cold, &c->h_cold_last, sizeof(FsCold), hipMemcpyHostToDevice, st) != hipSuccess || hipStreamSynchronize(st) != hipSuccess) {
        err = "small path: argument upload";
        return ANX_ENODEVICE;
      }
      c->cold_valid = true;
    }
  }
  launch_filter_score(plan, dim3(((fs_cap + SMALL_FS_BLK - 1) / SMALL_FS_BLK) * SCAN_REGIONS), st, fa, pa, static_cast<const FsCold*>(c->d_cold));
  const int do_wide = (plan.split_wide && plan.enable_filter) ? 1 : 0;
  if (threads == 256) {
    launch_small_lists(plan, st, SmallListArgs{sl.lw, sl.l8, sl.lg, do_wide, (fastD && (plan.have_long_q || use8)) ? 1 : 0, fastD}, fa, pa, so);
  } else {
    const dim3 lgrid(SMALL_LIST_BLOCKS * SCAN_REGIONS);
    if (do_wide) hipLaunchKernelGGL(k_filter_wide, lgrid, dim3(256), 0, st, sl.lw, fa, pa, sa, fastD, sl.l8, sl.lg);
    if (fastD && plan.have_long_q) launch_score_fast8(fastD, lgrid, st, sl.l8, pa, sa, so);
    hipLaunchKernelGGL(k_score_pairs, lgrid, dim3(threads), plan.lds_bytes(), st, sl.lg, pa, sa, so);
  }
  const RankArgs ra = rank_args_of(m, dl, p, p.cutoff_threshold);
  const uint32_t crow_cap = (uint32_t)c->row_cap;
  hipLaunchKernelGGL(k_small_offsets, dim3(1), dim3(SMALL_T), 0, st, c->qsurv, n32, c->soff, c->qcur);
  if (dl->any_variants)
    hipLaunchKernelGGL(k_compact_expand, dim3(EXPAND_P * SCAN_REGIONS), dim3(EXPAND_B), 0, st, c->surv, c->sctr, SMALL_SURV_CAP, m.have_freq ? 1 : 0, c->qcur, dl->ent_rec,
                       dl->ent_var_off, dl->var_target, dl->var_target_freq, dl->var_score, c->c_rows, c->soff + n32, crow_cap, c->counters + CTR_OVERFLOW);
  else
    hipLaunchKernelGGL(k_compact_grouped, dim3(SCAN_REGIONS), dim3(COMPACT_B), 0, st, c->surv, c->sctr, SMALL_SURV_CAP, m.have_freq ? 1 : 0, c->qcur, dl->ent_rec, c->c_rows,
                       c->soff + n32, crow_cap, c->counters + CTR_OVERFLOW);
  launch_rank(ra, st, n32, c->soff, c->c_rows, c->qmaxfreq, c->qexpand, c->t_key, c->r_rows, c->r_count, crow_cap, c->counters + CTR_OVERFLOW, SegRows{nullptr, 0u, nullptr});
  hipLaunchKernelGGL(k_small_fetch, dim3(n32 > 256u ? SMALL_FETCH_BLOCKS : 1u), dim3(SMALL_T), 0, st, n32, c->soff, c->r_count, c->r_rows, c->rctr, c->sctr, c->lctr, c->counters, h_off64, rows, (uint32_t)row_cap, crow_cap, h_ctl);
  if (hipGetLastError() != hipSuccess || hipStreamSynchronize(st) != hipSuccess) {
    err = std::string("small path: ") + hipGetErrorString(hipGetLastError());
    return ANX_ENODEVICE;
  }
  guard.drain = false;
  const SmallCtl ctl = *h_ctl;
  if (ctl.rows > row_cap || ctl.maxfill > fs_cap || ctl.surv_fill > SMALL_SURV_CAP || ctl.list_fill > SMALL_SURV_CAP || ctl.total_surv > crow_cap || ctl.overflow) {
    g_small_overflow.fetch_add(1, std::memory_order_relaxed);
    return 1;
  }
  size_t* offs = static_cast<size_t*>(malloc((n + 1) * sizeof(size_t)));
  if (!offs) { err = "out of memory"; return ANX_EINVAL; }
  static_assert(sizeof(size_t) == sizeof(unsigned long long), "offsets are copied as they are");
  memcpy(offs, h_off64, (n + 1) * sizeof(size_t));
  guard.rows = nullptr;
  *out_rows = rows;
  *out_offs = offs;
  g_small_taken.fetch_add(1, std::memory_order_relaxed);
  return ANX_OK;
}
```

Before: 54.52 billion.

## Fold result totals into rank kernel and consolidate counters into one block

Removes the post-rank exclusive scan over result counts (and the r_off buffer). Per-block sum and max of kept rows are now reduced inside k_rank and k_conf_apply_late and atomically added into regional slots. All device counters are packed into one contiguous block so they can be cleared with one memset and read back with one D2H copy, replacing several memsets and memcpys. The per-query qsurv/qmaxfreq/qexpand arrays are also merged into one allocation with a single memset. This trades a few kernel launches and API calls for extra shuffles, a block barrier and atomics at the end of the rank kernels.

New measurement: 53.99 billion. No clear change (-1.0%).

```diff
diff --git a/analiticcl_amd/csrc/conf.hip b/analiticcl_amd/csrc/conf.hip
--- a/analiticcl_amd/csrc/conf.hip
+++ b/analiticcl_amd/csrc/conf.hip
@@ -272,11 +272,9 @@
   if (x.dist_score != y.dist_score) return x.dist_score > y.dist_score;
   return x.freq_score > y.freq_score;
 }
-__global__ __launch_bounds__(256) void k_conf_apply_late(ConfArgs a, uint32_t* __restrict__ r_count) {
-  const uint32_t s = blockIdx.x * 256 + threadIdx.x;
-  if (s >= a.nq || a.soff[a.nq] > a.row_cap || *a.overflow) return;
+__device__ inline uint32_t conf_late_query(const ConfArgs& a, uint32_t s, uint32_t* __restrict__ r_count) {
   const uint32_t n = r_count[s], base = a.soff[s];
-  if (n == 0) return;
+  if (n == 0) return 0u;
   DevRow* __restrict__ v = a.r_rows + base;
   bool any = false;
   for (uint32_t k = 0; k < n; ++k) {
@@ -297,6 +295,30 @@
       if (conf_vr_score(v[k], a.freq_weight) <= best / a.cutoff_threshold) { len = k; break; }
   }
   r_count[s] = len;
+  return len;
+}
+__global__ __launch_bounds__(256) void k_conf_apply_late(ConfArgs a, uint32_t* __restrict__ r_count, uint32_t* __restrict__ rtot) {
+  __shared__ uint32_t s_sum[4], s_max[4];
+  if (a.soff[a.nq] > a.row_cap || *a.overflow) return;
+  const uint32_t s = blockIdx.x * 256 + threadIdx.x;
+  const uint32_t len = s < a.nq ? conf_late_query(a, s, r_count) : 0u;
+  uint32_t sum = len, mx = len;
+#pragma unroll
+  for (int o = 32; o; o >>= 1) {
+    sum += (uint32_t)__shfl_xor((int)sum, o);
+    mx = max(mx, (uint32_t)__shfl_xor((int)mx, o));
+  }
+  if ((threadIdx.x & 63u) == 0u) { s_sum[threadIdx.x >> 6] = sum; s_max[threadIdx.x >> 6] = mx; }
+  __syncthreads();
+  if (threadIdx.x == 0) {
+    sum = s_sum[0] + s_sum[1] + s_sum[2] + s_sum[3];
+    mx = max(max(s_max[0], s_max[1]), max(s_max[2], s_max[3]));
+    if (sum) {
+      uint32_t* slot = rtot + (blockIdx.x % SCAN_REGIONS) * RC_STRIDE;
+      atomicAdd(&slot[RT_SUM_LATE], sum);
+      atomicMax(&slot[RT_MAX_LATE], mx);
+    }
+  }
 }
 
 namespace {
@@ -375,7 +397,6 @@
     b->cf_sort_tmp_bytes = bytes;
   }
   uint32_t* sort_buf = b->cf_sort;
-  if (!b->cf_ctr) HIP_TRY(pool_malloc(reinterpret_cast<void**>(&b->cf_ctr), 16));
   const uint32_t cf_blocks = std::min<uint32_t>(CF_BLOCKS, std::max<uint32_t>(1u, (row_cap + 63u) / 64u));
   if (b->cf_work && b->cf_work_blocks < cf_blocks) { pool_free(b->cf_work); b->cf_work = nullptr; }
   if (!b->cf_work) {
@@ -387,7 +408,6 @@
     }
     b->cf_work_blocks = cf_blocks;
   }
-  HIP_TRY(hipMemsetAsync(b->cf_ctr, 0, 16, st));
   ConfArgs a;
   a.nq = nq; a.row_cap = row_cap; a.early = early ? 1 : 0; a.soff = b->soff; a.r_count = b->r_count; a.c_rows = b->c_rows; a.r_rows = b->r_rows;
   a.overflow = b->counters + CTR_OVERFLOW;
@@ -409,7 +429,7 @@
   hipLaunchKernelGGL(k_conf_script, dim3(b->cf_work_blocks), dim3(CF_THREADS), 0, st, a);
   ktimer_end(kt, st);
   if (early) { if (nblk) hipLaunchKernelGGL(k_conf_apply_early, dim3(nblk), dim3(256), 0, st, a); }
-  else hipLaunchKernelGGL(k_conf_apply_late, dim3((nq + 255u) / 256u), dim3(256), 0, st, a, b->r_count);
+  else hipLaunchKernelGGL(k_conf_apply_late, dim3((nq + 255u) / 256u), dim3(256), 0, st, a, b->r_count, b->rtot);
   HIP_TRY(hipGetLastError());
   return ANX_OK;
 }
diff --git a/analiticcl_amd/csrc/engine.hip b/analiticcl_amd/csrc/engine.hip
--- a/analiticcl_amd/csrc/engine.hip
+++ b/analiticcl_amd/csrc/engine.hip
@@ -36,8 +36,7 @@
 #include "kernels_score.hpp"
 #include "kernels_rank.hpp"
 
-enum { HR_RCTR = 0, HR_SCTR = SCAN_REGIONS * RC_STRIDE, HR_LCTR = 2 * SCAN_REGIONS * RC_STRIDE, HR_CTR = 5 * SCAN_REGIONS * RC_STRIDE,
-       HR_TOTAL_SURV = HR_CTR + CTR_N, HR_TOTAL_RESULTS = HR_TOTAL_SURV + 1, HR_CONF = HR_TOTAL_RESULTS + 1 , HR_N = HR_CONF + 2 };
+enum { HR_RCTR = CB_RCTR, HR_SCTR = CB_SCTR, HR_LCTR = CB_LCTR, HR_RTOT = CB_RTOT, HR_CTR = CB_CTR, HR_CONF = CB_CONF , HR_N = CB_N };
 constexpr size_t HR_COLD_OFF = (HR_N * sizeof(uint32_t) + 63) & ~(size_t)63;
 static void shells_destroy(int device);
 static void small_ctxs_destroy(int device);
@@ -920,10 +919,13 @@
   const size_t nq = b->nq;
   int rc;
   const size_t nblk = (nq + SCAN_TILE - 1) / SCAN_TILE + 2;
-  if ((rc = dalloc(&b->counters, CTR_N, err)) || (rc = dalloc(&b->rctr, SCAN_REGIONS * RC_STRIDE, err)) || (rc = dalloc(&b->sctr, SCAN_REGIONS * RC_STRIDE, err)) || (rc = dalloc(&b->lctr, 3 * SCAN_REGIONS * RC_STRIDE, err)) || (rc = dalloc(&b->qexpand, nq, err)) || (rc = dalloc(&b->qsurv, nq, err)) ||
-      (rc = dalloc(&b->soff, nq + 1, err)) || (rc = dalloc(&b->qcur, nq, err)) || (rc = dalloc(&b->qmaxfreq, nq, err)) ||
-      (rc = dalloc(&b->scan_tmp, nblk, err)) || (rc = dalloc(&b->r_count, nq, err)) || (rc = dalloc(&b->r_off, nq + 1, err)))
+  if ((rc = dalloc(&b->cblock, CB_N, err)) || (rc = dalloc(&b->qsurv, 3 * nq, err)) ||
+      (rc = dalloc(&b->soff, nq + 1, err)) || (rc = dalloc(&b->qcur, nq, err)) ||
+      (rc = dalloc(&b->scan_tmp, nblk, err)) || (rc = dalloc(&b->r_count, nq, err)))
     return rc;
+  b->rctr = b->cblock + CB_RCTR; b->sctr = b->cblock + CB_SCTR; b->lctr = b->cblock + CB_LCTR; b->rtot = b->cblock + CB_RTOT;
+  b->counters = b->cblock + CB_CTR; b->cf_ctr = b->cblock + CB_CONF;
+  b->qmaxfreq = b->qsurv + nq; b->qexpand = b->qsurv + 2 * nq;
   return shell_acquire(b, err);
 }
 
@@ -1008,10 +1010,10 @@
   return batch_encode_spans(m, dl, blob.data(), blob.size(), off.data(), n, p, err, code, keep_text);
 }
 
-static int exclusive_scan(const uint32_t* in, uint32_t n, uint32_t* out, uint32_t* tmp, hipStream_t st, uint32_t* maxout = nullptr, uint32_t* copy = nullptr) {
+static int exclusive_scan(const uint32_t* in, uint32_t n, uint32_t* out, uint32_t* tmp, hipStream_t st, uint32_t* copy = nullptr) {
   const uint32_t nb = (n + SCAN_TILE - 1) / SCAN_TILE;
   if (nb == 0) return hipMemsetAsync(out, 0, sizeof(uint32_t), st) == hipSuccess ? 0 : -1;
-  hipLaunchKernelGGL(k_scan_local, dim3(nb), dim3(SCAN_THREADS), 0, st, in, n, out, tmp, maxout);
+  hipLaunchKernelGGL(k_scan_local, dim3(nb), dim3(SCAN_THREADS), 0, st, in, n, out, tmp);
   hipLaunchKernelGGL(k_scan_sums, dim3(1), dim3(SCAN_THREADS), 0, st, tmp, nb);
   hipLaunchKernelGGL(k_scan_add, dim3(nb), dim3(SCAN_THREADS), 0, st, out, n, tmp, nb, copy);
   return 0;
@@ -1254,8 +1256,8 @@
 
 int Run::scan() {
   int rc;
-  HIP_TRY(hipMemsetAsync(b->counters, 0, CTR_N * sizeof(uint32_t), st));
-  HIP_TRY(hipMemsetAsync(b->rctr, 0, SCAN_REGIONS * RC_STRIDE * sizeof(uint32_t), st));
+  HIP_TRY(hipMemsetAsync(b->cblock, 0, CB_N * sizeof(uint32_t), st));
+  HIP_TRY(hipMemsetAsync(b->qsurv, 0, (dl->any_variants ? 3 : 2) * (size_t)nq * sizeof(uint32_t), st));
   if (b->ntiles == 0) { HIP_TRY(hipEventRecord(b->ev_scan0, st)); HIP_TRY(hipEventRecord(b->ev[5], st)); }
   if (b->ntiles) {
     ScanArgs A = scan_args_of(dl);
@@ -1282,7 +1284,6 @@
     const uint32_t nsad = b->n_sad_tiles, nbits = A.ntiles - nsad, nadj = std::min(b->n_adj_tiles, nbits);
     with_nplanes(dl->nplanes, [&](auto np) { launch_scan<decltype(np)::value>(A, nadj, nbits, nsad, st, b->ev_scan0, b->ev[5]); });
   }
-  HIP_TRY(hipMemcpyAsync(b->h_read + HR_RCTR, b->rctr, SCAN_REGIONS * RC_STRIDE * sizeof(uint32_t), hipMemcpyDeviceToHost, st));
   HIP_TRY(hipEventRecord(b->ev[1], st));
   b->n_raw = (uint32_t)(SCAN_REGIONS << b->region_shift);
   return ANX_OK;
@@ -1290,9 +1291,6 @@
 
 int Run::score() {
   int rc;
-  HIP_TRY(hipMemsetAsync(b->qsurv, 0, nq * sizeof(uint32_t), st));
-  HIP_TRY(hipMemsetAsync(b->qmaxfreq, 0, nq * sizeof(uint32_t), st));
-  if (dl->any_variants) HIP_TRY(hipMemsetAsync(b->qexpand, 0, nq * sizeof(uint32_t), st));
   ScorePlan plan = score_plan_of(m, dl, b->params.score_threshold, b->qw, b->dmax);
   ScoreArgs& sa = plan.sa;
 #ifdef ANX_DEBUG_SWITCHES
@@ -1308,8 +1306,6 @@
   const bool need_lists = !fastD || plan.have_long_q || dl->max_len > 16;
   if (need_lists && (rc = ensure_slot_lists(b, b->prev_list_fill ? (size_t)b->prev_list_fill + (b->prev_list_fill >> 3) + 256 : (fastD ? (size_t)fill_cap / 2 : (size_t)fill_cap) / cap_div() + 256, err)))
     return rc;
-  HIP_TRY(hipMemsetAsync(b->sctr, 0, SCAN_REGIONS * RC_STRIDE * sizeof(uint32_t), st));
-  HIP_TRY(hipMemsetAsync(b->lctr, 0, 3 * SCAN_REGIONS * RC_STRIDE * sizeof(uint32_t), st));
   const SlotLists sl = slot_lists_of(b->list8, b->listg, b->listw, b->lctr, (uint32_t)b->list_cap);
   const PairArgs pa = pair_args_of(dl, b->raw, b->q_meta, b->q_rows, b->q_rec, b->p_score, b->p_meta, b->qmaxfreq, b->qsurv, b->qexpand);
   FilterArgs fa;
@@ -1338,7 +1334,7 @@
 int Run::compact_rank() {
   int rc;
   const RankArgs ra = rank_args_of(m, dl, b->params, b->conf_mode == 1 ? 0.0 : b->params.cutoff_threshold);
-  exclusive_scan(b->qsurv, nq, b->soff, b->scan_tmp, st, nullptr, b->qcur);
+  exclusive_scan(b->qsurv, nq, b->soff, b->scan_tmp, st, b->qcur);
   if (dl->any_variants) {
     uint32_t total_surv = 0;
     HIP_TRY(hipMemcpyAsync(&total_surv, b->soff + nq, sizeof(uint32_t), hipMemcpyDeviceToHost, st));
@@ -1366,21 +1362,14 @@
   HIP_TRY(hipEventRecord(b->ev[3], st));
   if (b->conf_mode == 2 && (rc = conf_launch(m, dl, b, st, true, row_cap, err))) return rc;
   launch_rank(ra, st, nq, b->soff, b->c_rows, b->qmaxfreq, b->qexpand, b->t_key, b->r_rows, b->r_count, dl->any_variants ? 0xFFFFFFFFu : row_cap, b->counters + CTR_OVERFLOW,
-              dl->any_variants ? SegRows{nullptr, 0u, nullptr} : SegRows{so.seg, so.seg_cap, dl->ent_rec});
+              dl->any_variants ? SegRows{nullptr, 0u, nullptr} : SegRows{so.seg, so.seg_cap, dl->ent_rec}, b->rtot);
   if (b->conf_mode == 1 && (rc = conf_launch(m, dl, b, st, false, row_cap, err))) return rc;
-  exclusive_scan(b->r_count, nq, b->r_off, b->scan_tmp, st, b->counters + CTR_MAXROWS);
   HIP_TRY(hipEventRecord(b->ev[4], st));
   return ANX_OK;
 }
 
 int Run::readback() {
-  HIP_TRY(hipMemcpyAsync(b->h_read + HR_SCTR, b->sctr, SCAN_REGIONS * RC_STRIDE * sizeof(uint32_t), hipMemcpyDeviceToHost, st));
-  HIP_TRY(hipMemcpyAsync(b->h_read + HR_LCTR, b->lctr, 3 * SCAN_REGIONS * RC_STRIDE * sizeof(uint32_t), hipMemcpyDeviceToHost, st));
-  HIP_TRY(hipMemcpyAsync(b->h_read + HR_CTR, b->counters, CTR_N * sizeof(uint32_t), hipMemcpyDeviceToHost, st));
-  HIP_TRY(hipMemcpyAsync(b->h_read + HR_TOTAL_SURV, b->soff + nq, sizeof(uint32_t), hipMemcpyDeviceToHost, st));
-  HIP_TRY(hipMemcpyAsync(b->h_read + HR_TOTAL_RESULTS, b->r_off + nq, sizeof(uint32_t), hipMemcpyDeviceToHost, st));
-  b->h_read[HR_CONF] = b->h_read[HR_CONF + 1] = 0;
-  if (b->conf_mode && b->cf_ctr) HIP_TRY(hipMemcpyAsync(b->h_read + HR_CONF, b->cf_ctr, 2 * sizeof(uint32_t), hipMemcpyDeviceToHost, st));
+  HIP_TRY(hipMemcpyAsync(b->h_read, b->cblock, CB_N * sizeof(uint32_t), hipMemcpyDeviceToHost, st));
   HIP_TRY(hipEventRecord(b->ev_done, st));
   HIP_TRY(hipGetLastError());
   return ANX_OK;
@@ -1439,7 +1428,15 @@
     nsel += h[HR_SCTR + r * RC_STRIDE + 1];
     for (int l = 0; l < 3; ++l) list_fill = std::max(list_fill, h[HR_LCTR + (l * SCAN_REGIONS + r) * RC_STRIDE]);
   }
-  const uint32_t total_surv = h[HR_TOTAL_SURV], total_results = h[HR_TOTAL_RESULTS];
+  const bool late = b->conf_mode == 1 && !b->conf_skipped;
+  uint64_t total_results = 0;
+  uint32_t max_rows = 0;
+  for (uint32_t r = 0; r < SCAN_REGIONS; ++r) {
+    const uint32_t* t = h + HR_RTOT + r * RC_STRIDE;
+    total_results += t[late ? RT_SUM_LATE : RT_SUM];
+    max_rows = std::max(max_rows, t[late ? RT_MAX_LATE : RT_MAX]);
+  }
+  const uint32_t total_surv = h[HR_RTOT + RT_TOTAL_SURV];
   b->conf_fallback = b->conf_mode != 0 && (h[HR_CONF + 1] != 0 || b->conf_skipped);
   b->stats.n_conf_scripts = b->conf_mode ? h[HR_CONF] : 0;
   b->stats.n_adj_tiles = std::min(b->n_adj_tiles, b->ntiles - b->n_sad_tiles);
@@ -1466,7 +1463,7 @@
   b->n_surv = total_surv;
   b->n_sel = nsel;
   b->n_results = total_results;
-  b->max_rows = h[HR_CTR + CTR_MAXROWS];
+  b->max_rows = max_rows;
   b->ran = true;
   anx_batch_stats& s = b->stats;
   s.n_queries = nq;
@@ -1789,11 +1786,11 @@
   (void)hipSetDevice(b->device);
   if (b->async_pending) (void)hipStreamSynchronize(reinterpret_cast<hipStream_t>(b->async_stream));
   if (b->launched) (void)hipEventSynchronize(b->ev_done);
-  for (void* p : {(void*)b->q_cv, (void*)b->q_bits, (void*)b->q_rows, (void*)b->q_rec, (void*)b->q_meta, (void*)b->q_orig, (void*)b->d_tiles, (void*)b->rctr, (void*)b->sctr, (void*)b->surv,
-                  (void*)b->counters, (void*)b->qexact, (void*)b->qsurv, (void*)b->soff, (void*)b->qcur,
-                  (void*)b->qmaxfreq, (void*)b->d_cold, (void*)b->qpairs, (void*)b->x_cnt, (void*)b->x_tmp, (void*)b->scan_tmp, (void*)b->raw, (void*)b->p_score, (void*)b->p_meta, (void*)b->list8, (void*)b->listg, (void*)b->listw, (void*)b->lctr,
-                  (void*)b->c_rows, (void*)b->sseg, (void*)b->qexpand, (void*)b->r_rows, (void*)b->t_key, (void*)b->r_count, (void*)b->r_off,
-                  (void*)b->d_text, (void*)b->d_textoff, (void*)b->cf_weight, (void*)b->cf_need, (void*)b->cf_ctr, b->cf_work, (void*)b->cf_sort, b->cf_sort_tmp})
+  for (void* p : {(void*)b->q_cv, (void*)b->q_bits, (void*)b->q_rows, (void*)b->q_rec, (void*)b->q_meta, (void*)b->q_orig, (void*)b->d_tiles, (void*)b->cblock, (void*)b->surv,
+                  (void*)b->qexact, (void*)b->qsurv, (void*)b->soff, (void*)b->qcur,
+                  (void*)b->d_cold, (void*)b->qpairs, (void*)b->x_cnt, (void*)b->x_tmp, (void*)b->scan_tmp, (void*)b->raw, (void*)b->p_score, (void*)b->p_meta, (void*)b->list8, (void*)b->listg, (void*)b->listw,
+                  (void*)b->c_rows, (void*)b->sseg, (void*)b->r_rows, (void*)b->t_key, (void*)b->r_count,
+                  (void*)b->d_text, (void*)b->d_textoff, (void*)b->cf_weight, (void*)b->cf_need, b->cf_work, (void*)b->cf_sort, b->cf_sort_tmp})
     if (p) pool_free(p);
   shell_release(b);
   delete b;
diff --git a/analiticcl_amd/csrc/kernels_common.hpp b/analiticcl_amd/csrc/kernels_common.hpp
--- a/analiticcl_amd/csrc/kernels_common.hpp
+++ b/analiticcl_amd/csrc/kernels_common.hpp
@@ -120,7 +120,10 @@
   mutable struct DeviceConf* dconf = nullptr;
 };
 
-enum { CTR_SKIPPED = 2, CTR_MAXROWS = 3 , CTR_OVERFLOW = 4 , CTR_N = 8 };
+enum { CTR_SKIPPED = 2, CTR_OVERFLOW = 4 , CTR_N = 8 };
+enum { CB_RCTR = 0, CB_SCTR = SCAN_REGIONS * RC_STRIDE, CB_LCTR = 2 * SCAN_REGIONS * RC_STRIDE, CB_RTOT = 5 * SCAN_REGIONS * RC_STRIDE,
+       CB_CTR = 6 * SCAN_REGIONS * RC_STRIDE, CB_CONF = CB_CTR + CTR_N, CB_N = CB_CONF + 8 };
+enum { RT_SUM = 0, RT_MAX = 1, RT_SUM_LATE = 2, RT_MAX_LATE = 3, RT_TOTAL_SURV = 4 };
 
 struct SurvRow {
   double score;
@@ -163,8 +166,10 @@
   uint32_t* q_meta = nullptr;
   uint32_t* q_orig = nullptr;
   Tile* d_tiles = nullptr;
+  uint32_t* cblock = nullptr;
   uint32_t* counters = nullptr;
   uint32_t* rctr = nullptr;
+  uint32_t* rtot = nullptr;
   uint32_t region_shift = 0;
   uint32_t region_fill[SCAN_REGIONS] = {};
   uint32_t* qexact = nullptr;
@@ -212,7 +217,6 @@
   double* t_key = nullptr;
   size_t surv_cap = 0;
   uint32_t* r_count = nullptr;
-  uint32_t* r_off = nullptr;
   uint32_t n_raw = 0;
   uint64_t n_sel = 0;
   uint64_t n_pairs = 0, n_surv = 0, n_results = 0;
diff --git a/analiticcl_amd/csrc/kernels_prefix.hpp b/analiticcl_amd/csrc/kernels_prefix.hpp
--- a/analiticcl_amd/csrc/kernels_prefix.hpp
+++ b/analiticcl_amd/csrc/kernels_prefix.hpp
@@ -24,7 +24,7 @@
 }
 __global__ __launch_bounds__(SCAN_THREADS) void k_scan_local(const uint32_t* __restrict__ in, uint32_t n,
                                                              uint32_t* __restrict__ out,
-                                                             uint32_t* __restrict__ blocksum, uint32_t* __restrict__ maxout) {
+                                                             uint32_t* __restrict__ blocksum) {
   const uint32_t i0 = blockIdx.x * SCAN_TILE + threadIdx.x * SCAN_ITEMS;
   uint32_t v[SCAN_ITEMS], s = 0;
 #pragma unroll
@@ -40,14 +40,6 @@
     ex += v[i];
   }
   if (threadIdx.x == 0) blocksum[blockIdx.x] = tot;
-  if (maxout) {
-    uint32_t mx = 0;
-#pragma unroll
-    for (int i = 0; i < SCAN_ITEMS; ++i) mx = max(mx, v[i]);
-#pragma unroll
-    for (int o = 32; o; o >>= 1) mx = max(mx, (uint32_t)__shfl_xor((int)mx, o));
-    if ((threadIdx.x & 63) == 0 && mx) atomicMax(maxout, mx);
-  }
 }
 __global__ __launch_bounds__(SCAN_THREADS) void k_scan_sums(uint32_t* __restrict__ blocksum, uint32_t nb) {
   uint32_t carry = 0;
diff --git a/analiticcl_amd/csrc/kernels_rank.hpp b/analiticcl_amd/csrc/kernels_rank.hpp
--- a/analiticcl_amd/csrc/kernels_rank.hpp
+++ b/analiticcl_amd/csrc/kernels_rank.hpp
@@ -137,6 +137,10 @@
   int have_freq, any_variants;
 };
 constexpr int RANK_LCAP = 128;
+struct RankTot {
+  uint32_t sum, mx;
+  __device__ __forceinline__ void add(uint32_t len) { sum += len; mx = max(mx, len); }
+};
 
 struct SegRows {
   const SurvSeg* seg;
@@ -170,7 +174,7 @@
                                   unsigned long long* __restrict__ s_ord, uint32_t* __restrict__ s_freq,
                                   double* __restrict__ s_sdist, double* __restrict__ s_sfreq, uint32_t seg0, uint32_t n,
                                   uint32_t maxf, uint32_t qex, const SurvRow* __restrict__ c_rows, const SegRows& sr, const RankArgs& a,
-                                  double* __restrict__ t_key, DevRow* __restrict__ r_rows, uint32_t* __restrict__ r_count) {
+                                  double* __restrict__ t_key, DevRow* __restrict__ r_rows, uint32_t* __restrict__ r_count, RankTot& tot) {
   const unsigned long long gmask = G >= 64 ? ~0ull : ((1ull << (G & 63)) - 1ull);
   if (!valid) n = 0;
   if (valid && n == 0 && gl == 0) r_count[q] = 0;
@@ -245,7 +249,7 @@
     const double best = docut ? result_score(s_sdist[0], s_sfreq[0], fw) : 0.0;
     const unsigned long long cut = (__ballot(have && docut && gl >= 1 && (uint32_t)gl < len && si <= best / a.cutoff_threshold) >> gshift) & gmask;
     if (cut) len = (uint32_t)__ffsll((long long)cut) - 1;
-    if (parallel_tail && gl == 0) r_count[q] = len;
+    if (parallel_tail && gl == 0) { r_count[q] = len; tot.add(len); }
   }
   if (n && !parallel_tail && gl == 0) {
     const float fw = a.freq_weight;
@@ -289,6 +293,7 @@
     }
     if (cutoff > 0) len = cutoff;
     r_count[q] = len;
+    tot.add(len);
   }
 }
 
@@ -298,7 +303,7 @@
                                   uint16_t* __restrict__ s_src, double* __restrict__ s_sdist, double* __restrict__ s_sfreq,
                                   uint32_t seg0, uint32_t n, uint32_t maxf, uint32_t qex,
                                   const SurvRow* __restrict__ c_rows, const SegRows& sr, const RankArgs& a, double* __restrict__ t_key,
-                                  DevRow* __restrict__ r_rows, uint32_t* __restrict__ r_count) {
+                                  DevRow* __restrict__ r_rows, uint32_t* __restrict__ r_count, RankTot& tot) {
   const unsigned long long gmask = G >= 64 ? ~0ull : ((1ull << (G & 63)) - 1ull);
   if (!valid) n = 0;
   const double max_freq = a.have_freq ? (double)maxf : (maxf ? 1.0 : 0.0);
@@ -377,7 +382,7 @@
   }
   if (kept > (uint32_t)LCAP) {
     rank_query_all<G, LCAP>(q, valid, gl, gshift, s_key, s_ord, s_freq, s_sdist, s_sfreq, seg0, n, maxf, qex, c_rows, sr, a, t_key,
-                            r_rows, r_count);
+                            r_rows, r_count, tot);
     return;
   }
   const bool one_row_per_lane = nloop <= (uint32_t)G;
@@ -468,7 +473,7 @@
     if (docut && !prune) cutthr = result_score(s_sdist[0], s_sfreq[0], fw) / a.cutoff_threshold;
     const unsigned long long cut = (__ballot(have && docut && gl >= 1 && (uint32_t)gl < len && si <= cutthr) >> gshift) & gmask;
     if (cut) len = (uint32_t)__ffsll((long long)cut) - 1;
-    if (parallel_tail && gl == 0) r_count[q] = len;
+    if (parallel_tail && gl == 0) { r_count[q] = len; tot.add(len); }
   }
   if (n && !parallel_tail && gl == 0) {
     const float fw = a.freq_weight;
@@ -512,6 +517,7 @@
     }
     if (cutoff > 0) len = cutoff;
     r_count[q] = len;
+    tot.add(len);
   }
 }
 
@@ -524,11 +530,13 @@
                                               const uint32_t* __restrict__ qexpand, RankArgs aa,
                                               double* __restrict__ t_key, DevRow* __restrict__ r_rows,
                                               uint32_t* __restrict__ r_count, uint32_t row_cap, const uint32_t* __restrict__ overflow,
-                                              SegRows sr) {
+                                              SegRows sr, uint32_t* __restrict__ rtot) {
   RankArgs a = aa;
   if (SIMPLE) { a.any_variants = 0; a.freq_weight = 0.0f; }
   __shared__ __attribute__((aligned(16))) uint8_t s_raw[4 * RANK_WAVE_BYTES];
+  if (rtot && blockIdx.x == 0 && threadIdx.x == 0) rtot[RT_TOTAL_SURV] = soff[nq];
   if (soff[nq] > row_cap || *overflow) return;
+  RankTot tot{0u, 0u};
   const int lane = threadIdx.x & 63, wid = threadIdx.x >> 6;
   uint8_t* wl = s_raw + wid * RANK_WAVE_BYTES;
   const uint32_t qbase = (blockIdx.x * 4 + wid) * RANK_QPW;
@@ -551,7 +559,7 @@
                        reinterpret_cast<unsigned long long*>(gb + 128), reinterpret_cast<uint32_t*>(gb + 256),
                        reinterpret_cast<uint16_t*>(gb + 320), reinterpret_cast<double*>(gb + 352), reinterpret_cast<double*>(gb + 480),
                        (uint32_t)__shfl((int)my_seg0, grp), ng, (uint32_t)__shfl((int)my_maxf, grp),
-                       (uint32_t)__shfl((int)my_qex, grp), c_rows, sr, a, t_key, r_rows, r_count);
+                       (uint32_t)__shfl((int)my_qex, grp), c_rows, sr, a, t_key, r_rows, r_count, tot);
   }
   if (nmax > 16) {
     __builtin_amdgcn_fence(__ATOMIC_SEQ_CST, "workgroup");
@@ -573,7 +581,7 @@
                          reinterpret_cast<unsigned long long*>(gb + 256), reinterpret_cast<uint32_t*>(gb + 512),
                          reinterpret_cast<uint16_t*>(gb + 640), reinterpret_cast<double*>(gb + 704), reinterpret_cast<double*>(gb + 960),
                          (uint32_t)__shfl((int)my_seg0, src), (uint32_t)__shfl((int)my_n, src), (uint32_t)__shfl((int)my_maxf, src),
-                         (uint32_t)__shfl((int)my_qex, src), c_rows, sr, a, t_key, r_rows, r_count);
+                         (uint32_t)__shfl((int)my_qex, src), c_rows, sr, a, t_key, r_rows, r_count, tot);
       __builtin_amdgcn_fence(__ATOMIC_SEQ_CST, "workgroup");
     }
     for (int k = 0; k < RANK_QPW; ++k) {
@@ -585,21 +593,34 @@
                                 reinterpret_cast<uint32_t*>(wl + RANK_LCAP * 16), reinterpret_cast<uint16_t*>(wl + RANK_LCAP * 20),
                                 reinterpret_cast<double*>(wl + RANK_LCAP * 22), reinterpret_cast<double*>(wl + RANK_LCAP * 22 + 512),
                                 (uint32_t)__shfl((int)my_seg0, k), nk, (uint32_t)__shfl((int)my_maxf, k), (uint32_t)__shfl((int)my_qex, k),
-                                c_rows, sr, a, t_key, r_rows, r_count);
+                                c_rows, sr, a, t_key, r_rows, r_count, tot);
       __builtin_amdgcn_fence(__ATOMIC_SEQ_CST, "workgroup");
     }
   }
-}
-
-__global__ __launch_bounds__(256) void k_pack_rows(uint32_t nq, const uint32_t* __restrict__ soff,
-                                                   const uint32_t* __restrict__ r_off,
-                                                   const uint32_t* __restrict__ r_count,
-                                                   const DevRow* __restrict__ r_rows, DevRow* __restrict__ out) {
-  const uint32_t q = blockIdx.x * 256 + threadIdx.x;
-  if (q >= nq) return;
-  const uint32_t n = r_count[q], src = soff[q], dst = r_off[q];
-  for (uint32_t i = 0; i < n; ++i) out[dst + i] = r_rows[src + i];
-}
+  if (rtot) {
+    tot.sum += (uint32_t)__shfl_xor((int)tot.sum, 16);
+    tot.mx = max(tot.mx, (uint32_t)__shfl_xor((int)tot.mx, 16));
+    tot.sum += (uint32_t)__shfl_xor((int)tot.sum, 32);
+    tot.mx = max(tot.mx, (uint32_t)__shfl_xor((int)tot.mx, 32));
+    uint32_t* const wt = reinterpret_cast<uint32_t*>(wl);
+    if (lane == 0) { wt[0] = tot.sum; wt[1] = tot.mx; }
+    __syncthreads();
+    if (threadIdx.x == 0) {
+      uint32_t sum = 0, mx = 0;
+      for (int w = 0; w < 4; ++w) {
+        const uint32_t* o = reinterpret_cast<const uint32_t*>(s_raw + w * RANK_WAVE_BYTES);
+        sum += o[0];
+        mx = max(mx, o[1]);
+      }
+      if (sum) {
+        uint32_t* slot = rtot + (blockIdx.x % SCAN_REGIONS) * RC_STRIDE;
+        atomicAdd(&slot[RT_SUM], sum);
+        atomicMax(&slot[RT_MAX], mx);
+      }
+    }
+  }
+}
+
 __global__ __launch_bounds__(256) void k_fetch_counts(uint32_t nq, const uint32_t* __restrict__ r_count,
                                                       const uint32_t* __restrict__ q_orig, uint32_t* __restrict__ cnt_orig) {
   const uint32_t s = blockIdx.x * 256 + threadIdx.x;
diff --git a/analiticcl_amd/csrc/launch_plan.hpp b/analiticcl_amd/csrc/launch_plan.hpp
--- a/analiticcl_amd/csrc/launch_plan.hpp
+++ b/analiticcl_amd/csrc/launch_plan.hpp
@@ -115,8 +115,8 @@
   return ra;
 }
 static inline void launch_rank(const RankArgs& ra, hipStream_t st, uint32_t nq, const uint32_t* soff, const SurvRow* c_rows, const uint32_t* qmaxfreq, const uint32_t* qexpand, double* t_key,
-                               DevRow* r_rows, uint32_t* r_count, uint32_t row_cap, const uint32_t* overflow, const SegRows& seg) {
+                               DevRow* r_rows, uint32_t* r_count, uint32_t row_cap, const uint32_t* overflow, const SegRows& seg, uint32_t* rtot) {
   const dim3 grid((nq + 4 * RANK_QPW - 1) / (4 * RANK_QPW));
-  if (!ra.any_variants && ra.freq_weight == 0.0f) hipLaunchKernelGGL(k_rank<true>, grid, dim3(256), 0, st, nq, soff, c_rows, qmaxfreq, qexpand, ra, t_key, r_rows, r_count, row_cap, overflow, seg);
-  else hipLaunchKernelGGL(k_rank<false>, grid, dim3(256), 0, st, nq, soff, c_rows, qmaxfreq, qexpand, ra, t_key, r_rows, r_count, row_cap, overflow, seg);
+  if (!ra.any_variants && ra.freq_weight == 0.0f) hipLaunchKernelGGL(k_rank<true>, grid, dim3(256), 0, st, nq, soff, c_rows, qmaxfreq, qexpand, ra, t_key, r_rows, r_count, row_cap, overflow, seg, rtot);
+  else hipLaunchKernelGGL(k_rank<false>, grid, dim3(256), 0, st, nq, soff, c_rows, qmaxfreq, qexpand, ra, t_key, r_rows, r_count, row_cap, overflow, seg, rtot);
 }
diff --git a/analiticcl_amd/csrc/small_path.hpp b/analiticcl_amd/csrc/small_path.hpp
--- a/analiticcl_amd/csrc/small_path.hpp
+++ b/analiticcl_amd/csrc/small_path.hpp
@@ -214,7 +214,7 @@
   else
     hipLaunchKernelGGL(k_compact_grouped, dim3(SCAN_REGIONS), dim3(COMPACT_B), 0, st, c->surv, c->sctr, SMALL_SURV_CAP, m.have_freq ? 1 : 0, c->qcur, dl->ent_rec, c->c_rows,
                        c->soff + n32, crow_cap, c->counters + CTR_OVERFLOW);
-  launch_rank(ra, st, n32, c->soff, c->c_rows, c->qmaxfreq, c->qexpand, c->t_key, c->r_rows, c->r_count, crow_cap, c->counters + CTR_OVERFLOW, SegRows{nullptr, 0u, nullptr});
+  launch_rank(ra, st, n32, c->soff, c->c_rows, c->qmaxfreq, c->qexpand, c->t_key, c->r_rows, c->r_count, crow_cap, c->counters + CTR_OVERFLOW, SegRows{nullptr, 0u, nullptr}, nullptr);
   hipLaunchKernelGGL(k_small_fetch, dim3(n32 > 256u ? SMALL_FETCH_BLOCKS : 1u), dim3(SMALL_T), 0, st, n32, c->soff, c->r_count, c->r_rows, c->rctr, c->sctr, c->lctr, c->counters, h_off64, rows, (uint32_t)row_cap, crow_cap, h_ctl);
   if (hipGetLastError() != hipSuccess || hipStreamSynchronize(st) != hipSuccess) {
     err = std::string("small path: ") + hipGetErrorString(hipGetLastError());
```
